# DamRsn/VocoderProject

Measured on AMD Instinct MI355X. Metric: STFT-geometry frames/sec (1024-pt frames, hop 256) through the pitch-corrector/vocoder path, higher is better.
Workload: dtype f64

## Files before the change

### include/vp_amd.h

```cpp
#ifndef VP_AMD_H
#define VP_AMD_H

#include <stddef.h>

#ifdef __cplusplus
extern "C" {
#endif

#define VP_ABI_VERSION 3

enum {
    VP_OK = 0,
    VP_ERR_INVALID_ARG = -1,
    VP_ERR_NOT_PREPARED = -2,
    VP_ERR_INVALID_OVERLAP = -3,
    VP_ERR_GEOMETRY = -4,
    VP_ERR_ORDER = -5,
    VP_ERR_NO_DEVICE = -6,
    VP_ERR_HIP = -7,
    VP_ERR_OOM = -8,
    VP_ERR_TIMEOUT = -9
};

typedef struct vp_params {
// ... 23 lines not shown

int vp_create(int device, vp_handle **out);
int vp_destroy(vp_handle *h);

int vp_set_params(vp_handle *h, const vp_params *p);
int vp_get_params(const vp_handle *h, vp_params *p);
int vp_set_stream_params(vp_handle *h, int stream, const vp_params *p);
int vp_get_stream_params(const vp_handle *h, int stream, vp_params *p);
void vp_default_params(vp_params *p);

int vp_set_pitch_shift(vp_handle *h, int stream, int on, double semitones);
int vp_get_pitch_shift(const vp_handle *h, int stream, int *on, double *semitones);

int vp_prepare_to_play(vp_handle *h, double sample_rate, int samples_per_block, int n_streams);

int vp_prepare_explicit(vp_handle *h, double sample_rate, int samples_per_block, int n_streams,
                        int frame_len_pitch, int hop_pitch, int wlen_voc, int hop_voc);

int vp_process_block(vp_handle *h, const float *in, float *out);

int vp_process_block_inplace(vp_handle *h, float *io);

int vp_process_block_device(vp_handle *h, const float *d_in, float *d_out, void *hip_stream);
int vp_process_block_mono(vp_handle *h, const float *voice, float *out);
int vp_process_block_mono_device(vp_handle *h, const float *d_voice, float *d_out, void *hip_stream);
int vp_process_blocks_mono_device(vp_handle *h, const float *d_voice, float *d_out, int n_blocks, void *hip_stream);
int vp_process_blocks_device(vp_handle *h, const float *d_in, float *d_out, int n_blocks, void *hip_stream);
int vp_process_blocks(vp_handle *h, const float *in, float *out, int n_blocks);
int vp_process_block_channels(vp_handle *h, const float *const *in, int n_in, float *const *out, int n_out);
int vp_process_block_channels_device(vp_handle *h, const float *const *d_in, int n_in, float *const *d_out, int n_out, void *hip_stream);
int vp_process_blocks_channels_device(vp_handle *h, const float *const *d_in, int n_in, float *const *d_out, int n_out, int n_blocks, void *hip_stream);
int vp_reserve_blocks(vp_handle *h, int n_blocks);
int vp_get_reserved_blocks(const vp_handle *h);
long vp_debug_alloc_count(const vp_handle *h);

#define VP_IIR_EXACT 0
#define VP_IIR_FAST 1
int vp_set_iir_mode(vp_handle *h, int mode);
int vp_get_iir_mode(const vp_handle *h);

#define VP_VOC_AUTO 0
#define VP_VOC_WORKGROUP 1
#define VP_VOC_BATCHED 2
int vp_set_vocoder_path(vp_handle *h, int path);
int vp_get_vocoder_path(const vp_handle *h);

#define VP_OVERLAP_AUTO 2
int vp_set_overlap(vp_handle *h, int on);
int vp_get_overlap(const vp_handle *h);
int vp_set_time_parallel(vp_handle *h, int on);
int vp_get_time_parallel(const vp_handle *h);
int vp_set_wave_specialised(vp_handle *h, int on);
int vp_get_wave_specialised(const vp_handle *h);

#define VP_YIN_DIRECT 0
#define VP_YIN_FFT 1
#define VP_YIN_XCORR 2
#define VP_YIN_XCORR_FORCE_FALLBACK 3
int vp_set_yin_mode(vp_handle *h, int mode);
int vp_get_yin_mode(const vp_handle *h);

int vp_get_latency(const vp_handle *h);
int vp_get_geometry(const vp_handle *h, int out[12]);
int vp_get_num_streams(const vp_handle *h);

int vp_read_pitch_state(vp_handle *h, int stream, vp_pitch_state *out);

int vp_synchronize(vp_handle *h);
int vp_debug_set_spin_limit(vp_handle *h, int polls);

#define VP_NUM_KERNEL_SLOTS 4
int vp_profile_enable(vp_handle *h, int on);
int vp_profile_read(vp_handle *h, double ms[VP_NUM_KERNEL_SLOTS], long launches[VP_NUM_KERNEL_SLOTS], int reset);
const char *vp_kernel_slot_name(int slot);
const char *vp_pitch_kernel_name(const vp_handle *h);
const char *vp_vocoder_kernel_name(const vp_handle *h);

int vp_read_ub_counters(vp_handle *h, long out[5]);

int vp_debug_read_stamps(vp_handle *h, unsigned long long out[64], int reset);
int vp_debug_read_ws_stamps(vp_handle *h, unsigned long long out[512], int reset);
int vp_debug_read_stream_ticks(vp_handle *h, unsigned long long *out, int n, int reset);

typedef struct vp_stft vp_stft;
int vp_stft_create(int device, int n_streams, int n_samples, int frame_len, int hop, vp_stft **out);
int vp_stft_destroy(vp_stft *p);
int vp_stft_num_frames(const vp_stft *p);
int vp_stft_roundtrip(vp_stft *p, const float *d_in, float *d_out, float *d_mag, void *hip_stream);
int vp_stft_pitch_shift(vp_stft *p, const float *d_in, float *d_out, double semitones, void *hip_stream);
int vp_stft_pitch_shift_curve(vp_stft *p, const float *d_in, float *d_out, const double *d_ratio, void *hip_stream);
int vp_stft_pitch_shift_locked(vp_stft *p, const float *d_in, float *d_out, const double *d_ratio, void *hip_stream);
int vp_stft_pitch_shift_locked_subbin(vp_stft *p, const float *d_in, float *d_out, const double *d_ratio, void *hip_stream);
#define VP_HARM_MAX_VOICES 4
int vp_stft_harmonize(vp_stft *p, const float *d_in, float *d_out, int n_voices, const double *d_ratio, const double *d_gain, const double *d_dry,
                      void *hip_stream);
#define VP_FORMANT_LIFTER_MIN 4
#define VP_FORMANT_LIFTER_MAX 64
int vp_stft_pitch_shift_formant(vp_stft *p, const float *d_in, float *d_out, const double *d_ratio, const double *d_formant, int lifter,
                                void *hip_stream);
int vp_stft_cross_synth(vp_stft *p, const float *d_voice, const float *d_carrier, float *d_out, const double *d_depth, int lifter, void *hip_stream);
int vp_semitones_to_ratios(const double *semitones, double *ratios, long n);
int vp_stft_time_stretch(vp_stft *p, const float *d_in, int n_in, const int *d_pos, float *d_out, double semitones, void *hip_stream);
int vp_stft_time_stretch_locked(vp_stft *p, const float *d_in, int n_in, const int *d_pos, float *d_out, const double *d_ratio, void *hip_stream);
int vp_stretch_positions(int *pos, int n_frames, int hop, double stretch, int n_in, int frame_len);
int vp_onset_num_frames(int n_in, int frame_len, int hop);
int vp_stft_onset_flux(vp_stft *p, const float *d_in, int n_in, double *d_flux, double *d_mass, void *hip_stream);
// ... 87 lines not shown
```

### vocoderproject_amd/build.py

```python
import os
import re
import shutil
import subprocess
import sys
import time

HERE = os.path.dirname(os.path.abspath(__file__))
CSRC = os.path.join(HERE, "csrc")
ROOT = os.path.dirname(HERE)
LIB = os.path.join(HERE, "libvp_amd.so")
SOURCES = ["vp_kernels.hip", "vp_voc2.hip", "vp_stft.hip", "vp_channels.hip", "vp_track.hip", "vp_capi.hip"]
ARCH = "gfx950"
NUM_TUS = 9


def deps_of(source):
    seen, todo = set(), [os.path.join(CSRC, source)]
    while todo:
        path = os.path.normpath(todo.pop())
        if path in seen:
            continue
        seen.add(path)
        with open(path, encoding="utf-8", errors="replace") as f:
            for inc in re.findall(r'^[ \t]*#[ \t]*include[ \t]*"([^"]+)"', f.read(), re.M):
                for d in (os.path.dirname(path), CSRC, os.path.join(ROOT, "include")):
                    if os.path.exists(os.path.join(d, inc)):
                        todo.append(os.path.join(d, inc))
                        break
    return sorted(seen)


DEP_PATHS = sorted({p for s in SOURCES for p in deps_of(s)})
DEPS = [os.path.basename(p) for p in DEP_PATHS]


def hipcc():
    return shutil.which("hipcc") or "/opt/rocm/bin/hipcc"


_HIPCC_VERSION = None


def hipcc_version():
    global _HIPCC_VERSION
    if _HIPCC_VERSION is None:
        try:
            _HIPCC_VERSION = subprocess.run([hipcc(), "--version"], capture_output=True, text=True, timeout=60).stdout
        except (OSError, subprocess.SubprocessError):
            _HIPCC_VERSION = "unknown"
    return _HIPCC_VERSION


def needs_build():
    if not os.path.exists(LIB):
        return True
    t = os.path.getmtime(LIB)
    return any(os.path.getmtime(p) > t for p in DEP_PATHS)


LIB_STAMPS = os.path.join(HERE, "libvp_amd_stamps.so")
LIB_POISON = os.path.join(HERE, "libvp_amd_poison.so")


CACHE_CAP_BYTES = 600 << 20


def prune_cache(cap=CACHE_CAP_BYTES):
    cache = os.path.join(HERE, ".build_cache")
    try:
        ents = []
        now = time.time()
        for f in os.listdir(cache):
            p = os.path.join(cache, f)
            try:
                if ".part" in f:
                    if now - os.path.getmtime(p) > 3600:
                        os.remove(p)
                    continue
                ents.append((os.path.getmtime(p), os.path.getsize(p), p))
            except OSError:
                pass
    except OSError:
        return
    total = sum(e[1] for e in ents)
    for _, size, path in sorted(ents):
        if total <= cap:
            break
        try:
            os.remove(path)
            total -= size
        except OSError:
            pass


def build(force=False, verbose=False, stamps=False, poison=False):
    lib = LIB_STAMPS if stamps else LIB_POISON if poison else (os.environ.get("VP_LIB_OUT") or LIB)
    if not stamps and not poison and not force and lib == LIB and not needs_build():
        return LIB
    import tempfile
    from concurrent.futures import ThreadPoolExecutor
    common = [hipcc(), "-std=c++17", "-O3", "-ffp-contract=off", "-fdenormal-fp-math=preserve-sign", "-fPIC", f"--offload-arch={ARCH}", "-Wall", "-Wno-unused-function",
              "-I", os.path.join(ROOT, "include"), "-I", CSRC]
    common += os.environ.get("VP_EXTRA_HIPCC_FLAGS", "").split()
    if stamps:
        common.append("-DVP_STAMPS")
    if poison:
        common.append("-DVP_POISON_LDS")
    groups = [0] if not (stamps or poison or os.environ.get("VP_SPLIT_BUILD") == "1") else list(range(1, NUM_TUS + 1))
    with tempfile.TemporaryDirectory(prefix="vp_build_") as tmp:
        jobs = [(os.path.join(CSRC, "vp_kernels.hip"), os.path.join(tmp, f"k{k}.o"), [f"-DVP_TU={k}"]) for k in groups]
        jobs.append((os.path.join(CSRC, "vp_voc2.hip"), os.path.join(tmp, "voc2.o"), []))
        jobs.append((os.path.join(CSRC, "vp_stft.hip"), os.path.join(tmp, "stft.o"), os.environ.get("VP_STFT_EXTRA_FLAGS", "-fno-slp-vectorize -ffp-contract=fast").split()))
        jobs.append((os.path.join(CSRC, "vp_channels.hip"), os.path.join(tmp, "channels.o"), []))
        jobs.append((os.path.join(CSRC, "vp_track.hip"), os.path.join(tmp, "track.o"), []))
        jobs.append((os.path.join(CSRC, "vp_capi.hip"), os.path.join(tmp, "capi.o"), []))

        def compile_one(job):
            import hashlib
            src, obj, extra = job
            cmd = common + extra + ["-c", src, "-o", obj]
            hsh = hashlib.sha256((hipcc_version() + " ".join(cmd[:-1]).replace(tmp, "")).encode())
            for dep in deps_of(src):
                with open(dep, "rb") as f:
                    hsh.update(f.read())
            cache = os.path.join(HERE, ".build_cache")
            os.makedirs(cache, exist_ok=True)
            cached = os.path.join(cache, os.path.basename(obj) + "." + hsh.hexdigest()[:20])
            if os.path.exists(cached) and not force and not os.environ.get("VP_NO_OBJ_CACHE"):
                try:
                    shutil.copy(cached, obj)
                    os.utime(cached)
                    return obj
                except OSError:
                    pass
            if verbose:
                print(" ".join(cmd))
            subprocess.check_call(cmd)
            part = cached + ".part%d" % os.getpid()
            shutil.copy(obj, part)
            os.replace(part, cached)
            return obj

        with ThreadPoolExecutor(len(jobs)) as ex:
            objs = list(ex.map(compile_one, jobs))
        prune_cache()
        link = [hipcc(), "-shared", "-fPIC", f"--offload-arch={ARCH}"] + objs + ["-o", lib]
        if verbose:
            print(" ".join(link))
        subprocess.check_call(link)
    return lib


if __name__ == "__main__":
    print(build(force="--force" in sys.argv, verbose=True, stamps="--stamps" in sys.argv, poison="--poison" in sys.argv))
```

### vocoderproject_amd/csrc/vp_capi.hip

```cpp
#include <hip/hip_runtime.h>

#include <algorithm>
#include <cmath>
#include <cstdint>
#include <cstdio>
#include <cstdlib>
#include <cstring>
#include <string>
#include <type_traits>
#include <vector>

#include "../../include/vp_amd.h"
#include "vp_kernels.h"
#include "vp_voc2.h"
#include "vp_stft.h"
#include "vp_channels.h"
#include "vp_track.h"

struct vp_handle {
    int device = 0;
    bool prepared = false;
    vp_params params;
    VpGeom g;
    VpDev d;
    int inCounter = 0, outCounter = 0, currCounter = 0;
    struct Cohort { int pitchOn, vocOn, vStart, pStart, nChunk, n; int *dMap; std::vector<int> ids; int ordHi = 0, oVmax = 0, oSmax = 0; };
    std::vector<Cohort> cohorts;
    bool cohortsDirty = false;
    int *dMapAll = nullptr;
    std::vector<int> mapHost;
    bool poisoned = false;
    int poisonCode = VP_ERR_HIP;
    unsigned int *faultHost = nullptr, *faultDev = nullptr;
    int spinLimit = 1 << 22;
    VpV2 v2;
    int vocPath = VP_VOC_AUTO, oVmax = 0, oSmax = 0, nWinMax = 0;
    VpV2 v2mb;
    int v2mbWin = 0;
    std::vector<void *> mbAllocs;
    float *snapV = nullptr, *snapS = nullptr; int *gateB = nullptr; double *pLin = nullptr;
    std::vector<void *> bothAllocs;
    hipStream_t auxStream = nullptr;
    hipEvent_t evFork = nullptr, evJoin = nullptr;
    double *acc2 = nullptr;
    int overlap = VP_OVERLAP_AUTO, acc2Live = 0;
    int accLive = 0;
    int waveSpec = 1;
    int timeParallel = 0;
    std::vector<void *> allocs;
    float *stageIn = nullptr, *stageOut = nullptr;
    int synthNonZero = 0;
    float *stageInB = nullptr, *stageOutB = nullptr; int stageBlocks = 0;
    int reservedBlocks = 0;
    float *chHostIn = nullptr, *chHostOut = nullptr;
    long nAllocs = 0;
    hipStream_t ownStream = nullptr;
    int vocWaves = 8;
    size_t vocLds = 0, pitchLds = 0, ldsMax = 0;
    int prof = 0;
    unsigned profTick = 0;
    bool profThis = false;
    int iirMode = 0, yinMode = 0;
    std::vector<vp_params> sparams;
    std::vector<VpStreamParams> spHost;
    std::vector<int> shiftOn;
    std::vector<double> shiftSemi, shiftBeta;
    bool perStream = false, spDirty = false;
    struct EvPair { hipEvent_t a, b; int slot; };
    std::vector<EvPair> pending;
    std::vector<hipEvent_t> evPool;
    double profMs[VP_NUM_KERNEL_SLOTS] = {0, 0, 0, 0};
    long profN[VP_NUM_KERNEL_SLOTS] = {0, 0, 0, 0};
    std::string lastError;
};

static int fail_hip(vp_handle *h, hipError_t e, const char *what)
{
    char buf[256];
    snprintf(buf, sizeof buf, "%s: %s", what, hipGetErrorString(e));
    if (h) h->lastError = buf;
    return VP_ERR_HIP;
}
#define HIPCHK(h, call) do { hipError_t _e = (call); if (_e != hipSuccess) return fail_hip((h), _e, #call); } while (0)

static int poisoned_rc(vp_handle *h)
{
    h->lastError = h->poisonCode == VP_ERR_TIMEOUT
        ? "an earlier launch timed out on an inter-wavefront wait (its output and the device state are void): prepare again"
        : "an earlier HIP failure left the handle out of step with its device state: prepare again";
    return h->poisonCode;
}
static int check_fault(vp_handle *h)
{
    if (!h->faultHost) return VP_OK;
    const unsigned f = *(volatile unsigned int *)h->faultHost;
    if (f == 0) return VP_OK;
    h->poisoned = true; h->poisonCode = VP_ERR_TIMEOUT;
    char buf[200];
    snprintf(buf, sizeof buf, "a kernel's bounded wait ran out (counter dbg[%u], see vp_debug_read_stamps): the block's output is invalid; prepare again", f & 0xff);
    h->lastError = buf;
// ... 17 lines not shown
    case VP_ERR_INVALID_OVERLAP: return "Invalid overlap";
    case VP_ERR_GEOMETRY: return "invalid frame geometry";
    case VP_ERR_ORDER: return "LPC order is larger than OrderMax";
    case VP_ERR_NO_DEVICE: return "no HIP device (this library has no CPU fallback)";
    case VP_ERR_HIP: return "HIP runtime error";
    case VP_ERR_OOM: return "out of device memory";
    case VP_ERR_TIMEOUT: return "a kernel's bounded inter-wavefront wait ran out: the output is invalid, prepare again";
    default: return "unknown error";
    }
}

extern "C" const char *vp_last_error(const vp_handle *h) { return h ? h->lastError.c_str() : ""; }

static bool pitch_lite(const vp_handle *h, bool iirFast)
{
    return h->g.S > 256 && (iirFast || h->g.orderPitch <= 16) && h->pitchLds <= 80 * 1024 && h->g.htabGlobal;
}

static bool pitch_common_geom(const vp_handle *h)
{
    return (h->g.C & 63) == 0 && h->g.orderPitch <= 15 && h->g.tauMax <= 512 && h->g.eLen >= h->g.F + 4 * h->g.tauMax + 1;
}
static bool pitch_common(const vp_handle *h)
{
    return pitch_common_geom(h) && (h->g.F == 512 || h->g.F == 1024) && h->pitchLds + 16 + vp_pitch_fft_lds_bytes(2 * (h->g.F >> 9)) <= h->ldsMax;
}

typedef void (*vp_dsp_kernel)(VpGeom, VpCall, VpDev, const float *, float *);
struct PitchPlan { vp_dsp_kernel fn; const char *name; size_t lds; };
#define VP_PLAN(K, LDS) PitchPlan{K, #K, LDS}
static PitchPlan pitch_plan(const vp_handle *h, bool fast, int nBlocks)
{
    const bool lite = pitch_lite(h, fast), com = lite ? pitch_common_geom(h) : pitch_common(h);
    const size_t lds = h->pitchLds;
    if (nBlocks > 1) {
        if (lite) return com ? VP_PLAN(vp_k_pitch_lite_fast_multi_c, lds) : VP_PLAN(vp_k_pitch_lite_fast_multi, lds);
        return fast ? (com ? VP_PLAN(vp_k_pitch_fast_multi_c, lds) : VP_PLAN(vp_k_pitch_fast_multi, lds)) : VP_PLAN(vp_k_pitch_multi, lds);
    }
    if (lite) return fast ? (com ? VP_PLAN(vp_k_pitch_lite_fast_c, lds) : VP_PLAN(vp_k_pitch_lite_fast, lds)) : VP_PLAN(vp_k_pitch_lite, lds);
    if (com) return fast ? VP_PLAN(vp_k_pitch_fast_c, lds) : VP_PLAN(vp_k_pitch_c, lds);
    return fast ? VP_PLAN(vp_k_pitch_fast, lds) : VP_PLAN(vp_k_pitch, lds);
}
static bool pitch_ws_ok(const vp_handle *h, bool fast, int nBlocks, int nSteps)
{
    static const bool off = getenv("VP_NO_WS") != nullptr;
    const VpGeom &g = h->g;
    if (off || !h->waveSpec || nBlocks != 1 || nSteps <= 0 || pitch_lite(h, fast) || g.F != 1024 || (g.C & 63) != 0 || g.C > 512 || g.cpf < 2 ||
        g.orderPitch > WS_ORDER_MAX || g.tauMax > 512) return false;
    if ((size_t)(g.toKeep + g.F + (nSteps - 1) * g.C) >= (size_t)g.inSize) return false;
    if (nSteps + (nSteps + g.cpf - 2) / (g.cpf - 1) + 1 > WS_MAXI || (nSteps + g.cpf - 2) / (g.cpf - 1) + 1 > WS_MAXS) return false;
    return vp_pitch_ws_lds_bytes(g, nSteps) + 256 <= h->ldsMax;
}

static int pitch_xfft_waves(const vp_handle *h, bool fast, int nBlocks)
{
    if (!pitch_common(h) || pitch_lite(h, fast) || (nBlocks > 1 && !fast)) return 0;
    int fw = 2 * (h->g.F >> 9);
    static const int envWaves = [] { const char *e = getenv("VP_XFFT_WAVES"); return e ? atoi(e) : 0; }();
    if (envWaves == fw / 2) fw = envWaves;
    return fw;
}
static size_t pitch_xfft_lds(const vp_handle *h) { return vp_pitch_fft_lds_bytes(2 * (h->g.F >> 9)); }
#undef VP_PLAN

extern "C" const char *vp_pitch_kernel_name(const vp_handle *h)
{
    if (!h || !h->prepared) return "";
    const bool fast = h->iirMode == VP_IIR_FAST;
    if (pitch_ws_ok(h, fast, 1, (h->g.N + h->g.C - 1) / h->g.C))
        return h->g.orderPitch > 15 ? (fast ? "vp_k_pitch_ws_o24" : "vp_k_pitch_ws_x_o24") : (fast ? "vp_k_pitch_ws" : "vp_k_pitch_ws_x");
    return pitch_plan(h, fast, 1).name;
}

static int voc_lite_slots(const vp_handle *h, bool iirFast, int nw)
{
    if (!(h->g.S > 256 && iirFast) || getenv("VP_VOC_NO_LITE")) return 0;
    int nl = std::max(1, std::min(nw, 4));
    while (nl > 1 && vp_voc_lds_bytes(h->g.W, nl) > (size_t)(80 * 1024 - 512)) nl--;
    return vp_voc_lds_bytes(h->g.W, nl) <= (size_t)(80 * 1024 - 512) ? nl : 0;
}

#define VP_V2_MIN_STREAMS 257
#define VP_V2_MIN_WINDOWS 1024
static bool voc_auto_batched(const vp_handle *h)
{
    return h->g.S >= VP_V2_MIN_STREAMS && (size_t)h->g.S * h->nWinMax >= VP_V2_MIN_WINDOWS;
}
static bool voc_pipeline_wanted(const vp_handle *h)
{
    return h->v2.xT && h->vocPath != VP_VOC_WORKGROUP && (h->vocPath == VP_VOC_BATCHED || voc_auto_batched(h));
}
static bool voc_batched_for(const vp_handle *h, int nWin, int oV, int oS)
{
    if (!voc_pipeline_wanted(h) || nWin < 1 || nWin > 64) return false;
    return oV <= V2_ORDER_MAX && oS <= VP_ORDER_MAX_SYNTH && oV >= 2 && oS >= 2;
}

static bool voc_o48(int oVmax) { return oVmax > 32 && oVmax <= 48; }

extern "C" int vp_set_vocoder_path(vp_handle *h, int path)
{
    if (!h || path < VP_VOC_AUTO || path > VP_VOC_BATCHED) return VP_ERR_INVALID_ARG;
    if (path != h->vocPath) h->cohortsDirty = true;
    h->vocPath = path;
    return VP_OK;
}
extern "C" int vp_get_vocoder_path(const vp_handle *h) { return h ? h->vocPath : VP_ERR_INVALID_ARG; }
extern "C" int vp_set_overlap(vp_handle *h, int on)
{
    if (!h || on < 0 || on > VP_OVERLAP_AUTO) return VP_ERR_INVALID_ARG;
    h->overlap = on;
    return VP_OK;
}
extern "C" int vp_get_overlap(const vp_handle *h) { return h ? h->overlap : VP_ERR_INVALID_ARG; }
extern "C" int vp_set_time_parallel(vp_handle *h, int on)
{
    if (!h) return VP_ERR_INVALID_ARG;
    h->timeParallel = on ? 1 : 0;
    return VP_OK;
}
extern "C" int vp_get_time_parallel(const vp_handle *h) { return h ? h->timeParallel : VP_ERR_INVALID_ARG; }
extern "C" int vp_set_wave_specialised(vp_handle *h, int on)
{
    if (!h) return VP_ERR_INVALID_ARG;
    h->waveSpec = on ? 1 : 0;
    return VP_OK;
}
extern "C" int vp_get_wave_specialised(const vp_handle *h) { return h ? h->waveSpec : VP_ERR_INVALID_ARG; }

extern "C" const char *vp_vocoder_kernel_name(const vp_handle *h)
{
    if (!h || !h->prepared) return "";
    {
        int oV = 0, oS = 0, nLow = 0;
        for (const auto &q : h->sparams) if (q.lpcVoice <= V2_ORDER_MAX) { oV = std::max(oV, q.lpcVoice); oS = std::max(oS, q.lpcSynth); nLow++; }
        if (nLow > 0 && voc_batched_for(h, h->nWinMax, oV, oS)) return "vp_k_v2_pipeline";
    }
    if (voc_lite_slots(h, h->iirMode == VP_IIR_FAST, h->vocWaves)) return "vp_k_vocoder_lite";
    int oV = 0;
    for (const auto &q : h->sparams) oV = std::max(oV, q.lpcVoice);
    return (oV > 32 && oV <= 48) ? "vp_k_vocoder_o48" : "vp_k_vocoder";
}

extern "C" const char *vp_kernel_slot_name(int slot)
{
    static const char *n[VP_NUM_KERNEL_SLOTS] = {"vp_k_ingest_gate", "vp_k_vocoder", "vp_k_pitch", "vp_k_emit"};
    return (slot >= 0 && slot < VP_NUM_KERNEL_SLOTS) ? n[slot] : "";
}

extern "C" void vp_default_params(vp_params *p)
{
    p->gainPitch = 0.0f; p->gainVoice = -60.0f; p->gainSynth = -60.0f; p->gainVoc = 0.0f;
    p->lpcVoice = 40; p->lpcPitch = 15; p->lpcSynth = 5; p->keyPitch = 12;
    p->pitchBool = 1; p->vocBool = 1;
}

static bool params_valid(const vp_params *p)
{
    auto gain_ok = [](float v) { return v >= -60.0f && v <= 6.0f; };
    return gain_ok(p->gainPitch) && gain_ok(p->gainVoice) && gain_ok(p->gainSynth) && gain_ok(p->gainVoc) &&
           p->lpcVoice >= 2 && p->lpcVoice <= VP_ORDER_MAX && p->lpcPitch >= 2 && p->lpcPitch <= VP_ORDER_MAX &&
           p->lpcSynth >= 2 && p->lpcSynth <= VP_ORDER_MAX_SYNTH && p->keyPitch >= 0 && p->keyPitch <= 12 &&
           (p->pitchBool == 0 || p->pitchBool == 1) && (p->vocBool == 0 || p->vocBool == 1);
}

extern "C" int vp_create(int device, vp_handle **out)
{
    if (!out) return VP_ERR_INVALID_ARG;
    *out = nullptr;
    int n = 0;
    if (hipGetDeviceCount(&n) != hipSuccess || n <= 0) return VP_ERR_NO_DEVICE;
    if (device < 0 || device >= n) return VP_ERR_INVALID_ARG;
    vp_handle *h = new vp_handle();
    h->device = device;
    vp_default_params(&h->params);
    memset(&h->g, 0, sizeof h->g);
    memset(&h->d, 0, sizeof h->d);
    if (hipSetDevice(device) != hipSuccess || hipStreamCreateWithFlags(&h->ownStream, hipStreamNonBlocking) != hipSuccess ||
        hipStreamCreateWithFlags(&h->auxStream, hipStreamNonBlocking) != hipSuccess ||
        hipEventCreateWithFlags(&h->evFork, hipEventDisableTiming) != hipSuccess ||
// ... 257 lines not shown
    int rc = fill_voc_window(vocWin, W, hop);
    if (rc) return rc;
    rc = fill_pitch_st_window(pitchSt, F, H);
    if (rc) return rc;

    std::vector<int> hannOff(g.tauMax + 1, 0);
    size_t tot = 0;
    for (int T = 1; T <= g.tauMax; T++) { hannOff[T] = (int)tot; tot += 2 * (size_t)T + 1; }
    std::vector<double> hannTab(tot);
    for (int T = 1; T <= g.tauMax; T++) fill_hann(hannTab.data() + hannOff[T], 2 * T + 1);

    std::vector<double> notes(13 * VP_NOTES_STRIDE, 0.0);
    std::vector<int> notesN(13);
    for (int k = 0; k < 13; k++) notesN[k] = build_notes(k, fMin, fMax, notes.data() + (size_t)k * VP_NOTES_STRIDE);

    hipDeviceProp_t prop;
    HIPCHK(h, hipGetDeviceProperties(&prop, h->device));
    const size_t ldsMax = std::min<size_t>((size_t)prop.maxSharedMemoryPerMultiProcessor ? prop.maxSharedMemoryPerMultiProcessor : 65536, 160 * 1024) - 256;
    g.xsSteps = 1;
    g.htabGlobal = 0;
    if (g.S > 256) {
        VpGeom t = g;
        t.xsSteps = 1;
        if (vp_pitch_lds_bytes(t) <= (size_t)80 * 1024) g.htabGlobal = 1;
    }
    {
        const int stepsMax = (N + g.C - 1) / g.C;
        size_t budget = std::min<size_t>(ldsMax, (g.S > 256 ? 80 : 112) * 1024);
        {
            VpGeom t = g;
            t.xsSteps = 1;
            if (vp_pitch_lds_bytes(t) > budget) budget = ldsMax;
        }
        for (int k = stepsMax; k >= 1; k--) {
            VpGeom t = g;
            t.xsSteps = k;
            if ((size_t)(g.toKeep + F + (k - 1) * g.C) < (size_t)g.inSize && vp_pitch_lds_bytes(t) <= budget) { g.xsSteps = k; break; }
        }
    }
    h->pitchLds = vp_pitch_lds_bytes(g);
    h->ldsMax = ldsMax;
    if (h->pitchLds > ldsMax) { h->lastError = "pitch frame does not fit LDS"; return VP_ERR_GEOMETRY; }
    int nw = 8;
    while (nw > 1 && vp_voc_lds_bytes(W, nw) > ldsMax) nw--;
    if (const char *e = getenv("VP_VOC_WAVES")) { int v = atoi(e); if (v >= 1 && v < nw) nw = v; }
    if (vp_voc_lds_bytes(W, nw) > ldsMax) { h->lastError = "vocoder window does not fit LDS"; return VP_ERR_GEOMETRY; }
    h->vocWaves = nw;
    h->vocLds = vp_voc_lds_bytes(W, nw);
    {
        const void *fns[] = {(const void *)vp_k_pitch, (const void *)vp_k_pitch_fast, (const void *)vp_k_pitch_multi,
                             (const void *)vp_k_pitch_fast_multi, (const void *)vp_k_pitch_lite, (const void *)vp_k_pitch_lite_fast,
                             (const void *)vp_k_pitch_c, (const void *)vp_k_pitch_fast_c, (const void *)vp_k_pitch_fast_multi_c,
                             (const void *)vp_k_pitch_lite_fast_c, (const void *)vp_k_pitch_lite_fast_multi, (const void *)vp_k_pitch_lite_fast_multi_c,
                             (const void *)vp_k_pitch_ws, (const void *)vp_k_pitch_ws_x, (const void *)vp_k_pitch_ws_mb, (const void *)vp_k_pitch_ws_x_mb, (const void *)vp_k_pitch_ws_mb_o24, (const void *)vp_k_pitch_ws_x_mb_o24, (const void *)vp_k_pitch_ws_o24, (const void *)vp_k_pitch_ws_x_o24,
                             (const void *)vp_k_vocoder, (const void *)vp_k_vocoder_o48, (const void *)vp_k_vocoder_lite};
        for (const void *f : fns) {
            hipFuncAttributes fa;
            HIPCHK(h, hipFuncGetAttributes(&fa, f));
            HIPCHK(h, hipFuncSetAttribute(f, hipFuncAttributeMaxDynamicSharedMemorySize, (int)(ldsMax + 256 - fa.sharedSizeBytes)));
        }
    }

    VpDev d;
    memset(&d, 0, sizeof d);
    RC(dev_alloc(h, &d.voiceRing, (size_t)S * g.inSize));
    RC(dev_alloc(h, &d.synthRing, (size_t)S * 2 * g.inSize));
    RC(dev_alloc(h, &d.outAcc, (size_t)S * g.outSize));
    RC(dev_alloc(h, &h->acc2, (size_t)S * g.outSize));
    h->acc2Live = 0; h->accLive = 0;
    RC(dev_alloc(h, &d.gate, (size_t)S * 2));
    RC(dev_alloc(h, &d.pitch, (size_t)S));
    RC(dev_alloc(h, &d.eFrame, (size_t)S * g.eLen));
    RC(dev_alloc(h, &d.outEFrame, (size_t)S * F));
    RC(dev_alloc(h, &d.yFrame, (size_t)S * F));
    RC(dev_alloc(h, &d.EeArr, (size_t)S * 20));
    RC(dev_alloc(h, &d.hImp, (size_t)S * 128));
    RC(dev_alloc(h, &d.ub, (size_t)5));
    RC(dev_alloc(h, &d.dbg, (size_t)64 + (size_t)S + 512));
    vocWin.resize((size_t)W + 16, 0.0);
    RC(dev_upload(h, &d.vocWin, vocWin));
    RC(dev_upload(h, &d.pitchStWin, pitchSt));
    RC(dev_upload(h, &d.hannTab, hannTab));
    RC(dev_upload(h, &d.hannOff, hannOff));
    RC(dev_upload(h, &d.notes, notes));
    RC(dev_upload(h, &d.notesN, notesN));
    {
        const double PI = 3.141592653589793238;
        std::vector<double> t1(64 * 8 * 2), t2(64 * 8 * 2), ts(64 * 4 * 2);
        for (int lane = 0; lane < 64; lane++) {
            for (int r = 0; r < 8; r++) {
                const double a1 = -2.0 * PI * (double)(r * (lane >> 3)) / 64.0, a2 = -2.0 * PI * (double)(r * lane) / 512.0;
                t1[(lane * 8 + r) * 2] = std::cos(a1); t1[(lane * 8 + r) * 2 + 1] = std::sin(a1);
                t2[(lane * 8 + r) * 2] = std::cos(a2); t2[(lane * 8 + r) * 2 + 1] = std::sin(a2);
            }
            for (int q = 0; q < 4; q++) {
                const double a = -2.0 * PI * (double)(64 * q + lane) / 1024.0;
                ts[(lane * 4 + q) * 2] = std::cos(a); ts[(lane * 4 + q) * 2 + 1] = std::sin(a);
            }
        }
        RC(dev_upload(h, &d.fftTw1, t1));
        RC(dev_upload(h, &d.fftTw2, t2));
        RC(dev_upload(h, &d.fftTws, ts));
    }
    RC(dev_alloc(h, &h->dMapAll, (size_t)S));
    {
        memset(&h->v2, 0, sizeof h->v2);
        h->nWinMax = (N + hop - 1) / hop;
        const size_t NW = (size_t)S * h->nWinMax;
        if (h->nWinMax <= 64 && vp_v2_init() == 0) {
            h->v2.nGroupsMax = (int)((NW + 63) / 64);
            h->v2.W4p = (W + 3) / 4 + 16;
            h->v2.W2p = (W + 1) / 2 + 2;
            RC(dev_alloc(h, &h->v2.xT, (size_t)2 * h->v2.nGroupsMax * h->v2.W4p * 256));
            RC(dev_alloc(h, &h->v2.eT, (size_t)2 * h->v2.nGroupsMax * h->v2.W2p * 128));
            RC(dev_alloc(h, &h->v2.out, NW * W));
            const size_t NWp = (size_t)h->v2.nGroupsMax * 64;
            RC(dev_alloc(h, &h->v2.rV, NWp * V2_RV_STRIDE));
            RC(dev_alloc(h, &h->v2.aV, NWp * V2_RV_STRIDE));
            RC(dev_alloc(h, &h->v2.rS, NWp * V2_RS_STRIDE));
            RC(dev_alloc(h, &h->v2.aS, NWp * V2_RS_STRIDE));
            RC(dev_alloc(h, &h->v2.meta, NWp));
            RC(dev_alloc(h, &h->v2.rank, NWp + S));
            RC(dev_alloc(h, &h->v2.liveList, NWp));
            RC(dev_alloc(h, &h->v2.EE, NW * 2));
            h->v2.nSlices = (W + V2_FIR_SLICE - 1) / V2_FIR_SLICE;
            RC(dev_alloc(h, &h->v2.EEp, NW * 2 * h->v2.nSlices));
        }
    }
    RC(dev_alloc(h, &h->stageIn, (size_t)S * 3 * N, false));
    RC(dev_alloc(h, &h->stageOut, (size_t)S * 3 * N, false));
    if (hipHostMalloc((void **)&h->chHostIn, (size_t)S * 3 * N * sizeof(float), hipHostMallocDefault) != hipSuccess ||
        hipHostMalloc((void **)&h->chHostOut, (size_t)S * 2 * N * sizeof(float), hipHostMallocDefault) != hipSuccess) {
        (void)hipGetLastError();
        free_all(h);
        h->lastError = "out of pinned host memory for the channel staging buffers";
        return VP_ERR_OOM;
    }
    {
        std::vector<VpPitchState> init(S);
        memset(init.data(), 0, init.size() * sizeof(VpPitchState));
        for (auto &p : init) p.beta = 1;
        if (hipMemcpy(d.pitch, init.data(), init.size() * sizeof(VpPitchState), hipMemcpyHostToDevice) != hipSuccess) {
            free_all(h);
            return VP_ERR_HIP;
        }
    }
    d.fault = h->faultDev; d.spinLimit = h->spinLimit;
    *(volatile unsigned int *)h->faultHost = 0;
    h->g = g;
    h->d = d;
    h->inCounter = g.toKeep + g.latency;
    h->outCounter = 0;
    h->currCounter = g.toKeep;
    h->cohorts.assign(1, vp_handle::Cohort{h->params.pitchBool, h->params.vocBool, 0, 0, 0, S, nullptr, {}});
    h->cohortsDirty = false; h->poisoned = false; h->poisonCode = VP_ERR_HIP;
    h->sparams.assign((size_t)S, h->params);
    h->spHost.assign((size_t)S, VpStreamParams{});
    h->synthNonZero = 0;
    h->shiftOn.assign((size_t)S, 0); h->shiftSemi.assign((size_t)S, 0.0); h->shiftBeta.assign((size_t)S, 1.0);
    h->perStream = false; h->spDirty = true;
    h->prepared = true;
    (void)hipDeviceSynchronize();
    return VP_OK;
}

extern "C" int vp_prepare_to_play(vp_handle *h, double sampleRate, int samplesPerBlock, int nStreams)
{
    if (!h || !(sampleRate > 0)) return VP_ERR_INVALID_ARG;
    double ratioSR = sampleRate / 44100.0;
    int hopVoc = (int)std::floor(128.0 * ratioSR);
    int wlenVoc = 4 * hopVoc;
    int corres_256 = (int)std::floor(256.0 * ratioSR);
    int hopPitch = 3 * corres_256;
    int frameLenPitch = 4 * corres_256;
    return vp_prepare_explicit(h, sampleRate, samplesPerBlock, nStreams, frameLenPitch, hopPitch, wlenVoc, hopVoc);
}

static hipEvent_t get_event(vp_handle *h)
{
    if (!h->evPool.empty()) { hipEvent_t e = h->evPool.back(); h->evPool.pop_back(); return e; }
    hipEvent_t e;
    (void)hipEventCreate(&e);
    return e;
}

struct ProfScope {
    vp_handle *h; hipStream_t st; int slot; hipEvent_t a, b; bool on;
    ProfScope(vp_handle *h_, hipStream_t st_, int slot_) : h(h_), st(st_), slot(slot_)
    {
        on = h->profThis;
        if (on) { a = get_event(h); b = get_event(h); (void)hipEventRecord(a, st); }
    }
    ~ProfScope()
    {
        if (on) { (void)hipEventRecord(b, st); h->pending.push_back({a, b, slot}); }
    }
};

static void fill_stream_params(VpStreamParams &o, const vp_params &P)
{
    o.orderVoice = P.lpcVoice; o.orderSynth = P.lpcSynth; o.key = P.keyPitch;
    o.dryOn = ((double)P.gainVoice > -59.0);
    o.synthOn = ((double)P.gainSynth > -59.0);
    o.gainPitch = (double)db_to_gain_f(P.gainPitch);
    o.gainVoc = (double)db_to_gain_f(P.gainVoc);
    o.gainVoice = (double)db_to_gain_f(P.gainVoice);
    o.gainSynth = (double)db_to_gain_f(P.gainSynth);
}
// ... 68 lines not shown
    if (rc) return rc;
    VpCall c0;
    memset(&c0, 0, sizeof c0);
    c0.inCounter = h->inCounter; c0.outCounter = h->outCounter; c0.currCounter = h->currCounter;
    c0.inplace = inplace;
    c0.iirFast = h->iirMode;
    c0.nBlocks = 1;
    if (mono) {
        c0.inMono = h->synthNonZero > 0 ? 1 : 2;
        h->synthNonZero = std::max(0, h->synthNonZero - g.N * nBlocks);
    } else {
        c0.inMono = 0;
        h->synthNonZero = g.inSize;
    }
    c0.yinCert = (h->yinMode == VP_YIN_XCORR || h->yinMode == VP_YIN_FFT) ? 1 : (h->yinMode == VP_YIN_XCORR_FORCE_FALLBACK) ? 2 : 0;

    for (auto &co : h->cohorts) {
        VpCall c = c0;
        VpDev d = h->d;
        d.streamMap = co.dMap;
        d.outAcc2 = h->acc2Live > 0 ? h->acc2 : nullptr;
        c.pitchOn = co.pitchOn; c.vocOn = co.vocOn;
        c.vStart = co.vStart;
        c.nWin = 0;
        if (c.vocOn && co.vStart < g.N) c.nWin = (g.N - co.vStart + g.h - 1) / g.h;
        c.pStart = co.pStart; c.nChunk0 = co.nChunk;
        c.nSteps = 0;
        if (c.pitchOn && co.pStart < g.N) c.nSteps = (g.N - co.pStart + g.C - 1) / g.C;

        const bool runVoc = c.nWin > 0, runPitch = c.nSteps > 0 || (nBlocks > 1 && c.pitchOn);
        bool runPitchDone = false;
        if (!runVoc && !runPitch) {
            { ProfScope ps(h, st, 0); hipLaunchKernelGGL(vp_k_ingest_gate, dim3(co.n), dim3(256), 0, st, g, c, d, d_in); }
            { ProfScope ps(h, st, 3); hipLaunchKernelGGL(vp_k_emit, dim3(co.n), dim3(256), 0, st, g, c, d, d_out); }
        } else {
            const bool batched = runVoc && voc_batched_for(h, c.nWin, co.oVmax, co.oSmax);
            if (batched && runPitch && c.iirFast && nBlocks == 1 && (h->overlap == 1 || (h->overlap == VP_OVERLAP_AUTO && !pitch_lite(h, true)))) {
                struct Fork { vp_handle *h; hipStream_t st; VpGeom g; VpCall cp; VpDev dp; const float *in; float *out; int n; hipError_t err; } fk;
                fk.h = h; fk.st = st; fk.g = g; fk.cp = c; fk.dp = d; fk.in = d_in; fk.out = d_out; fk.n = co.n; fk.err = hipSuccess;
                fk.cp.fuseIngest = 0; fk.cp.fuseEmit = 0; fk.cp.nBlocks = 1;
                fk.dp.outAcc = h->acc2; fk.dp.outAcc2 = nullptr;
                auto fork = [](void *a) {
                    Fork *f = (Fork *)a;
                    vp_handle *h = f->h;
                    if ((f->err = hipEventRecord(h->evFork, f->st)) != hipSuccess) return;
                    if ((f->err = hipStreamWaitEvent(h->auxStream, h->evFork, 0)) != hipSuccess) return;
                    ProfScope ps(h, h->auxStream, 2);
                    PitchPlan plan = pitch_plan(h, true, 1);
                    if (const int fw = f->cp.yinCert ? pitch_xfft_waves(h, true, 1) : 0) {
                        const size_t off = (plan.lds + 15) / 16 * 16;
                        f->cp.fftOff = (int)off; f->cp.fftWaves = fw; plan.lds = off + pitch_xfft_lds(h);
                    }
                    f->cp.ldsBytes = (int)plan.lds;
                    hipLaunchKernelGGL(plan.fn, dim3(f->n), dim3(512), plan.lds, h->auxStream, f->g, f->cp, f->dp, f->in, f->out);
                };
                VpCall cv = c;
                cv.fuseIngest = 1; cv.fuseEmit = 0;
                VpV2 v = h->v2;
                v.nStreams = co.n; v.oVmax = co.oVmax; v.oSmax = co.oSmax;
                { ProfScope ps(h, st, 1); vp_v2_launch(g, cv, d, v, d_in, d_out, st, fork, &fk); }
                if (fk.err != hipSuccess) return fail_hip(h, fk.err, "fork of the pitch kernel");
                HIPCHK(h, hipEventRecord(h->evJoin, h->auxStream));
                HIPCHK(h, hipStreamWaitEvent(st, h->evJoin, 0));
                VpDev de = d;
                de.outAcc2 = h->acc2;
                { ProfScope ps(h, st, 3); hipLaunchKernelGGL(vp_k_emit, dim3(co.n), dim3(256), 0, st, g, c, de, d_out); }
                h->acc2Live = (g.outSize + g.N - 1) / g.N + 1;
                runPitchDone = true;
            } else if (batched) {
                VpCall cv = c;
                cv.fuseIngest = 1; cv.fuseEmit = runPitch ? 0 : 1;
                ProfScope ps(h, st, 1);
                VpV2 v = h->v2;
                v.nStreams = co.n; v.oVmax = co.oVmax; v.oSmax = co.oSmax;
                vp_v2_launch(g, cv, d, v, d_in, d_out, st);
            } else if (runVoc) {
                VpCall cv = c;
                cv.fuseIngest = 1; cv.fuseEmit = runPitch ? 0 : 1;
                ProfScope ps(h, st, 1);
                int nw = std::min(h->vocWaves, c.nWin);
                if (nw < 4) nw = std::min(4, h->vocWaves);
                const int nl = voc_lite_slots(h, cv.iirFast != 0, nw);
                const bool lite = nl > 0;
                if (lite) nw = nl;
                cv.ldsBytes = (int)vp_voc_lds_bytes(g.W, nw);
                cv.vocWin = nw;
                const int nThreads = 64 * nw * std::max(1, 8 / nw);
                hipLaunchKernelGGL(lite ? vp_k_vocoder_lite : voc_o48(co.oVmax) ? vp_k_vocoder_o48 : vp_k_vocoder, dim3(co.n), dim3(nThreads), vp_voc_lds_bytes(g.W, nw), st,
                                   g, cv, d, d_in, d_out);
            }
            if (runPitch && !runPitchDone) {
                VpCall cp = c;
                cp.fuseIngest = runVoc ? 0 : 1; cp.fuseEmit = 1;
                cp.nBlocks = nBlocks;
                ProfScope ps(h, st, 2);
                PitchPlan plan = pitch_plan(h, cp.iirFast != 0, nBlocks);
                const int fw = cp.yinCert ? pitch_xfft_waves(h, cp.iirFast != 0, nBlocks) : 0;
                const size_t fftMin = fw ? pitch_xfft_lds(h) + 16 : 0;
                if (nBlocks == 1 && !pitch_lite(h, cp.iirFast != 0) && plan.lds + vp_pitch_acc_lds_bytes(g) + 16 + fftMin <= h->ldsMax) {
                    cp.ldsAcc = 1;
                    plan.lds = ((plan.lds + 15) / 16) * 16 + vp_pitch_acc_lds_bytes(g);
                }
                if (fw) {
                    const size_t off = (plan.lds + 15) / 16 * 16;
                    cp.fftOff = (int)off; cp.fftWaves = fw; plan.lds = off + pitch_xfft_lds(h);
                }
                cp.ldsBytes = (int)plan.lds;
                if (pitch_ws_ok(h, cp.iirFast != 0, nBlocks, cp.nSteps)) {
                    cp.ldsAcc = 1; cp.fftOff = 0; cp.fftWaves = 0;
                    cp.ldsBytes = (int)vp_pitch_ws_lds_bytes(g, cp.nSteps);
                    static const int wsWaves = [] { const char *e = getenv("VP_WS_WAVES"); const int v = e ? atoi(e) : 0; return (v >= 8 && v <= 12) ? v : 12; }();
                    VpWsSched sc;
                    memset(&sc, 0, sizeof sc);
                    if (!ws_build_sched(g, cp.nChunk0, cp.nSteps, sc)) return fail_hip(h, hipErrorInvalidValue, "pitch schedule");
                    const auto wsk = g.orderPitch > 15 ? (cp.iirFast ? vp_k_pitch_ws_o24 : vp_k_pitch_ws_x_o24) : (cp.iirFast ? vp_k_pitch_ws : vp_k_pitch_ws_x);
                    hipLaunchKernelGGL(wsk, dim3(co.n), dim3(64 * wsWaves), (size_t)cp.ldsBytes, st, g, cp, d, sc, d_in, d_out);
                } else
                hipLaunchKernelGGL(plan.fn, dim3(co.n), dim3(512), plan.lds, st, g, cp, d, d_in, d_out);
            }
        }
        hipError_t e = hipGetLastError();
        if (e != hipSuccess) return fail_hip(h, e, "kernel launch");

        for (int b = 0; b < nBlocks; b++) {
            if (co.vocOn) {
                const int nWin = (co.vStart < g.N) ? (g.N - co.vStart + g.h - 1) / g.h : 0;
                co.vStart = co.vStart + nWin * g.h - g.N;
            }
            if (co.pitchOn) {
                const int nSteps = (co.pStart < g.N) ? (g.N - co.pStart + g.C - 1) / g.C : 0;
                int nChunk = co.nChunk;
                for (int i = 0; i < nSteps; i++) {
                    if (nChunk % g.cpf == g.cpf - 1) nChunk = 1 % g.cpf;
                    else nChunk += 1;
                }
                co.nChunk = nChunk;
                co.pStart = co.pStart + nSteps * g.C - g.N;
            }
        }
    }
    for (auto &co : h->cohorts)
        if (co.vocOn) h->accLive = (g.outSize + g.N - 1) / g.N + 1;
    h->acc2Live = std::max(0, h->acc2Live - nBlocks);
    h->accLive = std::max(0, h->accLive - nBlocks);
    for (int b = 0; b < nBlocks; b++) {
        h->outCounter = (h->outCounter + g.N) % g.outSize;
        h->inCounter = (h->inCounter + g.N) % g.inSize;
        h->currCounter = (h->currCounter + g.N) % g.inSize;
    }
    guard.armed = false;
    return VP_OK;
}

extern "C" int vp_process_block_device(vp_handle *h, const float *d_in, float *d_out, void *hip_stream)
{
    if (!h || !d_in || !d_out) return VP_ERR_INVALID_ARG;
    if (!h->prepared) return VP_ERR_NOT_PREPARED;
    if (hipSetDevice(h->device) != hipSuccess) return VP_ERR_NO_DEVICE;
    return process_device(h, d_in, d_out, (hipStream_t)hip_stream, 0);
}

static int ensure_v2mb(vp_handle *h, int nWin)
{
    if (nWin <= h->v2mbWin) return VP_OK;
    for (void *p : h->mbAllocs) (void)hipFree(p);
    h->mbAllocs.clear(); h->v2mbWin = 0;
    const VpGeom &g = h->g;
    VpV2 v;
    memset(&v, 0, sizeof v);
    const size_t NW = (size_t)g.S * nWin;
    v.nGroupsMax = (int)((NW + 63) / 64);
// ... 113 lines not shown
    *done = false;
    const VpGeom &g = h->g;
    if (h->cohorts.size() != 1 || nb < 2 || nb > V2_MB_MAX || h->iirMode != VP_IIR_FAST) return VP_OK;
    { const int mn = v2_mb_min_blocks(h, h->cohorts[0], true); if (mn == 0 || nb < mn) return VP_OK; }
    auto &co = h->cohorts[0];
    if (!co.vocOn || !co.pitchOn || !voc_pipeline_wanted(h)) return VP_OK;
    if (co.oVmax > V2_ORDER_MAX || co.oSmax > VP_ORDER_MAX_SYNTH || co.oVmax < 2 || co.oSmax < 2) return VP_OK;
    if ((size_t)g.outSize * sizeof(double) > (size_t)VP_V2_MB_LDS_MAX) return VP_OK;
    VpV2MB mb;
    memset(&mb, 0, sizeof mb);
    mb.nBlocks = nb; mb.preIngested = 1;
    int vs = co.vStart, NWs = 0;
    for (int b = 0; b < nb; b++) {
        const int nWin = (vs < g.N) ? (g.N - vs + g.h - 1) / g.h : 0;
        mb.vStart[b] = vs; mb.nWin[b] = nWin; mb.first[b] = NWs;
        NWs += nWin;
        vs = vs + nWin * g.h - g.N;
    }
    if (NWs < 1 || mb.nWin[0] < 1) return VP_OK;
    for (int b = 1; b < nb; b++)
        if (mb.nWin[b] > 0 && b * g.N + mb.vStart[b] != mb.vStart[0] + mb.first[b] * g.h) return VP_OK;
    if (h->poisoned) return poisoned_rc(h);
    if (int frc = check_fault(h)) return frc;
    if (NWs > h->v2mbWin || !h->pLin) return VP_OK;
    h->profThis = h->prof > 0 && (h->profTick++ % (unsigned)h->prof) == 0;
    struct Poison { vp_handle *h; bool armed; ~Poison() { if (armed) h->poisoned = true; } } guard{h, true};
    HIPCHK(h, hipMemcpyAsync(h->snapV, h->d.voiceRing, (size_t)g.S * g.inSize * sizeof(float), hipMemcpyDeviceToDevice, st));
    HIPCHK(h, hipMemcpyAsync(h->snapS, h->d.synthRing, (size_t)g.S * 2 * g.inSize * sizeof(float), hipMemcpyDeviceToDevice, st));
    VpCall c;
    memset(&c, 0, sizeof c);
    c.inCounter = h->inCounter; c.outCounter = h->outCounter; c.currCounter = h->currCounter;
    c.iirFast = 1; c.nBlocks = nb; c.inMono = 0; c.vocOn = 1; c.pitchOn = 1;
    c.yinCert = (h->yinMode == VP_YIN_XCORR || h->yinMode == VP_YIN_FFT) ? 1 : (h->yinMode == VP_YIN_XCORR_FORCE_FALLBACK) ? 2 : 0;
    VpDev d = h->d;
    d.streamMap = co.dMap;
    d.gateB = h->gateB;
    {
        VpGeom gp = g;
        gp.outSize = V2_MB_MAX * g.N + g.outSize;
        VpCall cp = c;
        cp.outCounter = 0;
        cp.pStart = co.pStart; cp.nChunk0 = co.nChunk;
        cp.nSteps = (co.pStart < g.N) ? (g.N - co.pStart + g.C - 1) / g.C : 0;
        cp.fuseIngest = 1; cp.fuseEmit = 0; cp.pitchLin = 1;
        VpDev dp = d;
        dp.outAcc = h->pLin; dp.outAcc2 = nullptr;
        PitchPlan plan = pitch_plan(h, true, nb);
        if (const int fw = cp.yinCert ? pitch_xfft_waves(h, true, nb) : 0) {
            const size_t off = (plan.lds + 15) / 16 * 16;
            cp.fftOff = (int)off; cp.fftWaves = fw; plan.lds = off + pitch_xfft_lds(h);
        }
        cp.ldsBytes = (int)plan.lds;
        ProfScope ps(h, st, 2);
        hipLaunchKernelGGL(plan.fn, dim3(co.n), dim3(512), plan.lds, st, gp, cp, dp, d_in, d_out);
    }
    {
        VpCall cv = c;
        cv.vStart = mb.vStart[0]; cv.nWin = NWs; cv.fuseIngest = 1; cv.fuseEmit = 1;
        VpDev dv = d;
        dv.voiceRing = h->snapV; dv.synthRing = h->snapS;
        dv.pLin = h->pLin;
        dv.outAcc2 = h->acc2Live > 0 ? h->acc2 : nullptr;
        VpV2 v = h->v2mb;
        v.nStreams = co.n; v.oVmax = co.oVmax; v.oSmax = co.oSmax;
        ProfScope ps(h, st, 1);
        vp_v2_launch_blocks(g, cv, dv, v, mb, d_in, d_out, st);
    }
    hipError_t e = hipGetLastError();
    if (e != hipSuccess) return fail_hip(h, e, "kernel launch");
    co.vStart = vs;
    for (int b = 0; b < nb; b++) {
        const int nSteps = (co.pStart < g.N) ? (g.N - co.pStart + g.C - 1) / g.C : 0;
        int nChunk = co.nChunk;
        for (int i = 0; i < nSteps; i++) nChunk = (nChunk % g.cpf == g.cpf - 1) ? 1 % g.cpf : nChunk + 1;
        co.nChunk = nChunk;
        co.pStart = co.pStart + nSteps * g.C - g.N;
    }
    h->synthNonZero = g.inSize;
    h->acc2Live = std::max(0, h->acc2Live - nb);
    h->accLive = (g.outSize + g.N - 1) / g.N;
    for (int b = 0; b < nb; b++) {
        h->outCounter = (h->outCounter + g.N) % g.outSize;
        h->inCounter = (h->inCounter + g.N) % g.inSize;
        h->currCounter = (h->currCounter + g.N) % g.inSize;
    }
    guard.armed = false;
    *done = true;
    return VP_OK;
}

static int process_ws_blocks(vp_handle *h, const float *d_in, float *d_out, int nb, hipStream_t st, bool mono, bool *done)
{
    *done = false;
    static const bool off = getenv("VP_NO_WS_MB") != nullptr;
    const VpGeom &g = h->g;
    const bool fast = h->iirMode == VP_IIR_FAST;
    if (off || h->cohorts.size() != 1 || nb < 2 || nb > WS_MB_MAX) return VP_OK;
    auto &co = h->cohorts[0];
    if (!co.pitchOn || co.vocOn || co.pStart != 0 || g.N % g.C != 0 || g.N < g.C) return VP_OK;
    const int nSteps = g.N / g.C;
    if (!pitch_ws_ok(h, fast, 1, nSteps)) return VP_OK;
    {
        const int nt = 768, span = g.toKeep + g.F + (nSteps - 1) * g.C;
        if (g.N > 2 * nt || g.C > nt || span - g.N > 3 * nt || span < g.N || g.latency > g.F + (nSteps - 1) * g.C || g.latency < g.N) return VP_OK;
    }
    if (h->poisoned) return poisoned_rc(h);
    if (int frc = check_fault(h)) return frc;
    VpWsMb mb;
    memset(&mb, 0, sizeof mb);
    mb.nBlocks = nb;
    int nSched = 0, schedChunk[WS_MB_SCHEDS];
    int nChunk = co.nChunk, inC = h->inCounter, outC = h->outCounter, curC = h->currCounter;
    for (int b = 0; b < nb; b++) {
        int k = 0;
        while (k < nSched && schedChunk[k] != nChunk) k++;
        if (k == nSched) {
            if (nSched == WS_MB_SCHEDS) return VP_OK;
            if (!ws_build_sched(g, nChunk, nSteps, mb.sc[nSched])) return VP_OK;
            schedChunk[nSched++] = nChunk;
        }
        mb.schedOf[b] = k; mb.nChunk0[b] = nChunk; mb.inCtr[b] = inC; mb.outCtr[b] = outC; mb.currCtr[b] = curC;
        for (int i = 0; i < nSteps; i++) nChunk = (nChunk % g.cpf == g.cpf - 1) ? 1 % g.cpf : nChunk + 1;
        inC = (inC + g.N) % g.inSize; outC = (outC + g.N) % g.outSize; curC = (curC + g.N) % g.inSize;
    }
    h->profThis = h->prof > 0 && (h->profTick++ % (unsigned)h->prof) == 0;
    VpCall c;
    memset(&c, 0, sizeof c);
    c.inCounter = h->inCounter; c.outCounter = h->outCounter; c.currCounter = h->currCounter;
    c.iirFast = fast ? 1 : 0; c.nBlocks = 1; c.pitchOn = 1; c.vocOn = 0;
    c.pStart = 0; c.nChunk0 = co.nChunk; c.nSteps = nSteps;
    c.fuseIngest = 1; c.fuseEmit = 1; c.ldsAcc = 1;
    if (mono) {
        c.inMono = h->synthNonZero > 0 ? 1 : 2;
        h->synthNonZero = std::max(0, h->synthNonZero - g.N * nb);
    } else {
        c.inMono = 0;
        h->synthNonZero = g.inSize;
    }
    c.yinCert = (h->yinMode == VP_YIN_XCORR || h->yinMode == VP_YIN_FFT) ? 1 : (h->yinMode == VP_YIN_XCORR_FORCE_FALLBACK) ? 2 : 0;
    c.ldsBytes = (int)vp_pitch_ws_lds_bytes(g, nSteps);
    VpDev d = h->d;
    d.streamMap = co.dMap;
    d.outAcc2 = nullptr;
    {
        ProfScope ps(h, st, 2);
        const auto wsk = g.orderPitch > 15 ? (fast ? vp_k_pitch_ws_mb_o24 : vp_k_pitch_ws_x_mb_o24) : (fast ? vp_k_pitch_ws_mb : vp_k_pitch_ws_x_mb);
        hipLaunchKernelGGL(wsk, dim3(co.n), dim3(64 * 12), (size_t)c.ldsBytes, st, g, c, d, mb, d_in, d_out);
    }
    hipError_t e = hipGetLastError();
    if (e != hipSuccess) { h->poisoned = true; h->poisonCode = VP_ERR_HIP; return fail_hip(h, e, "kernel launch"); }
    co.nChunk = nChunk;
    h->inCounter = inC; h->outCounter = outC; h->currCounter = curC;
    h->acc2Live = std::max(0, h->acc2Live - nb);
    h->accLive = std::max(0, h->accLive - nb);
    *done = true;
    return VP_OK;
}

static int process_blocks_device(vp_handle *h, const float *d_in, float *d_out, int n_blocks, void *hip_stream, bool mono)
{
    if (!h || !d_in || !d_out || n_blocks < 1) return VP_ERR_INVALID_ARG;
    if (!h->prepared) return VP_ERR_NOT_PREPARED;
    if (hipSetDevice(h->device) != hipSuccess) return VP_ERR_NO_DEVICE;
    if (h->poisoned) return process_device(h, d_in, d_out, (hipStream_t)hip_stream, 0, 1, mono);
    int rc = sync_stream_state(h, (hipStream_t)hip_stream);
    if (rc) { h->poisoned = true; return rc; }
    const bool fast = h->iirMode == VP_IIR_FAST;
    const bool pitchOnly = h->cohorts.size() == 1 && h->cohorts[0].pitchOn && !h->cohorts[0].vocOn;
    const bool wsBlocks = pitchOnly && pitch_ws_ok(h, fast, 1, (h->g.N + h->g.C - 1) / h->g.C);
    if (wsBlocks && n_blocks > 1 && h->acc2Live == 0 && h->accLive == 0) {
        const size_t nIn_ = (size_t)h->g.S * (mono ? 1 : 3) * h->g.N, nOut_ = (size_t)h->g.S * 2 * h->g.N;
        while (n_blocks > 1) {
            const int nb = std::min(n_blocks, WS_MB_MAX);
            bool done = false;
            rc = process_ws_blocks(h, d_in, d_out, nb, (hipStream_t)hip_stream, mono, &done);
            if (rc) return rc;
            if (!done) break;
            d_in += nb * nIn_; d_out += nb * nOut_; n_blocks -= nb;
        }
        if (n_blocks == 0) return VP_OK;
    }
    if (pitchOnly && n_blocks > 1 && !wsBlocks && (!pitch_lite(h, fast) || fast))
        return process_device(h, d_in, d_out, (hipStream_t)hip_stream, 0, n_blocks, mono);
    const size_t nIn = (size_t)h->g.S * (mono ? 1 : 3) * h->g.N, nOut = (size_t)h->g.S * 2 * h->g.N;
    if (!mono && n_blocks > 1 && !wsBlocks) {
        int b = 0;
        while (b < n_blocks) {
            const int nb = std::min(n_blocks - b, std::min(V2_MB_MAX, std::max(h->reservedBlocks, 1)));
            bool done = false;
            rc = process_voc_blocks(h, d_in + b * nIn, d_out + b * nOut, nb, (hipStream_t)hip_stream, &done);
            if (rc) return rc;
            if (!done) rc = process_both_blocks(h, d_in + b * nIn, d_out + b * nOut, nb, (hipStream_t)hip_stream, &done);
            if (rc) return rc;
            if (!done) break;
            b += nb;
        }
        if (b == n_blocks) return VP_OK;
        d_in += b * nIn; d_out += b * nOut; n_blocks -= b;
    }
    for (int b = 0; b < n_blocks; b++) {
// ... 1324 lines not shown
```

### vocoderproject_amd/csrc/vp_common.h

```cpp
#pragma once
#include <stddef.h>

#define VP_MARKS 64
#define VP_ORDER_MAX 100
#define VP_ORDER_MAX_SYNTH 30
#define VP_NOTES_STRIDE 89

struct VpGeom {
    int S, N, F, H, C, cpf, W, h, toKeep, latency, inSize, outSize, tauMax;
    int eLen;
    int orderPitch;
    int tau0;
    int bufferIdxMax;
    int xsSteps;
    int htabGlobal;
    double fs, delta, yinTol;
    double gateThrSum;
    double levEps;
    double eeFloor;
};

struct VpCall {
    int inCounter, outCounter, currCounter;
    int vStart, nWin;
// ... 132 lines not shown
        nCh += 1;
    }
    sc.nInst = nI; sc.nStart = nS; sc.nSeg = nG;
    for (int q = 0; q <= WS_MAXS; q++) {
#ifdef WS_PARK_EVERY
        sc.segPark[q] = (q < nG) ? 1 : 0;
#else
        sc.segPark[q] = (nS > 0 && q == nG - 1) ? 1 : 0;
#endif
    }
    return nI > 0;
}

#define WS_MB_MAX 16
#define WS_MB_SCHEDS 4
struct VpWsMb {
    int nBlocks;
    int schedOf[WS_MB_MAX], nChunk0[WS_MB_MAX], inCtr[WS_MB_MAX], outCtr[WS_MB_MAX], currCtr[WS_MB_MAX];
    VpWsSched sc[WS_MB_SCHEDS];
};

struct WsCarve {
    int xs, eF, fr, qtab, htab, P, dY, gtab, r, aPrev, hp, aF, xp, hist, tw, oA, st, ctl, end;
};
VP_HD static inline int ws_even(int v) { return (v + 1) & ~1; }
VP_HD static inline WsCarve ws_carve(const VpGeom &g, int nSteps)
{
    WsCarve c;
    int o = 0;
    c.xs = o;    o += ws_even(g.toKeep + g.F + (nSteps - 1) * g.C + 4);
    c.eF = o;    o += ws_even(g.eLen);
    c.fr = o;    o += 4 * g.F + 2048;
    c.qtab = o;  o += ws_even(2 * g.tauMax + 4);
    c.htab = o;  o += ws_even(2 * g.tauMax + 2);
    c.P = o;     o += ws_even(g.F + g.tauMax + 2 > 450 ? g.F + g.tauMax + 2 : 450);
    c.dY = o;    o += ws_even(vp_dy_len(g.tauMax) + 1);
    c.gtab = o;  o += 2 * VP_MARKS + (6 * VP_MARKS + 1) / 2 + 1;
    o = ws_even(o);
    c.r = o;     o += 2 * 64;
    c.aPrev = o; o += 2 * (VP_ORDER_MAX + 1 + 1);
    c.hp = o;    o += 2 * WS_HP(g);
    c.aF = o;    o += 2 * WS_AF(g);
    c.xp = o;    o += (g.orderPitch > 15 ? 128 : 64);
    c.hist = o;  o += 2 * WS_HIST(g);
    c.tw = o;    o += 2 * VP_FFT_TW_D2;
    c.oA = o;    o += ws_even(g.N + g.C + 1);
    c.st = o;    o += 2 * ((int)(sizeof(VpPitchState) + 15) / 16 * 2);
    c.ctl = o;   o += ((int)sizeof(WsCtl) + 7) / 8;
    c.end = ws_even(o);
    return c;
}
VP_HD static inline size_t vp_pitch_ws_lds_bytes(const VpGeom &g, int nSteps) { return (size_t)ws_carve(g, nSteps).end * sizeof(double); }

VP_HD static inline size_t voc_wave_doubles(int W)
{
    return (size_t)4 * W + 2 * (VP_ORDER_MAX + 1) + 2 * (VP_ORDER_MAX_SYNTH + 1) + 2;
}
#define VP_VOC_SHARED_DOUBLES(W) ((size_t)(W) + 20 + 16 + 8)
```

### vocoderproject_amd/csrc/vp_kernels.h

```cpp
#pragma once
#include <hip/hip_runtime.h>

#include "vp_common.h"

__global__ void vp_k_ingest_gate(VpGeom g, VpCall c, VpDev d, const float *__restrict__ in);
__global__ void vp_k_vocoder(VpGeom g, VpCall c, VpDev d, const float *__restrict__ in, float *__restrict__ out);
__global__ void vp_k_vocoder_o48(VpGeom g, VpCall c, VpDev d, const float *__restrict__ in, float *__restrict__ out);
__global__ void vp_k_vocoder_lite(VpGeom g, VpCall c, VpDev d, const float *__restrict__ in, float *__restrict__ out);
__global__ void vp_k_pitch(VpGeom g, VpCall c, VpDev d, const float *__restrict__ in, float *__restrict__ out);
__global__ void vp_k_pitch_lite(VpGeom g, VpCall c, VpDev d, const float *__restrict__ in, float *__restrict__ out);
__global__ void vp_k_pitch_fast(VpGeom g, VpCall c, VpDev d, const float *__restrict__ in, float *__restrict__ out);
__global__ void vp_k_pitch_lite_fast(VpGeom g, VpCall c, VpDev d, const float *__restrict__ in, float *__restrict__ out);
__global__ void vp_k_pitch_multi(VpGeom g, VpCall c, VpDev d, const float *__restrict__ in, float *__restrict__ out);
__global__ void vp_k_pitch_fast_multi(VpGeom g, VpCall c, VpDev d, const float *__restrict__ in, float *__restrict__ out);
__global__ void vp_k_pitch_c(VpGeom g, VpCall c, VpDev d, const float *__restrict__ in, float *__restrict__ out);
__global__ void vp_k_pitch_fast_c(VpGeom g, VpCall c, VpDev d, const float *__restrict__ in, float *__restrict__ out);
__global__ void vp_k_pitch_fast_multi_c(VpGeom g, VpCall c, VpDev d, const float *__restrict__ in, float *__restrict__ out);
__global__ void vp_k_pitch_lite_fast_c(VpGeom g, VpCall c, VpDev d, const float *__restrict__ in, float *__restrict__ out);
__global__ void vp_k_pitch_lite_fast_multi(VpGeom g, VpCall c, VpDev d, const float *__restrict__ in, float *__restrict__ out);
__global__ void vp_k_pitch_lite_fast_multi_c(VpGeom g, VpCall c, VpDev d, const float *__restrict__ in, float *__restrict__ out);
__global__ void vp_k_pitch_ws(VpGeom g, VpCall c, VpDev d, VpWsSched sc, const float *__restrict__ in, float *__restrict__ out);
__global__ void vp_k_pitch_ws_x(VpGeom g, VpCall c, VpDev d, VpWsSched sc, const float *__restrict__ in, float *__restrict__ out);
__global__ void vp_k_pitch_ws_mb(VpGeom g, VpCall c, VpDev d, VpWsMb mb, const float *__restrict__ in, float *__restrict__ out);
__global__ void vp_k_pitch_ws_x_mb(VpGeom g, VpCall c, VpDev d, VpWsMb mb, const float *__restrict__ in, float *__restrict__ out);
__global__ void vp_k_pitch_ws_mb_o24(VpGeom g, VpCall c, VpDev d, VpWsMb mb, const float *__restrict__ in, float *__restrict__ out);
__global__ void vp_k_pitch_ws_x_mb_o24(VpGeom g, VpCall c, VpDev d, VpWsMb mb, const float *__restrict__ in, float *__restrict__ out);
__global__ void vp_k_pitch_ws_o24(VpGeom g, VpCall c, VpDev d, VpWsSched sc, const float *__restrict__ in, float *__restrict__ out);
__global__ void vp_k_pitch_ws_x_o24(VpGeom g, VpCall c, VpDev d, VpWsSched sc, const float *__restrict__ in, float *__restrict__ out);
__global__ void vp_k_emit(VpGeom g, VpCall c, VpDev d, float *__restrict__ out);


static inline size_t vp_pitch_fft_lds_bytes(int waves) { return 64 + (size_t)VP_FFT_TW_D2 * 16 + (size_t)waves * 8192; }
static inline size_t vp_voc_lds_bytes(int W, int nWaves)
{
    return (VP_VOC_SHARED_DOUBLES(W) + (size_t)nWaves * voc_wave_doubles(W)) * sizeof(double);
}
```

### vocoderproject_amd/csrc/vp_kernels.hip

```cpp
#include <hip/hip_runtime.h>
#include <utility>
#include <limits.h>

#include "vp_common.h"

#ifndef VP_TU
#define VP_TU 0
#endif
#define VP_TU_HAS(K) (VP_TU == 0 || VP_TU == (K))
#define VP_NUM_TUS 6

#define WAVE 64

#ifndef VP_LEV_SCALAR_MIN
#define VP_LEV_SCALAR_MIN 41
#endif

typedef __attribute__((address_space(3))) double lds_f64;
typedef __attribute__((address_space(3))) float lds_f32;
typedef __attribute__((address_space(3))) int lds_i32;

struct VpTmo { unsigned long long *ctr; unsigned int *fault; int limit; };
__device__ __forceinline__ VpTmo vp_tmo(const VpDev &d, int slot) { VpTmo t; t.ctr = &d.dbg[slot]; t.fault = d.fault; t.limit = d.spinLimit; return t; }
__device__ __forceinline__ void vp_timeout(const VpTmo &t, int slot = 61)
{
    atomicAdd(t.ctr, 1ULL);
    if (t.fault) __hip_atomic_store(t.fault, (unsigned)(0x100 | slot), __ATOMIC_RELAXED, __HIP_MEMORY_SCOPE_SYSTEM);
}

#ifdef VP_STAMPS
__device__ unsigned long long vp_last_stamp;
#define STAMP(D, ID) do { if (blockIdx.x == 0 && threadIdx.x == 0) { unsigned long long _t = wall_clock64(); \
        (D).dbg[ID] += _t - vp_last_stamp; vp_last_stamp = _t; } } while (0)
#define STAMP0(D) do { if (blockIdx.x == 0 && threadIdx.x == 0) { vp_last_stamp = wall_clock64(); vp_dbg_g = (D).dbg; } } while (0)
__device__ unsigned long long *vp_dbg_g;
__device__ unsigned long long vp_last_g;
#define STAMPG_BEGIN() do { if (blockIdx.x == 0 && threadIdx.x == 0) vp_last_g = wall_clock64(); } while (0)
#define STAMPG(ID) do { if (blockIdx.x == 0 && threadIdx.x == 0) { unsigned long long _t = wall_clock64(); \
        vp_dbg_g[ID] += _t - vp_last_g; vp_last_g = _t; } } while (0)
__device__ unsigned long long vp_last_l;
#define STAMPL_BEGIN() do { if (blockIdx.x == 0 && threadIdx.x == blockDim.x - 1) vp_last_l = wall_clock64(); } while (0)
#define STAMPL(ID) do { if (blockIdx.x == 0 && threadIdx.x == blockDim.x - 1) { unsigned long long _t = wall_clock64(); \
        vp_dbg_g[ID] += _t - vp_last_l; vp_last_l = _t; } } while (0)
__device__ unsigned long long vp_last_w[16];
#define STAMPW_BEGIN() do { if (blockIdx.x == 0 && (threadIdx.x & 63) == 0) vp_last_w[threadIdx.x >> 6] = wall_clock64(); } while (0)
#define STAMPW(ID) do { if (blockIdx.x == 0 && (threadIdx.x & 63) == 0) { unsigned long long _t = wall_clock64(); \
        vp_dbg_g[(ID) + (threadIdx.x >> 6)] += _t - vp_last_w[threadIdx.x >> 6]; vp_last_w[threadIdx.x >> 6] = _t; } } while (0)
#else
#define STAMPW_BEGIN() do { } while (0)
#define STAMPW(ID) do { } while (0)
#define STAMPL_BEGIN() do { } while (0)
#define STAMPL(ID) do { } while (0)
#define STAMPG_BEGIN() do { } while (0)
#define STAMPG(ID) do { } while (0)
#define STAMP(D, ID) do { } while (0)
#define STAMP0(D) do { } while (0)
#endif

#ifndef VP_LPC_FAST
#define VP_LPC_FAST 1
#endif
#ifndef VP_ACR_AHEAD
#define VP_ACR_AHEAD 1
// ... 240 lines not shown
```

### vocoderproject_amd/csrc/vp_pitch_ws.inc

```

#ifdef VP_STAMPS
#define WS_SLOT(D, W, E) (D).dbg[64 + g.S + (c.nChunk0 & 3) * 128 + (W) * 8 + (E)]
#define WS_EV(D, W, E) do { if (blockIdx.x == 0 && (threadIdx.x & 63) == 0) atomicAdd(&WS_SLOT(D, W, E), (unsigned long long)wall_clock64()); } while (0)
#define WS_EV0(D, W, E) do { if (blockIdx.x == 0 && threadIdx.x == 0) atomicAdd(&WS_SLOT(D, W, E), (unsigned long long)wall_clock64()); } while (0)
#define WS_TB() unsigned long long ws_tb_ = wall_clock64()
#define WS_TA(D, W, E) do { if (blockIdx.x == 0 && (threadIdx.x & 63) == 0) { const unsigned long long t_ = wall_clock64(); atomicAdd(&WS_SLOT(D, W, E), t_ - ws_tb_); ws_tb_ = t_; } } while (0)
#define WS_TR() do { ws_tb_ = wall_clock64(); } while (0)
#define WS_FINE(D, K) do { if (i == 0) WS_EV(D, 12 + (K) / 8, (K) % 8); } while (0)
#define WS_FINEP(D, K) do { if (si == 0 && rank < 2) WS_EV(D, 13 + rank, K); } while (0)
#define WS_FINER(D, J) do { if ((J) < 7) WS_EV(D, 15, J); } while (0)
#define WS_STAT(D, K, V) do { if (blockIdx.x == 0 && (threadIdx.x & 63) == 0) atomicAdd(&(D).dbg[64 + g.S + (K)], (unsigned long long)(V)); } while (0)
#define WS_CLK() wall_clock64()
#else
#define WS_EV(D, W, E) do { } while (0)
#define WS_EV0(D, W, E) do { } while (0)
#define WS_TB() do { } while (0)
#define WS_TA(D, W, E) do { } while (0)
#define WS_TR() do { } while (0)
#define WS_FINE(D, K) do { } while (0)
#define WS_FINEP(D, K) do { } while (0)
#define WS_FINER(D, J) do { } while (0)
#define WS_STAT(D, K, V) do { } while (0)
#define WS_CLK() 0ULL
#endif

typedef __attribute__((address_space(3))) WsCtl lds_ctl;
__device__ __forceinline__ void ws_wait_ge(lds_i32 *flag, int target, const VpDev &d)
{
    int spin = 0;
    while (__hip_atomic_load(flag, __ATOMIC_ACQUIRE, __HIP_MEMORY_SCOPE_WORKGROUP) < target) {
        if (++spin >= d.spinLimit) { if ((vp_tid() & 63) == 0) vp_timeout(vp_tmo(d, 61)); break; }
        __builtin_amdgcn_s_sleep(1);
    }
}
__device__ __forceinline__ void ws_signal(lds_i32 *flag, int value)
{
    __threadfence_block();
    if ((vp_tid() & 63) == 0) __hip_atomic_store(flag, value, __ATOMIC_RELEASE, __HIP_MEMORY_SCOPE_WORKGROUP);
}
__device__ __forceinline__ void ws_group_barrier(lds_i32 *ctr, int n, int &gen, const VpDev &d)
{
    gen += 1;
    __threadfence_block();
    if ((vp_tid() & 63) == 0) __hip_atomic_fetch_add(ctr, 1, __ATOMIC_RELEASE, __HIP_MEMORY_SCOPE_WORKGROUP);
    ws_wait_ge(ctr, n * gen, d);
}

__device__ __forceinline__ void ws_prefix_sums(const lds_f64 *w, lds_f64 *P, int nb)
{
    asm volatile("" : "+s"(nb));
    const int lane = vp_tid() & 63, per = (nb + WAVE - 1) / WAVE, j0 = lane * per;
    double v[24];
#pragma unroll
    for (int u = 0; u < 24; u++) { const int j = j0 + u; v[u] = (u < per && j < nb) ? w[min(j, nb - 1)] : 0.0; }
    double loc = 0.0;
#pragma unroll
    for (int u = 0; u < 24; u++) { const int j = j0 + u; if (u < per && j < nb) loc += v[u] * v[u]; }
    double inc = loc;
    for (int off = 1; off < WAVE; off <<= 1) { const double o = __shfl_up(inc, off, WAVE); if (lane >= off) inc += o; }
    double run = inc - loc;
#pragma unroll
    for (int u = 0; u < 24; u++) { const int j = j0 + u; if (u < per && j <= nb) { P[j] = run; if (j < nb) run += v[u] * v[u]; } }
}

__device__ __forceinline__ void ws_yin_pick_wave(const VpGeom &g, const VpDev &d, const PitchLds &L, lds_state *st)
{
    const int lane = vp_tid() & 63;
    for (int k = 1 + lane; k < g.tauMax; k += WAVE) {
        const double cm = L.cum[k], q = (double)k / cm;
        L.dY[k] = L.dY[k] * q;
    }
    wave_sync();
    int tau = INT_MAX;
    for (int k0 = g.tau0; k0 < g.tauMax; k0 += WAVE) {
        const int k = k0 + lane;
        const unsigned long long m = __ballot(k < g.tauMax && L.dY[min(k, g.tauMax - 1)] < g.yinTol);
        if (m) { tau = k0 + (int)__builtin_ctzll(m); break; }
    }
    if (tau < g.tauMax) {
        while (true) {
            const double a = L.dY[tau + 1], b = L.dY[tau];
            if (!(a < b)) break;
            tau += 1;
            if (tau + 1 >= g.tauMax) break;
        }
        if (lane == 0) {
            if (tau >= g.tauMax) atomicAdd(&d.ub[3], 1ULL);
            st->pitch = g.fs / tau;
            st->period = tau;
        }
    }
}


struct SegTab {
    lds_f64 *x0, *xN;
    lds_i32 *stMark, *srcBase, *flags, *startIdx, *stopIdx, *eLim;
};
// ... 8 lines not shown
__device__ __forceinline__ void ws_psola_table_seg(const VpGeom &g, const VpDev &d, const lds_state *st, lds_state *stIdx, const SegTab &G, int kFirst, int kLast,
                                                   int pSFirst, lds_ctl *ctl, int sg, bool park)
{
    const int lane = vp_tid() & 63;
    const int T = (st->pitch > 1) ? st->period : st->prevVoicedPeriod;
    const int nG = 2 * T + 1;
    const int nSt = st->nSt;
    const int smi0 = stIdx->stMarkIdx;
    const int smi = smi0 + lane;
    const bool have = smi < nSt;
    const int stMark = have ? st->stMarks[smi] : 0;
    const int v = stMark - T;
    const int kd = max(kFirst, v >= 0 ? v / g.C : 0);
    const bool due = have && kd <= kLast;
    const unsigned long long notDue = ~__ballot(due);
    const int ng = notDue ? (int)__builtin_ctzll(notDue) : 64;
    if (lane < ng) {
        const int pS = pSFirst + (kd - kFirst) * g.C;
        bool q2 = false;
        int clIdx = closest_an_mark_idx(g, st, stMark, T, kd, pS, q2);
        if (q2) atomicAdd(&d.ub[0], 1ULL);
        int clAnMark;
        if (clIdx >= 0)
            clAnMark = st->anMarks[clIdx];
        else {
            int j = st->nPrevAn - clIdx;
            atomicAdd(&d.ub[1], 1ULL);
            clAnMark = (j >= 0 && j < VP_MARKS) ? st->prevAnMarks[j] : 0;
        }
        const double dSt = (double)stMark;
        const double beta = st->beta;
        const double x0 = dSt + (double)(0 - T) / beta;
        const double xN = dSt + (double)(nG - 1 - T) / beta;
        G.x0[lane] = x0; G.xN[lane] = xN;
        G.stMark[lane] = stMark;
        G.srcBase[lane] = g.toKeep + clAnMark - T;
        G.flags[lane] = (smi == 0 ? 1 : 0) | (smi == nSt - 1 ? 2 : 0);
        G.startIdx[lane] = max(max((int)floor(x0), 0), kd * g.C);
        G.stopIdx[lane] = min((int)ceil(xN), g.F);
        G.eLim[lane] = min(g.eLen, g.toKeep + g.F + kd * g.C);
    }
    int lo = 0, hi = 0;
    if (lane < ng) { lo = G.startIdx[lane]; hi = G.stopIdx[lane]; }
    lo = __builtin_amdgcn_readfirstlane(lo);
#pragma unroll
    for (int off = 32; off > 0; off >>= 1) hi = max(hi, __shfl_xor(hi, off, WAVE));
    if (park) { lo = kFirst * g.C; hi = max(hi, (kLast + 1) * g.C); }
    if (lane == 0) {
        stIdx->stMarkIdx = smi0 + ng;
        ctl->gNg[sg] = ng; ctl->gLo[sg] = lo; ctl->gHi[sg] = hi;
        ctl->gNT[sg] = ((ng > 0 || park) && hi > lo) ? (hi - lo + WAVE - 1) / WAVE : 0;
    }
}
__device__ __forceinline__ void ws_psola_gather_seg(const VpGeom &g, const VpDev &d, const PitchLds &L, const SegTab &G, lds_ctl *ctl, int sg, int jA, int jB,
                                                    int kFirst, bool first, const lds_f64 *hpPark = nullptr, int nChunk0 = 0)
{
    const lds_state *st = L.st;
    const int lane = vp_tid() & 63;
    const int nT = ctl->gNT[sg], lo = ctl->gLo[sg], hi = ctl->gHi[sg], ng = ctl->gNg[sg];
    const lds_f64 *hw = L.htab;
    bool have = false;
    int T = 0, nG = 1;
    double beta = 1.0, mx0 = 0.0, mxN = 0.0;
    int mst = 0, msrc = 0, mfl = 0, ma = 0, mb = 0, mlim = 0;
    auto below = [&](int x) -> int { return (x <= lo) ? 0 : min((x - lo + WAVE - 1) / WAVE, nT); };
    auto count = [&](int r) -> int {
        const int a = (r == 0) ? 0 : below((kFirst + r) * g.C), b = (r == jB - jA) ? nT : below((kFirst + r + 1) * g.C);
        return b - a;
    };
    auto release = [&](int j) {
        ws_wait_ge(&ctl->psDone, j, d);
        for (;;) {
            if (lane == 0) ctl->instMode[j] = hpPark ? 3 : 2;
            ws_signal(&ctl->psDone, j + 1);
            j++;
            if (j > jB || count(j - jA) != 0) break;
        }
    };
    if (first) {
        if (count(0) == 0) release(jA);
    }
    for (;;) {
        int m = 0;
        if (lane == 0) m = __hip_atomic_fetch_add((lds_i32 *)&ctl->gNext[sg], 1, __ATOMIC_RELAXED, __HIP_MEMORY_SCOPE_WORKGROUP);
        m = __builtin_amdgcn_readfirstlane(m);
        if (m >= nT) break;
        const unsigned long long tTrip0 = WS_CLK();
        (void)tTrip0;
        if (!have) {
            have = true;
            T = (st->pitch > 1) ? st->period : st->prevVoicedPeriod;
            nG = 2 * T + 1;
            beta = st->beta;
            const int ql = max(min(lane, ng - 1), 0);
            mx0 = G.x0[ql]; mxN = G.xN[ql];
            mst = G.stMark[ql]; msrc = G.srcBase[ql]; mfl = G.flags[ql]; ma = G.startIdx[ql]; mb = G.stopIdx[ql]; mlim = G.eLim[ql];
        }
        const int b = lo + WAVE * m;
        const int i = b + lane;
        const bool in = i < hi;
        const double di = (double)i;
        double accv = in ? L.oE[i] : 0.0;
        unsigned long long mask = __ballot(lane < ng && ma < b + WAVE && mb > b);
        struct Entry { int sa, sb, stM, srcBase, fl, eLim; double x0, xN; };
        auto entry = [&](int q) -> Entry {
            Entry e;
            e.sa = __builtin_amdgcn_readlane(ma, q); e.sb = __builtin_amdgcn_readlane(mb, q);
            e.x0 = __hiloint2double(__builtin_amdgcn_readlane(__double2hiint(mx0), q), __builtin_amdgcn_readlane(__double2loint(mx0), q));
            e.xN = __hiloint2double(__builtin_amdgcn_readlane(__double2hiint(mxN), q), __builtin_amdgcn_readlane(__double2loint(mxN), q));
            e.stM = __builtin_amdgcn_readlane(mst, q); e.srcBase = __builtin_amdgcn_readlane(msrc, q); e.fl = __builtin_amdgcn_readlane(mfl, q);
            e.eLim = __builtin_amdgcn_readlane(mlim, q);
            return e;
        };
        auto slow = [&](const Entry &e, bool &act) -> double {
            act = in && i >= e.sa && i < e.sb && di >= e.x0 && di <= e.xN;
            if (!act) return 0.0;
            const double dSt = (double)e.stM;
            int j = (int)ceil((di - dSt) * beta) + T;
            j = max(0, min(j, nG - 1));
            const double q0 = L.qtab[j], qm = L.qtab[max(j - 1, 0)], qp = L.qtab[min(j + 1, nG - 1)];
            double xj = dSt + q0, xjm = 0.0;
            if (j < nG - 1 && xj < di) {
                xjm = xj; j++; xj = dSt + qp;
                while (j < nG - 1 && xj < di) { xjm = xj; j++; xj = dSt + L.qtab[j]; }
// ... 28 lines not shown
            const double xj0 = dSt + q0, xm0 = dSt + qm, xp0 = dSt + qp;
            const bool up = j0 < nG - 1 && xj0 < di;
            const bool upMore = up && (j0 + 1 < nG - 1) && xp0 < di;
            const bool down = !up && j0 > 0 && xm0 >= di;
            ok = !act || !(upMore || down);
            const int j = up ? j0 + 1 : j0;
            const double xj = up ? xp0 : xj0, xjm = up ? xj0 : xm0;
            const int ja = max(j - 1, 0);
            const int srcA = e.srcBase + ja, srcB = e.srcBase + j;
            const double ea = L.eF[max(0, min(srcA, e.eLim - 1))], eb = L.eF[max(0, min(srcB, e.eLim - 1))];
            const double ha = hw[ja], hb = hw[j];
            const double eva = (srcA >= 0 && srcA < e.eLim) ? ea : 0.0, evb = (srcB >= 0 && srcB < e.eLim) ? eb : 0.0;
            const bool wa = (e.fl & 1) ? (ja >= T) : ((e.fl & 2) ? (ja < T) : true), wb = (e.fl & 1) ? (j >= T) : ((e.fl & 2) ? (j < T) : true);
            const double ya = wa ? eva * ha : eva, yb = wb ? evb * hb : evb;
            const double itp = ya + (yb - ya) / (xj - xjm) * (di - xjm);
            return (j > 0) ? itp : yb;
        };
        while (mask) {
            const int q1 = (int)__builtin_ctzll(mask);
            mask &= mask - 1;
            const bool two = mask != 0;
            const int q2 = two ? (int)__builtin_ctzll(mask) : q1;
            mask &= mask - 1;
            const Entry e1 = entry(q1), e2 = entry(q2);
            bool a1, a2, ok1, ok2;
            double v1 = fast(e1, a1, ok1), v2 = fast(e2, a2, ok2);
            WS_STAT(d, 2, 1);
#ifdef WS_GATHER_TEST
            if (WS_GATHER_TEST == 1) ok1 = false;
            if (WS_GATHER_TEST == 2 && ((b >> 6) & 1) && lane == 5) ok2 = false;
#endif
            if (__ballot(!(ok1 && ok2))) { v1 = slow(e1, a1); v2 = slow(e2, a2); WS_STAT(d, 3, 1); }
            if (a1) accv += v1;
            if (two && a2) accv += v2;
        }
        if (in) L.oE[i] = accv;
        if (hpPark && b < (kFirst + jB - jA + 1) * g.C) {
            iir_block_park((const lds_f64 *)L.oE, L.yF, b, hpPark);
#ifdef VP_STAMPS
            { const struct { int nChunk0; } c = {nChunk0}; if (m == 0) WS_EV(d, 13, 7); }
#endif
        }
        WS_STAT(d, 0, 1); WS_STAT(d, 1, WS_CLK() - tTrip0);
        int r = 0;
        for (int q = 1; q <= jB - jA; q++) r += (b >= (kFirst + q) * g.C) ? 1 : 0;
        __threadfence_block();
        int was = 0;
        if (lane == 0) was = __hip_atomic_fetch_add((lds_i32 *)&ctl->gDone[jA + r], 1, __ATOMIC_ACQ_REL, __HIP_MEMORY_SCOPE_WORKGROUP);
        was = __builtin_amdgcn_readfirstlane(was);
        if (was + 1 == count(r)) release(jA + r);
    }
}

template <bool FAST, bool BIG>
__device__ __forceinline__ void ws_background(const VpGeom &g0, const VpCall &c, const VpDev &d, const VpWsSched &sc, lds_f64 *sm, const WsCarve &cv0,
                                              lds_ctl *ctl, int bw, int gateOpen)
{
    lds_state *stBG = (lds_state *)(sm + cv0.st) + 1;
    const bool lead = bw == WS_NBG - 1;
    int bgBarGen = 0;
    PitchLds L;
    L.qtab = nullptr; L.htab = nullptr;
    L.st = stBG;
    L.ishare = (int *)ctl->ishareBG;
    L.fftFlag = (int *)ctl->fftFlag;
    L.xcA = nullptr;
    L.oA = nullptr; L.pend = nullptr;
    L.gateOpen = gateOpen;
    const int wq = (int)(blockDim.x / WAVE) - WS_NBG + bw;
    (void)wq;
    const int nStart = sc.nStart;
    for (int i = 0; i < nStart; i++) {
        const int gen = i + 1;
        VpGeom g = g0;
        WsCarve cv = cv0;
        asm volatile("" : "+s"(g.tauMax), "+s"(g.F), "+s"(g.C), "+s"(g.toKeep), "+s"(g.orderPitch), "+s"(g.tau0));
        asm volatile("" : "+s"(cv.xs), "+s"(cv.fr), "+s"(cv.P), "+s"(cv.dY), "+s"(cv.r), "+s"(cv.aPrev), "+s"(cv.hp), "+s"(cv.xp), "+s"(cv.aF), "+s"(cv.tw));
        L.eF = sm + cv.P;
        L.cum = sm + cv.P;
        L.dY = sm + cv.dY;
        L.fftTw = (lds_d2 *)(sm + cv.tw);
        if (lead) WS_FINE(d, 0);
        const int lane = vp_tid() & 63;
        if (!gateOpen) {
            if (lead) {
                ws_wait_ge(&ctl->bgAdopt, i, d);
                if (lane == 0) { stBG->nAn = 0; stBG->prevPitch = 0; stBG->gateOpen = 0; ctl->pubMode = 0; }
                ws_signal(&ctl->bgPub, gen);
            }
            continue;
        }
        const int pn = sc.startPar[i], tS = sc.startStep[i];
        ws_wait_ge(&ctl->fillTurn, sc.startNeed[i], d);
        if (i == 0) WS_EV(d, wq, 0);
        L.xs = sm + cv.xs + ((g.toKeep - g.tauMax) & 1) + tS * g.C;
        L.r = sm + cv.r + pn * 64;
        L.aPrev = sm + cv.aPrev + pn * (VP_ORDER_MAX + 2);
        lds_f64 *frBase = sm + cv.fr;
        lds_f64 *oEn = pn ? frBase + 3 * g.F + 2048 : frBase, *yFn = pn ? frBase + 2 * g.F + 2048 : frBase + g.F;
        L.oE = oEn; L.yF = yFn;
        L.fftBuf = (lds_d2 *)(pn ? frBase + 2 * g.F : frBase);
        const int base = g.toKeep - g.tauMax;
        const lds_f64 *xw = L.xs + base, *xf = L.xs + g.toKeep;
        const int xcCert = c.yinCert;
        VP_PRIO_UP();
        if (xcCert) xcorr_fft_wave(g, d, L, xw, lead ? 0 : bw + 1, WS_NBG, gen);
        VP_PRIO_DOWN();
        if (i == 0) WS_EV(d, wq, 1);
        if (bw == 0) {
            if (xcCert) { ws_prefix_sums(xw, L.eF, g.F + g.tauMax); ws_signal(&ctl->pDone, gen); }
            if (i == 0) WS_EV(d, wq, 2);
        } else if (bw == 1) {
            if (BIG) {
                if (FAST) autocorr_rows_fast<true, false>(xf, g.F, g.orderPitch, L.r, 1, 2);
                else for (int lag0 = 8; lag0 <= g.orderPitch; lag0 += 16) autocorr_rows_exact8(xf, g.F, g.orderPitch, lag0, L.r);
            } else
            if (FAST) {
                const double t1 = autocorr_rows_fast_half<true>(xf, g.F, 1);
                if (lane < 16) L.r[32 + lane] = t1;
            } else
                autocorr_rows_exact8(xf, g.F, g.orderPitch, 0, L.r);
            ws_signal(&ctl->acDone, gen);
            if (i == 0) WS_EV(d, wq, 2);
        } else if (bw == 2) {
            VP_PRIO_UP();
            const int order = g.orderPitch;
            if (BIG) {
                if (FAST) autocorr_rows_fast<true, false>(xf, g.F, order, L.r, 0, 2);
                else for (int lag0 = 0; lag0 <= order; lag0 += 16) autocorr_rows_exact8(xf, g.F, order, lag0, L.r);
                ws_wait_ge(&ctl->acDone, gen, d);
            } else
            if (FAST) {
                const double t0 = autocorr_rows_fast_half<true>(xf, g.F, 0);
                ws_wait_ge(&ctl->acDone, gen, d);
                const double t1 = L.r[32 + (lane & 15)];
                if (lane < 16 && lane <= order) L.r[lane] = (t0 + t1) / vp_f64_here(g.F);
            } else {
                if (order >= 8) autocorr_rows_exact8(xf, g.F, order, 8, L.r);
                ws_wait_ge(&ctl->acDone, gen, d);
            }
            if (i == 0) WS_EV(d, wq, 2);
            const bool z = !BIG ? levinson_row16(L.r, L.aPrev, order, VP_ORDER_MAX + 1, g.levEps)
                           : FAST ? levinson_fast64(L.r, L.aPrev, order, VP_ORDER_MAX + 1, g.levEps)
                                  : levinson_row48(L.r, L.aPrev, order, VP_ORDER_MAX + 1, g.levEps);
            if (i == 0) WS_EV(d, wq, 3);
            lds_f64 *hpad = sm + cv.hp + pn * WS_HP(g), *xp = sm + cv.xp, *aFn = sm + cv.aF + pn * WS_AF(g);
            hpad[lane] = 0.0;
            xp[lane] = (lane == 0) ? 1.0 : 0.0;
            const int nh = (BIG && order > 16) ? 2 * WAVE : WAVE;
            if (BIG) xp[WAVE + lane] = 0.0;
            iir_fast_wave(xp, hpad + WAVE, nh, (const lds_f64 *)L.aPrev, order, (const lds_f64 *)nullptr, 1.0);
            if (lane < WS_AF(g)) aFn[lane] = (lane <= order) ? L.aPrev[lane] : 0.0;
            if (lane == 0) ctl->lpcZ[pn] = z ? 1 : 0;
            ws_signal(&ctl->lpcDone, gen);
            if (i == 0) WS_EV(d, wq, 4);
            VP_PRIO_DOWN();
        }
        if (lead) {
            VP_PRIO_UP();
            int fallback = 1;
            ws_wait_ge(&ctl->bgAdopt, i, d);
            if (lane == 0) {
                stBG->gateOpen = 1;
                stBG->prevPeriod = stBG->period;
                stBG->prevPitch = stBG->pitch;
                if (stBG->pitch > 1) { stBG->prevVoicedPeriod = stBG->period; stBG->prevVoicedPitch = stBG->pitch; }
                stBG->pitch = 0; stBG->period = 0;
                ctl->ishareBG[0] = INT_MAX;
                ctl->ishareBG[1] = 0;
            }
            wave_sync();
            WS_FINE(d, 1);
            if (xcCert) {
                ws_wait_ge(&ctl->pDone, gen, d);
                if (i == 0) WS_EV(d, wq, 2);
                xc_scan_pick(g, L, stBG, xcCert, true);
                wave_sync();
                fallback = ctl->ishareBG[1] != 0;
                if (lane == 0) atomicAdd(&d.dbg[fallback ? 63 : 62], 1ULL);
                ws_signal(&ctl->xcDone, gen);
                if (!fallback) {
                    if (lane == 0) ctl->pickT[pn] = (stBG->pitch > 1) ? stBG->period : stBG->prevVoicedPeriod;
                    ws_signal(&ctl->tDone, gen);
                }
            }
            if (lane == 0) ctl->pickState = fallback;
            ws_signal(&ctl->pickDone, gen);
            if (i == 0) WS_EV(d, wq, 3);
            VP_PRIO_DOWN();
        }
        ws_wait_ge(&ctl->pickDone, gen, d);
        if (ctl->pickState) {
            if (lead && lane == 0) { ctl->ishareBG[0] = INT_MAX; ctl->ishareBG[1] = 0; }
            yin2_exact_waves(g, L, base, bw * WAVE + (vp_tid() & 63), 0, WS_NBG, (g.tauMax + 1) >> 1);
            ws_group_barrier(&ctl->bgBar, WS_NBG, bgBarGen, d);
            if (lead) {
                yin_cumsum_wave(g, L, vp_tid() & 63);
                wave_sync();
                ws_yin_pick_wave(g, d, L, stBG);
                wave_sync();
                if ((vp_tid() & 63) == 0) ctl->pickT[pn] = (stBG->pitch > 1) ? stBG->period : stBG->prevVoicedPeriod;
                ws_signal(&ctl->tDone, gen);
            }
            ws_group_barrier(&ctl->bgBar, WS_NBG, bgBarGen, d);
        }
        if (!lead) {
            if (xcCert) ws_wait_ge(&ctl->xcDone, gen, d);
            for (int q = bw * WAVE + lane; q < g.F; q += (WS_NBG - 1) * WAVE) { oEn[q] = 0.0; yFn[q] = 0.0; }
            __threadfence_block();
            if (lane == 0) __hip_atomic_fetch_add((lds_i32 *)&ctl->zeroDone, 1, __ATOMIC_RELEASE, __HIP_MEMORY_SCOPE_WORKGROUP);
            continue;
        }
        VP_PRIO_UP();
        {
            const int key = stBG->sp.key;
            const NoteRegs nr = notes_request(d.notes + (size_t)key * VP_NOTES_STRIDE);
            const int notesN = d.notesN[key];
            WS_FINE(d, 2);
            pitch_marks(g, L, d.ub);
            WS_FINE(d, 3);
            place_st_marks(g, c, d, stBG, nr, notesN);
        }
        wave_sync();
        if (i == 0) WS_EV(d, wq, 4);
        ws_wait_ge(&ctl->lpcDone, gen, d);
        if (stBG->nAn != 0) {
            const int ncopy = ctl->lpcZ[pn] ? VP_ORDER_MAX + 1 : g.orderPitch + 1;
            for (int q = lane; q < ncopy; q += WAVE) stBG->a[q] = L.aPrev[q];
        }
        WS_FINE(d, 4);
        ws_wait_ge(&ctl->zeroDone, (WS_NBG - 1) * gen, d);
        WS_FINE(d, 5);
        if (lane == 0) ctl->pubMode = stBG->nAn != 0 ? 2 : 1;
        ws_signal(&ctl->bgPub, gen);
        WS_EV(d, wq, i == 0 ? 5 : 6);
        VP_PRIO_DOWN();
    }
}

template <bool FAST>
__device__ __forceinline__ void ws_producer(const VpGeom &g, const VpCall &c, const VpDev &d, const VpWsSched &sc, lds_f64 *sm, const WsCarve &cv,
                                            lds_ctl *ctl, int rank, int nP, int gateOpen, bool firstBlock = true, bool lastBlock = true)
{
    const int lane = vp_tid() & 63, tp = rank * WAVE + lane, ntp = nP * WAVE;
    lds_state *st = (lds_state *)(sm + cv.st), *stPub = st + 1;
    lds_f64 *xsAll = sm + cv.xs + ((g.toKeep - g.tauMax) & 1);
    lds_f64 *frBase = sm + cv.fr;
    int barGen = 0;
    bool qValid = false;
    PitchLds L;
    L.st = st;
    L.eF = sm + cv.eF;
    L.qtab = sm + cv.qtab;
    L.htab = sm + cv.htab;
    const SegTab G = ws_seg_tab(sm + cv.gtab);
    const int order = g.orderPitch;
    const int wq = rank + 2;
    (void)wq;
    WS_EV(d, wq, 0);
    WS_TB();
    const int s_ = vp_stream(d);
    if (firstBlock && c.nChunk0 != 0 && st->nAn != 0) {
        const double *ge = d.eFrame + (size_t)s_ * g.eLen;
        const int lim = min(g.eLen, g.toKeep + g.F + (c.nChunk0 - 1) * g.C);
        for (int q = tp; q < lim; q += ntp) L.eF[q] = ge[q];
    }
    for (int sg = 0; sg < sc.nSeg; sg++) {
        const int jA = sc.segA[sg], jB = sc.segB[sg];
        const int t = sc.instStep[jA], kFirst = sc.instK[jA], kLast = sc.instK[jB], p = sc.instPar[jA], si = sc.instStart[jA];
        const int pS = c.pStart + t * g.C;
        const bool park = FAST && order <= 16 && sc.segPark[sg] != 0;
        const lds_f64 *hpPark = park ? (const lds_f64 *)(sm + cv.hp + p * WS_HP(g)) : (const lds_f64 *)nullptr;
        WS_TR();
        L.xs = xsAll + t * g.C;
        L.oE = p ? frBase + 3 * g.F + 2048 : frBase;
        L.yF = p ? frBase + 2 * g.F + 2048 : frBase + g.F;
        int mode;
        if (si >= 0) {
            const int jEnd = g.toKeep + g.F + (jB - jA) * g.C;
            if (gateOpen && rank != 0) {
                ws_wait_ge(&ctl->lpcDone, si + 1, d);
                WS_TA(d, wq, 1);
                const lds_f64 *aN = sm + cv.aF + p * WS_AF(g);
                for (int q = 4 * (tp - WAVE); q < jEnd; q += 4 * (ntp - WAVE)) fir4((const lds_f64 *)L.xs, aN, order, q, jEnd, L.eF);
                for (int q = jEnd + tp - WAVE; q < g.eLen; q += ntp - WAVE) L.eF[q] = 0.0;
                WS_TA(d, wq, 2);
                ws_wait_ge(&ctl->tDone, si + 1, d);
                WS_TA(d, wq, 1);
                const int T = ctl->pickT[p];
                const double *hg = d.hannTab + d.hannOff[T];
                for (int q = tp - WAVE; q < 2 * T + 1; q += ntp - WAVE) L.htab[q] = hg[q];
                WS_TA(d, wq, 2);
            }
            ws_wait_ge(&ctl->bgPub, si + 1, d);
            WS_TA(d, wq, 1);
            WS_FINEP(d, 0);
            mode = ctl->pubMode;
            if (rank == 0) {
                if (mode == 2) {
                    if (lane == 0) st->stMarkIdx = 0;
                    wave_sync();
                    ws_psola_table_seg(g, d, stPub, st, G, kFirst, kLast, pS, ctl, sg, park);
                }
                WS_TA(d, wq, 4);
                WS_FINEP(d, 2);
            } else {
                if (rank == 1) {
                    const int keep = (int)(offsetof(VpPitchState, stMarkIdx) / sizeof(int));
                    const lds_i32 *src = (const lds_i32 *)stPub;
                    lds_i32 *dst = (lds_i32 *)st;
                    for (int q = lane; q < (int)(sizeof(VpPitchState) / sizeof(int)); q += WAVE) if (q != keep) dst[q] = src[q];
                    WS_FINEP(d, 1);
                }
                if (mode == 2) {
                    const int T = (stPub->pitch > 1) ? stPub->period : stPub->prevVoicedPeriod;
                    const double beta = stPub->beta;
                    for (int q = tp - WAVE; q < 2 * T + 1; q += ntp - WAVE) L.qtab[q] = (double)(q - T) / beta;
                }
                WS_TA(d, wq, 2);
                WS_FINEP(d, 2);
            }
            if (mode == 1) for (int q = tp; q < jEnd; q += ntp) L.eF[q] = 0.0;
            qValid = mode == 2;
            ws_group_barrier(&ctl->prodBar, nP, barGen, d);
            WS_TA(d, wq, 3);
            WS_FINEP(d, 3);
            if (rank == 0) ws_signal(&ctl->bgAdopt, si + 1);
        } else {
            mode = (st->nAn != 0) ? 2 : 0;
            if (mode == 2) {
                if (rank == 0) {
                    ws_psola_table_seg(g, d, st, st, G, kFirst, kLast, pS, ctl, sg, park);
                    WS_TA(d, wq, 4);
                } else {
                    const int j0 = g.toKeep + g.F - g.C, jEnd = j0 + (jB - jA + 1) * g.C;
                    for (int q = j0 + 4 * (tp - WAVE); q < jEnd; q += 4 * (ntp - WAVE)) fir4((const lds_f64 *)L.xs, (const lds_f64 *)st->a, order, q, jEnd, L.eF + kFirst * g.C);
                    for (int q = kFirst * g.C + jEnd + tp - WAVE; q < g.eLen; q += ntp - WAVE) L.eF[q] = 0.0;
                    if (!qValid) {
                        const int T = (st->pitch > 1) ? st->period : st->prevVoicedPeriod;
                        const double beta = st->beta;
                        const double *hg = d.hannTab + d.hannOff[T];
                        for (int q = tp - WAVE; q < 2 * T + 1; q += ntp - WAVE) { L.qtab[q] = (double)(q - T) / beta; L.htab[q] = hg[q]; }
                    }
                    WS_TA(d, wq, 2);
                }
                qValid = true;
                ws_group_barrier(&ctl->prodBar, nP, barGen, d);
                WS_TA(d, wq, 3);
            }
        }
        if (mode == 2) {
            ws_psola_gather_seg(g, d, L, G, ctl, sg, jA, jB, kFirst, rank == 0, hpPark, c.nChunk0);
            WS_FINEP(d, 4);
            WS_TA(d, wq, 5);
            ws_wait_ge(&ctl->psDone, jB + 1, d);
            WS_FINEP(d, 6);
            WS_TA(d, wq, 3);
        } else {
            ws_group_barrier(&ctl->prodBar, nP, barGen, d);
            WS_TA(d, wq, 3);
            if (rank == 0) {
                if (lane <= jB - jA) ctl->instMode[jA + lane] = (lane == 0) ? mode : 0;
                ws_signal(&ctl->psDone, jB + 1);
            }
        }
    }
    {
        int nChunkEnd = c.nChunk0;
        for (int t = 0; t < c.nSteps; t++) { if (nChunkEnd == g.cpf - 1) nChunkEnd = 0; nChunkEnd += 1; }
        if (lastBlock && nChunkEnd != 0 && st->nAn != 0) {
            double *ge = d.eFrame + (size_t)s_ * g.eLen;
            for (int q = tp; q < g.eLen; q += ntp) ge[q] = L.eF[q];
        }
    }
    WS_EV(d, wq, 7);
}

template <bool FAST, bool BIG>
__device__ __forceinline__ void ws_recursion(const VpGeom &g, const VpCall &c, const VpDev &d, const VpWsSched &sc, lds_f64 *sm, const WsCarve &cv,
                                             lds_ctl *ctl, int me, int nIir, double gainPitch)
{
    const int nInst = sc.nInst;
    const int lane = vp_tid() & 63;
    lds_f64 *frBase = sm + cv.fr, *oA = sm + cv.oA;
    const int order = g.orderPitch;
    const int nW = g.C / WAVE;
    VP_PRIO_UP();
    WS_EV(d, me, 0);
    WS_TB();
    auto fill = [&](int j, const double (&win)[8]) {
        const int p = sc.instPar[j], pS = c.pStart + sc.instStep[j] * g.C, shift = sc.instK[j] * g.C;
        const lds_f64 *yF = p ? frBase + 2 * g.F + 2048 : frBase + g.F;
        if (ctl->instMode[j] >= 1) {
#pragma unroll
            for (int u = 0; u < 8; u++) if (u < nW) {
                const int i = lane + WAVE * u;
                oA[pS + i] += yF[shift + i] * win[u] * gainPitch;
            }
        }
        ws_signal(&ctl->fillTurn, j + 1);
    };
    auto window = [&](int j, double (&win)[8]) {
        const int shift = sc.instK[j] * g.C;
#pragma unroll
        for (int u = 0; u < 8; u++) win[u] = (u < nW) ? d.pitchStWin[shift + lane + WAVE * u] : 0.0;
    };
    int fj = 0;
    auto flush = [&](int upto, bool block) {
        for (; fj < upto; fj++) {
            if (sc.instPar[fj] != me) continue;
            if (!block && __hip_atomic_load(&ctl->fillTurn, __ATOMIC_ACQUIRE, __HIP_MEMORY_SCOPE_WORKGROUP) < fj) break;
            ws_wait_ge(&ctl->fillTurn, fj, d);
            double win[8];
            window(fj, win);
            fill(fj, win);
        }
    };
    int jPark = nInst;
    if (FAST && order <= 16) for (int sg = sc.nSeg - 1; sg >= 0 && sc.segPark[sg] != 0; sg--) jPark = sc.segA[sg];
    for (int j = 0; j < jPark; j++) {
        const int p = sc.instPar[j];
        if (nIir > 1 && p != me) continue;
        WS_TR();
        const int k = sc.instK[j], shift = k * g.C;
        lds_f64 *oE = p ? frBase + 3 * g.F + 2048 : frBase, *yF = p ? frBase + 2 * g.F + 2048 : frBase + g.F;
        const lds_f64 *aF = sm + cv.aF + p * WS_AF(g), *hpad = sm + cv.hp + p * WS_HP(g);
        if (!FAST && nIir > 1) {
            int spin = 0;
            while (__hip_atomic_load(&ctl->psDone, __ATOMIC_ACQUIRE, __HIP_MEMORY_SCOPE_WORKGROUP) < j + 1) {
                flush(j, false);
                if (++spin >= d.spinLimit) { if (lane == 0) vp_timeout(vp_tmo(d, 61)); break; }
                __builtin_amdgcn_s_sleep(1);
            }
        } else
        ws_wait_ge(&ctl->psDone, j + 1, d);
        WS_TA(d, me, 1);
        if (me == 0) WS_FINER(d, j);
        const int mode = ctl->instMode[j];
        if (mode == 2) {
            if (FAST)
            {
                if (BIG && order > 16) iir_block_wave_hc<32>((const lds_f64 *)(oE + shift), yF + shift, g.C, aF, order, min(order, shift), hpad, 1.0);
                else iir_block_wave_regs((const lds_f64 *)(oE + shift), yF + shift, g.C, aF, order, shift > 0, hpad);
            } else {
                lds_f64 *hist = sm + cv.hist + me * WS_HIST(g);
                const int nh = min(order, shift);
                for (int q = 0; q < order; q++) hist[q] = (q < nh) ? yF[shift - 1 - q] : 0.0;
                if (BIG && order > 16) iir_exact_lane<24>((const lds_f64 *)(oE + shift), yF + shift, g.C, aF, order, (const lds_f64 *)hist, 1.0);
                else iir_exact_row16((const lds_f64 *)(oE + shift), yF + shift, g.C, aF, order, (const lds_f64 *)hist, 1.0);
            }
        }
        WS_TA(d, me, 2);
        if (FAST)
            ws_signal(&ctl->iirDone, j + 1);
        else
            flush(j + 1, false);
        WS_TA(d, me, 4);
    }
    if constexpr (FAST) {
        IirWalkRegs R;
        bool haveR = false;
        for (int j = jPark; j < nInst; j++) {
            const int p = sc.instPar[j];
            WS_TR();
            const int k = sc.instK[j], shift = k * g.C;
            lds_f64 *oE = p ? frBase + 3 * g.F + 2048 : frBase, *yF = p ? frBase + 2 * g.F + 2048 : frBase + g.F;
            const lds_f64 *aF = sm + cv.aF + p * WS_AF(g), *hpad = sm + cv.hp + p * WS_HP(g);
            if (sc.instStart[j] >= 0) haveR = false;
            else if (!haveR) { iir_block_walk_load(R, aF, order, hpad); haveR = true; }
            ws_wait_ge(&ctl->psDone, j + 1, d);
            WS_TA(d, me, 1);
            WS_FINER(d, j);
            if (ctl->instMode[j] == 3) {
                if (!haveR) { iir_block_walk_load(R, aF, order, hpad); haveR = true; }
                if (j == jPark) WS_EV(d, 14, 7);
                iir_block_walk(R, (const lds_f64 *)(oE + shift), yF + shift, g.C, order, shift > 0);
            }
            WS_TA(d, me, 2);
            ws_signal(&ctl->iirDone, j + 1);
            WS_TA(d, me, 4);
        }
    }
    if (!FAST) { WS_TR(); flush(nInst, true); WS_TA(d, me, 3); }
    WS_EV(d, me, me == 0 ? 6 : 7);
    VP_PRIO_DOWN();
}

__device__ __forceinline__ void ws_filler(const VpGeom &g, const VpCall &c, const VpDev &d, const VpWsSched &sc, lds_f64 *sm, const WsCarve &cv,
                                          lds_ctl *ctl, double gainPitch)
{
    const int lane = vp_tid() & 63;
    lds_f64 *frBase = sm + cv.fr, *oA = sm + cv.oA;
    const int nW = g.C / WAVE;
    VP_PRIO_UP();
    for (int j = 0; j < sc.nInst; j++) {
        const int p = sc.instPar[j], pS = c.pStart + sc.instStep[j] * g.C, shift = sc.instK[j] * g.C;
        const lds_f64 *yF = p ? frBase + 2 * g.F + 2048 : frBase + g.F;
        double win[8];
#pragma unroll
        for (int u = 0; u < 8; u++) win[u] = (u < nW) ? d.pitchStWin[shift + lane + WAVE * u] : 0.0;
        ws_wait_ge(&ctl->iirDone, j + 1, d);
        if (ctl->instMode[j] >= 1) {
#pragma unroll
            for (int u = 0; u < 8; u++) if (u < nW) {
                const int i = lane + WAVE * u;
                oA[pS + i] += yF[shift + i] * win[u] * gainPitch;
            }
        }
        ws_signal(&ctl->fillTurn, j + 1);
    }
    VP_PRIO_DOWN();
}

__device__ __forceinline__ void ws_emit_block(const VpGeom &g, const VpCall &c, const VpDev &d, float *__restrict__ out, const lds_state *stl,
                                              const lds_f64 *oA)
{
    const int s = vp_stream(d);
    const float *vr = d.voiceRing + (size_t)s * g.inSize;
    const float *sr0 = d.synthRing + (size_t)s * 2 * g.inSize;
    const float *sr1 = sr0 + g.inSize;
    double *acc = d.outAcc + (size_t)s * g.outSize;
    double *acc2 = d.outAcc2 ? d.outAcc2 + (size_t)s * g.outSize : nullptr;
    float *o = out + (size_t)s * (c.inplace ? 3 : 2) * g.N;
    const int dryOn = stl->sp.dryOn, synthOn = stl->sp.synthOn;
    const double gainVoice = stl->sp.gainVoice, gainSynth = stl->sp.gainSynth;
    for (int i = vp_tid(); i < g.N; i += blockDim.x) {
        int pos = c.outCounter + i, pin = c.currCounter + i;
        pos -= (pos >= g.outSize) ? g.outSize : 0;
        pin -= (pin >= g.inSize) ? g.inSize : 0;
        double v = oA[i];
        if (acc2) { v += acc2[pos]; acc2[pos] = 0.0; }
        if (dryOn) v += (double)vr[pin] * gainVoice;
        double l = v, r = v;
        if (synthOn) { l += (double)sr0[pin] * gainSynth; r += (double)sr1[pin] * gainSynth; }
        o[i] = (float)l;
        o[g.N + i] = (float)r;
        if (c.inplace) o[2 * g.N + i] = 0.0f;
        acc[pos] = 0.0;
    }
}

__device__ __forceinline__ void ws_mb_launder(VpGeom &g, VpCall &c, VpDev &d)
{
    asm volatile("" : "+s"(g.S), "+s"(g.N), "+s"(g.F), "+s"(g.H), "+s"(g.C), "+s"(g.cpf), "+s"(g.toKeep), "+s"(g.latency), "+s"(g.inSize), "+s"(g.outSize), "+s"(g.tauMax), "+s"(g.eLen), "+s"(g.orderPitch), "+s"(g.tau0));
    asm volatile("" : "+s"(c.inCounter), "+s"(c.outCounter), "+s"(c.currCounter), "+s"(c.pStart), "+s"(c.nChunk0), "+s"(c.nSteps), "+s"(c.inMono), "+s"(c.yinCert));
    asm volatile("" : "+s"(d.voiceRing), "+s"(d.synthRing), "+s"(d.outAcc), "+s"(d.pitch), "+s"(d.eFrame), "+s"(d.outEFrame), "+s"(d.yFrame), "+s"(d.hImp));
    asm volatile("" : "+s"(d.pitchStWin), "+s"(d.hannTab), "+s"(d.hannOff), "+s"(d.notes), "+s"(d.notesN), "+s"(d.fftTw1), "+s"(d.fftTw2), "+s"(d.fftTws), "+s"(d.dbg), "+s"(d.ub), "+s"(d.gate));
}
__device__ __forceinline__ void ws_lds_barrier() { asm volatile("s_waitcnt lgkmcnt(0)\n\ts_barrier" ::: "memory"); }
__device__ __forceinline__ void ws_mb_launder_carve(WsCarve &cv)
{
    asm volatile("" : "+s"(cv.xs), "+s"(cv.eF), "+s"(cv.fr), "+s"(cv.qtab), "+s"(cv.htab), "+s"(cv.P), "+s"(cv.dY), "+s"(cv.gtab), "+s"(cv.r), "+s"(cv.aPrev));
    asm volatile("" : "+s"(cv.hp), "+s"(cv.aF), "+s"(cv.xp), "+s"(cv.hist), "+s"(cv.tw), "+s"(cv.oA), "+s"(cv.st), "+s"(cv.ctl));
}
// ... 79 lines not shown
        const lds_i32 *src = (const lds_i32 *)st;
        lds_i32 *dst = (lds_i32 *)stBG;
        for (int i = tid; i < (int)(sizeof(VpPitchState) / sizeof(int)); i += nt) dst[i] = src[i];
    }
    if (pl == 1 && nChunkEnd != 0 && st->nAn != 0) {
        const lds_f64 *oE1 = oE0 + 3 * g.F + 2048, *yF1 = oE0 + 2 * g.F + 2048;
        for (int i = done + tid; i < g.F; i += nt) oE0[i] = oE1[i];
        for (int i = max(0, done - g.orderPitch) + tid; i < done; i += nt) yF0[i] = yF1[i];
        if (tid < WS_HP(g)) (sm + cv.hp)[tid] = (sm + cv.hp + WS_HP(g))[tid];
        if (tid < WS_AF(g)) (sm + cv.aF)[tid] = (sm + cv.aF + WS_AF(g))[tid];
    }
    {
        const double part = wave_sum(sn - so);
        if ((tid & 63) == 0) gateRed[tid >> 6] = part;
    }
    ws_lds_barrier();
    {
        double T = gateT;
#pragma unroll
        for (int w = 0; w < 16; w++) T += gateRed[w];
        const double Tm = fmax(gateRed[16], T);
        const double band = Tm * vp_f64_here(2 * g.inSize + 64 + 2 * (blk + 1) * (2 * N + 64)) * 1.1102230246251565e-16 * 1.5;
        gateT = T;
        if (tid == 0) gateRed[16] = Tm;
        if (T - g.gateThrSum > band) gateOpen = 1;
        else if (g.gateThrSum - T > band) gateOpen = 0;
        else {
            __threadfence_block();
            __syncthreads();
            if (tid == 0) {
                const float *vr = d.voiceRing + (size_t)s * g.inSize;
                double seq = 0.0;
                for (int i = 0; i < g.inSize; i++) { double a = (double)vr[i]; seq += a * a; }
                ctl->ishareP[0] = !(seq < g.gateThrSum);
                gateRed[15] = seq;
            }
            __syncthreads();
            gateOpen = ctl->ishareP[0];
            gateT = gateRed[15];
            __syncthreads();
            if (tid == 0) { ctl->ishareP[0] = 0; gateRed[15] = 0.0; gateRed[16] = gateT; }
        }
        if (tid == 0) d.gate[s * 2 + 0] = gateOpen;
    }
    asm volatile("" :: "v"(touch));
    c.inCounter = inCn; c.outCounter = outCn; c.currCounter = curCn; c.nChunk0 = mbp->nChunk0[blk + 1];
    scp = &mbp->sc[mbp->schedOf[blk + 1]];
    inb = inn;
    outb += (size_t)g.S * 2 * N;
    ws_mb_launder(g, c, d);
    ws_mb_launder_carve(cv);
}

#include "vp_pitch_ws_body.inc"
#define WS_MB 1
#include "vp_pitch_ws_body.inc"
#undef WS_MB

#if VP_TU_HAS(6)
__global__ __launch_bounds__(768) void vp_k_pitch_ws(VpGeom g, VpCall c, VpDev d, VpWsSched sc, const float *__restrict__ in, float *__restrict__ out)
{
    extern __shared__ double smem[];
    pitch_ws_body<true, false>(g, c, d, sc, in, out, smem);
}
__global__ __launch_bounds__(768) void vp_k_pitch_ws_x(VpGeom g, VpCall c, VpDev d, VpWsSched sc, const float *__restrict__ in, float *__restrict__ out)
{
    extern __shared__ double smem[];
    pitch_ws_body<false, false>(g, c, d, sc, in, out, smem);
}
#endif
#if VP_TU_HAS(6)
__global__ __launch_bounds__(768) void vp_k_pitch_ws_mb(VpGeom g, VpCall c, VpDev d, VpWsMb mb, const float *__restrict__ in, float *__restrict__ out)
{
    extern __shared__ double smem[];
    pitch_ws_body_mb<true, false>(g, c, d, &mb, in, out, smem);
}
#endif
#if VP_TU_HAS(7)
__global__ __launch_bounds__(768) void vp_k_pitch_ws_o24(VpGeom g, VpCall c, VpDev d, VpWsSched sc, const float *__restrict__ in, float *__restrict__ out)
{
    extern __shared__ double smem[];
    pitch_ws_body<true, true>(g, c, d, sc, in, out, smem);
}
__global__ __launch_bounds__(768) void vp_k_pitch_ws_x_o24(VpGeom g, VpCall c, VpDev d, VpWsSched sc, const float *__restrict__ in, float *__restrict__ out)
{
    extern __shared__ double smem[];
    pitch_ws_body<false, true>(g, c, d, sc, in, out, smem);
}
#endif
#if VP_TU_HAS(8)
__global__ __launch_bounds__(768) void vp_k_pitch_ws_x_mb(VpGeom g, VpCall c, VpDev d, VpWsMb mb, const float *__restrict__ in, float *__restrict__ out)
{
    extern __shared__ double smem[];
    pitch_ws_body_mb<false, false>(g, c, d, &mb, in, out, smem);
}
#endif
#if VP_TU_HAS(9)
__global__ __launch_bounds__(768) void vp_k_pitch_ws_mb_o24(VpGeom g, VpCall c, VpDev d, VpWsMb mb, const float *__restrict__ in, float *__restrict__ out)
{
    extern __shared__ double smem[];
    pitch_ws_body_mb<true, true>(g, c, d, &mb, in, out, smem);
}
__global__ __launch_bounds__(768) void vp_k_pitch_ws_x_mb_o24(VpGeom g, VpCall c, VpDev d, VpWsMb mb, const float *__restrict__ in, float *__restrict__ out)
{
    extern __shared__ double smem[];
    pitch_ws_body_mb<false, true>(g, c, d, &mb, in, out, smem);
}
#endif
```

### vocoderproject_amd/csrc/vp_pitch_ws_body.inc

```
#ifdef WS_MB
template <bool FAST, bool BIG>
__device__ __forceinline__ void pitch_ws_body_mb(const VpGeom &g_, const VpCall &c_, const VpDev &d_, const VpWsMb *mbp, const float *__restrict__ in,
                                                 float *__restrict__ out, double *smem)
{
    VpGeom g = g_;
    VpCall c = c_;
    VpDev d = d_;
    const VpWsSched *scp = &mbp->sc[mbp->schedOf[0]];
    c.inCounter = mbp->inCtr[0]; c.outCounter = mbp->outCtr[0]; c.currCounter = mbp->currCtr[0]; c.nChunk0 = mbp->nChunk0[0];
    ws_mb_launder(g, c, d);
#define sc (*scp)
#else
template <bool FAST, bool BIG>
__device__ __forceinline__ void pitch_ws_body(const VpGeom &g, const VpCall &c, const VpDev &d, const VpWsSched &sc, const float *__restrict__ in,
                                              float *__restrict__ out, double *smem)
{
#endif
    const int s = vp_stream(d), nt = blockDim.x, tid = vp_tid();
    const int nSteps = c.nSteps;
    VP_POISON(smem, c.ldsBytes);
    STAMP0(d);
#ifdef VP_STAMPS
    if (blockIdx.x == 0 && threadIdx.x == 0) atomicAdd(&WS_SLOT(d, 15, 7), (unsigned long long)wall_clock64());
#endif
    {
        const int *ws_ = (const int *)&sc;
        int acc_ = 0;
#pragma unroll
        for (int q = 0; q < (int)(sizeof(VpWsSched) / sizeof(int)); q += 16) acc_ += ws_[q];
        asm volatile("" :: "s"(acc_));
    }
    const bool fusedPro = c.fuseIngest && !c.vocOn;
    if (c.fuseIngest && !fusedPro) ingest_gate_block(g, c, d, in);
    lds_f64 *sm = (lds_f64 *)smem;
#ifdef WS_MB
    WsCarve cv = ws_carve(g, nSteps);
#else
    const WsCarve cv = ws_carve(g, nSteps);
#endif
    lds_ctl *ctl = (lds_ctl *)(sm + cv.ctl);
    lds_state *st = (lds_state *)(sm + cv.st), *stBG = st + 1;
    lds_f64 *xsAll = sm + cv.xs + ((g.toKeep - g.tauMax) & 1);
    lds_f64 *oE0 = sm + cv.fr, *yF0 = oE0 + g.F, *oA = sm + cv.oA;
    const float *vr = d.voiceRing + (size_t)s * g.inSize;
    const int pS0 = c.pStart;
    const int span = g.toKeep + g.F + (nSteps - 1) * g.C;

#ifdef WS_MB
    __shared__ double gateRed[17];
#else
    __shared__ double gateRed[16];
#endif
    constexpr int TR = 8;
    const int mono = c.inMono;
    const float *xin = in + (size_t)s * (mono ? 1 : 3) * g.N;
    float gv[TR], xv[TR], wv0[4], wv1[4], wv2[4];
    double av[4], ov[2], yv = 0.0, hv = 0.0, a0v = 0.0;
    int sv_[2];
    d2 tv[2];
    const int idx0 = pS0 - g.toKeep;
    const int p0 = ring_pos(c.currCounter, idx0, g.inSize);
    const int done0 = c.nChunk0 * g.C;
    typedef float f4v __attribute__((ext_vector_type(4)));
    typedef double d2v __attribute__((ext_vector_type(2)));
    const bool vec = ((g.N | g.inSize | c.inCounter | p0 | (idx0 - g.latency) | span) & 3) == 0 && ((c.outCounter | g.outSize | (g.N + g.C)) & 1) == 0 &&
                     g.inSize <= 4 * nt && span <= 4 * nt && g.N + g.C <= 2 * nt && (((size_t)xin | (size_t)vr) & 15) == 0;
    f4v gq = {0.f, 0.f, 0.f, 0.f}, xq = {0.f, 0.f, 0.f, 0.f}, w0q = {0.f, 0.f, 0.f, 0.f}, w1q = {0.f, 0.f, 0.f, 0.f}, w2q = {0.f, 0.f, 0.f, 0.f};
    d2v aq = {0.0, 0.0};
    if (vec) {
        if (fusedPro) {
            const int p = 4 * tid;
            if (p < g.inSize) {
                int k = p - c.inCounter;
                k += (k < 0) ? g.inSize : 0;
                gq = (k < g.N) ? *(const f4v *)(xin + k) : *(const f4v *)(vr + p);
            }
            if (p < g.N) {
                w0q = *(const f4v *)(xin + p);
                if (mono == 0) { w1q = *(const f4v *)(xin + g.N + p); w2q = *(const f4v *)(xin + 2 * g.N + p); }
            }
        }
        const int j = 4 * tid;
        if (j < span) {
            int pp = p0 + j;
            pp -= (pp >= g.inSize) ? g.inSize : 0;
            const int k = idx0 + j - g.latency;
            xq = (fusedPro && k >= 0 && k < g.N) ? *(const f4v *)(xin + k) : *(const f4v *)(vr + pp);
        }
        const int q = 2 * tid;
        if (q < g.N + g.C) {
            int pos = c.outCounter + q;
            pos -= (pos >= g.outSize) ? g.outSize : 0;
            aq = *(const d2v *)(d.outAcc + (size_t)s * g.outSize + pos);
        }
    } else {
    if (fusedPro) {
#pragma unroll
        for (int u = 0; u < TR; u++) {
            const int p = tid + u * nt;
            int k = p - c.inCounter;
            k += (k < 0) ? g.inSize : 0;
            gv[u] = (p < g.inSize) ? ((k < g.N) ? xin[k] : vr[p]) : 0.0f;
        }
#pragma unroll
        for (int u = 0; u < 4; u++) {
            const int i = tid + u * nt;
            wv0[u] = (i < g.N) ? xin[i] : 0.0f;
            wv1[u] = (i < g.N && mono == 0) ? xin[g.N + i] : 0.0f;
            wv2[u] = (i < g.N && mono == 0) ? xin[2 * g.N + i] : 0.0f;
        }
    }
#pragma unroll
    for (int u = 0; u < TR; u++) {
        const int j = tid + u * nt;
        int pp = p0 + j;
        pp -= (pp >= g.inSize) ? g.inSize : 0;
        const int k = idx0 + j - g.latency;
        xv[u] = (j < span) ? ((fusedPro && k >= 0 && k < g.N) ? xin[k] : vr[pp]) : 0.0f;
    }
// ... 78 lines not shown
                    float *sr0 = d.synthRing + (size_t)s * 2 * g.inSize;
                    sr0[p] = wv1[u];
                    sr0[g.inSize + p] = wv2[u];
                }
            }
        }
        for (int i = tid + 4 * nt; i < g.N; i += nt) {
            const int p = (c.inCounter + i) % g.inSize;
            vrw[p] = xin[i];
            if (mono != 2) {
                float *sr0 = d.synthRing + (size_t)s * 2 * g.inSize;
                sr0[p] = mono ? 0.0f : xin[g.N + i];
                sr0[g.inSize + p] = mono ? 0.0f : xin[2 * g.N + i];
            }
        }
    }
#pragma unroll
    for (int u = 0; u < TR; u++) { const int j = tid + u * nt; if (j < span) xsAll[j] = (double)xv[u]; }
    for (int j = tid + TR * nt; j < span; j += nt) {
        int pp = p0 + j;
        pp -= (pp >= g.inSize) ? g.inSize : 0;
        const int k = idx0 + j - g.latency;
        xsAll[j] = (double)((fusedPro && k >= 0 && k < g.N) ? xin[k] : vr[pp]);
    }
    {
        const double *acc = d.outAcc + (size_t)s * g.outSize;
#pragma unroll
        for (int u = 0; u < 4; u++) { const int q = tid + u * nt; if (q < g.N + g.C) oA[q] = av[u]; }
        for (int q = tid + 4 * nt; q < g.N + g.C; q += nt) oA[q] = acc[(c.outCounter + q) % g.outSize];
    }
    }
    {
        lds_i32 *dst = (lds_i32 *)st, *dst2 = (lds_i32 *)stBG;
#pragma unroll
        for (int u = 0; u < 2; u++) { const int i = tid + u * nt; if (i < (int)(sizeof(VpPitchState) / sizeof(int))) { dst[i] = sv_[u]; dst2[i] = sv_[u]; } }
    }
    if (c.nChunk0 != 0) {
        const double *go = d.outEFrame + (size_t)s * g.F;
#pragma unroll
        for (int u = 0; u < 2; u++) { const int i = done0 + tid + u * nt; if (i < g.F) oE0[i] = ov[u]; }
        for (int i = done0 + tid + 2 * nt; i < g.F; i += nt) oE0[i] = go[i];
        { const int i = max(0, done0 - g.orderPitch) + tid; if (i < done0) yF0[i] = yv; }
        lds_f64 *hp0 = sm + cv.hp;
        if (tid < WAVE) hp0[tid] = 0.0;
        if (tid < (BIG ? 2 * WAVE : WAVE)) hp0[WAVE + tid] = hv;
        if (tid < WS_AF(g)) (sm + cv.aF)[tid] = a0v;
    }
    {
        lds_d2 *tw = (lds_d2 *)(sm + cv.tw);
#pragma unroll
        for (int u = 0; u < 2; u++) { const int i = tid + u * nt; if (i < VP_FFT_TW_D2) tw[i] = tv[u]; }
    }
    for (int i = tid; i < (int)(sizeof(WsCtl) / sizeof(int)); i += nt) ((lds_i32 *)ctl)[i] = 0;
    if (tid >= nt / WAVE && tid < 16) gateRed[tid] = 0.0;
    WS_EV0(d, 1, 1);
    __syncthreads();
    WS_EV0(d, 1, 2);
    int gateOpen;
#ifdef WS_MB
    double gateT = 0.0;
#endif
    if (fusedPro) {
        double T = 0.0;
#pragma unroll
        for (int w = 0; w < 16; w++) T += gateRed[w];
#ifdef WS_MB
        gateT = T;
        if (tid == 0) gateRed[16] = T;
#endif
        const double band = T * vp_f64_here(2 * g.inSize + 64) * 1.1102230246251565e-16 * 1.5;
        if (T - g.gateThrSum > band) gateOpen = 1;
        else if (g.gateThrSum - T > band) gateOpen = 0;
        else {
            if (tid == 0) {
                double seq = 0.0;
                for (int i = 0; i < g.inSize; i++) { double a = (double)vr[i]; seq += a * a; }
                ctl->ishareP[0] = !(seq < g.gateThrSum);
            }
            __syncthreads();
            gateOpen = ctl->ishareP[0];
            __syncthreads();
        }
        if (tid == 0) d.gate[s * 2 + 0] = gateOpen;
    } else
        gateOpen = d.gate[s * 2 + 0];
    STAMP(d, 15);
    const double gainPitch = st->sp.gainPitch;
#ifndef WS_MB
    const int nInst = sc.nInst;
#endif
    const int wv = tid >> 6;
#ifdef WS_MB
    {
        double *acc = d.outAcc + (size_t)s * g.outSize;
        for (int q = tid; q < g.N + g.C; q += nt) {
            int pos = c.outCounter + q;
            pos -= (pos >= g.outSize) ? g.outSize : 0;
            acc[pos] = 0.0;
        }
    }
    const float *inb = in;
    float *outb = out;
    const int nB = mbp->nBlocks;
    for (int blk = 0; ; blk++) {
#endif

    const int NW = nt / WAVE, nRec = FAST ? 1 : 2, nFG = FAST ? 2 : 2, nP = NW - WS_NBG - nFG;
    if (wv >= NW - WS_NBG)
    {
        const int x = wv - (NW - WS_NBG);
        ws_background<FAST, BIG>(g, c, d, sc, sm, cv, ctl, FAST ? (0x1230 >> (4 * x)) & 15 : x, gateOpen);
    }
    else if (wv < nRec)
        ws_recursion<FAST, BIG>(g, c, d, sc, sm, cv, ctl, wv, nRec, gainPitch);
    else if (FAST && wv == 1)
        ws_filler(g, c, d, sc, sm, cv, ctl, gainPitch);
    else
#ifdef WS_MB
        ws_producer<FAST>(g, c, d, sc, sm, cv, ctl, wv - nFG, nP, gateOpen, blk == 0, blk == nB - 1);
    if (blk != nB - 1) ws_lds_barrier(); else
    __syncthreads();
    if (blk == nB - 1) break;
    ws_mb_boundary(g, c, d, mbp, blk, scp, sm, cv, ctl, st, stBG, xsAll, oE0, yF0, oA, gateRed, inb, outb, span, gateT, gateOpen);
    }
#define out outb
#else
        ws_producer<FAST>(g, c, d, sc, sm, cv, ctl, wv - nFG, nP, gateOpen);
    __syncthreads();
#endif
    STAMP(d, 8);

#ifdef WS_MB
    const int nInst = sc.nInst;
#endif
    {
        const int tid = vp_tid();
        {
            int *dst = (int *)(d.pitch + s);
            const lds_i32 *src = (const lds_i32 *)st;
            for (int i = tid; i < (int)(sizeof(VpPitchState) / sizeof(int)); i += nt) dst[i] = src[i];
        }
        const int pl = sc.instPar[nInst - 1];
        int nChunkEnd = c.nChunk0;
        for (int t = 0; t < nSteps; t++) { if (nChunkEnd == g.cpf - 1) nChunkEnd = 0; nChunkEnd += 1; }
        if (nChunkEnd != 0 && st->nAn != 0) {
            double *go = d.outEFrame + (size_t)s * g.F, *gy = d.yFrame + (size_t)s * g.F;
            const lds_f64 *oEl = pl ? oE0 + 3 * g.F + 2048 : oE0, *yFl = pl ? oE0 + 2 * g.F + 2048 : yF0;
            const int done = nChunkEnd * g.C;
            for (int i = done + tid; i < g.F; i += nt) go[i] = oEl[i];
            for (int i = max(0, done - g.orderPitch) + tid; i < done; i += nt) gy[i] = yFl[i];
            if (tid < (BIG ? 2 * WAVE : WAVE)) d.hImp[(size_t)s * 2 * WAVE + tid] = (sm + cv.hp + pl * WS_HP(g))[WAVE + tid];
        }
        STAMP(d, 11);
        double *acc = d.outAcc + (size_t)s * g.outSize;
        for (int q = (c.fuseEmit ? g.N : 0) + tid; q < g.N + g.C; q += nt) {
            int pos = c.outCounter + q;
            pos -= (pos >= g.outSize) ? g.outSize : 0;
            acc[pos] = oA[q];
        }
        if (c.fuseEmit) ws_emit_block(g, c, d, out, st, (const lds_f64 *)oA);
    }
#ifdef VP_STAMPS
    if (blockIdx.x == 0 && threadIdx.x == 0) { atomicAdd(&WS_SLOT(d, 0, 7), 1ULL); atomicAdd(&WS_SLOT(d, 0, 5), (unsigned long long)wall_clock64()); }
#endif
#ifdef WS_MB
#undef out
#undef sc
#endif
}
```

### vocoderproject_amd/processor.py

```python
import ctypes as C
import os

import numpy as np

_HERE = os.path.dirname(os.path.abspath(__file__))
LIB_PATH = os.environ.get("VP_AMD_LIB") or os.path.join(_HERE, "libvp_amd.so")

PARAM_IDS = ("gainPitch", "gainVoice", "gainSynth", "gainVoc", "lpcVoice", "lpcPitch",
             "lpcSynth", "keyPitch", "pitchBool", "vocBool")
KEYS = ("A", "A#", "B", "C", "C#", "D", "D#", "E", "F", "F#", "G", "G#", "Chrom")
GEOM_KEYS = ("N", "F", "H", "C", "W", "h", "toKeep", "latency", "inSize", "outSize", "tauMax", "chunksPerFrame")
KERNEL_SLOTS = 4
MARK_CAP = 64


class VpParams(C.Structure):
    _fields_ = [("gainPitch", C.c_float), ("gainVoice", C.c_float), ("gainSynth", C.c_float), ("gainVoc", C.c_float),
                ("lpcVoice", C.c_int), ("lpcPitch", C.c_int), ("lpcSynth", C.c_int), ("keyPitch", C.c_int),
                ("pitchBool", C.c_int), ("vocBool", C.c_int)]


class VpPitchState(C.Structure):
    _fields_ = [("period", C.c_int), ("prevPeriod", C.c_int), ("prevVoicedPeriod", C.c_int), ("periodNew", C.c_int),
                ("nAn", C.c_int), ("nSt", C.c_int), ("stMarkIdx", C.c_int), ("gateOpen", C.c_int),
# ... 31 lines not shown
    L.vp_prepare_explicit.argtypes = [vp, C.c_double, C.c_int, C.c_int, C.c_int, C.c_int, C.c_int, C.c_int]
    L.vp_process_block.argtypes = [vp, fp, fp]
    L.vp_process_block_inplace.argtypes = [vp, fp]
    L.vp_process_block_device.argtypes = [vp, fp, fp, C.c_void_p]
    L.vp_get_latency.argtypes = [vp]
    L.vp_get_geometry.argtypes = [vp, C.POINTER(C.c_int)]
    L.vp_get_num_streams.argtypes = [vp]
    L.vp_read_pitch_state.argtypes = [vp, C.c_int, C.POINTER(VpPitchState)]
    L.vp_synchronize.argtypes = [vp]
    L.vp_profile_enable.argtypes = [vp, C.c_int]
    L.vp_profile_read.argtypes = [vp, C.POINTER(C.c_double), C.POINTER(C.c_long), C.c_int]
    L.vp_kernel_slot_name.argtypes = [C.c_int]
    L.vp_kernel_slot_name.restype = C.c_char_p
    if hasattr(L, "vp_process_blocks_device"):
        L.vp_process_blocks_device.argtypes = [C.c_void_p, C.c_void_p, C.c_void_p, C.c_int, C.c_void_p]
    if hasattr(L, "vp_set_stream_params"):
        L.vp_set_stream_params.argtypes = [C.c_void_p, C.c_int, C.c_void_p]
        L.vp_get_stream_params.argtypes = [C.c_void_p, C.c_int, C.c_void_p]
    if hasattr(L, "vp_process_block_mono"):
        L.vp_process_block_mono.argtypes = [C.c_void_p, C.c_void_p, C.c_void_p]
        L.vp_process_block_mono_device.argtypes = [C.c_void_p, C.c_void_p, C.c_void_p, C.c_void_p]
        L.vp_process_blocks_mono_device.argtypes = [C.c_void_p, C.c_void_p, C.c_void_p, C.c_int, C.c_void_p]
    if hasattr(L, "vp_process_block_channels"):
        L.vp_process_block_channels.argtypes = [C.c_void_p, C.c_void_p, C.c_int, C.c_void_p, C.c_int]
        L.vp_process_block_channels_device.argtypes = [C.c_void_p, C.c_void_p, C.c_int, C.c_void_p, C.c_int, C.c_void_p]
        L.vp_process_blocks_channels_device.argtypes = [C.c_void_p, C.c_void_p, C.c_int, C.c_void_p, C.c_int, C.c_int, C.c_void_p]
    if hasattr(L, "vp_process_blocks"):
        L.vp_process_blocks.argtypes = [C.c_void_p, C.c_void_p, C.c_void_p, C.c_int]
    if hasattr(L, "vp_set_pitch_shift"):
        L.vp_set_pitch_shift.argtypes = [C.c_void_p, C.c_int, C.c_int, C.c_double]
        L.vp_get_pitch_shift.argtypes = [C.c_void_p, C.c_int, C.POINTER(C.c_int), C.POINTER(C.c_double)]
    L.vp_pitch_kernel_name.argtypes = [C.c_void_p]
    L.vp_pitch_kernel_name.restype = C.c_char_p
    if hasattr(L, "vp_vocoder_kernel_name"):
        L.vp_vocoder_kernel_name.argtypes = [C.c_void_p]
        L.vp_vocoder_kernel_name.restype = C.c_char_p
    if hasattr(L, "vp_set_vocoder_path"):
        L.vp_set_vocoder_path.argtypes = [C.c_void_p, C.c_int]
        L.vp_get_vocoder_path.argtypes = [C.c_void_p]
    if hasattr(L, "vp_set_overlap"):
        L.vp_set_overlap.argtypes = [C.c_void_p, C.c_int]
        L.vp_get_overlap.argtypes = [C.c_void_p]
    if hasattr(L, "vp_reserve_blocks"):
        L.vp_reserve_blocks.argtypes = [C.c_void_p, C.c_int]
        L.vp_get_reserved_blocks.argtypes = [C.c_void_p]
        L.vp_debug_alloc_count.argtypes = [C.c_void_p]
        L.vp_debug_alloc_count.restype = C.c_long
    if hasattr(L, "vp_set_time_parallel"):
        L.vp_set_time_parallel.argtypes = [C.c_void_p, C.c_int]
        L.vp_get_time_parallel.argtypes = [C.c_void_p]
    if hasattr(L, "vp_set_wave_specialised"):
        L.vp_set_wave_specialised.argtypes = [C.c_void_p, C.c_int]
        L.vp_get_wave_specialised.argtypes = [C.c_void_p]
    if hasattr(L, "vp_debug_set_spin_limit"):
        L.vp_debug_set_spin_limit.argtypes = [C.c_void_p, C.c_int]
    L.vp_read_ub_counters.argtypes = [vp, C.POINTER(C.c_long)]
    L.vp_debug_read_stamps.argtypes = [vp, C.POINTER(C.c_ulonglong), C.c_int]
    L.vp_set_yin_mode.argtypes = [vp, C.c_int]
    L.vp_get_yin_mode.argtypes = [vp]
    L.vp_set_iir_mode.argtypes = [vp, C.c_int]
    L.vp_get_iir_mode.argtypes = [vp]
    L.vp_stft_create.argtypes = [C.c_int, C.c_int, C.c_int, C.c_int, C.c_int, C.POINTER(vp)]
    L.vp_stft_destroy.argtypes = [vp]
    L.vp_stft_num_frames.argtypes = [vp]
    L.vp_stft_roundtrip.argtypes = [vp, fp, fp, fp, C.c_void_p]
    L.vp_stft_pitch_shift.argtypes = [vp, fp, fp, C.c_double, C.c_void_p]
    L.vp_stft_is_fused.argtypes = [vp]
    if hasattr(L, "vp_stft_pitch_shift_curve"):
        L.vp_stft_pitch_shift_curve.argtypes = [vp, fp, fp, C.c_void_p, C.c_void_p]
        L.vp_semitones_to_ratios.argtypes = [C.c_void_p, C.c_void_p, C.c_long]
        L.vp_pv_process_blocks_curve_device.argtypes = [vp, fp, fp, C.c_void_p, C.c_int, C.c_void_p]
    if hasattr(L, "vp_stft_pitch_shift_locked"):
        L.vp_stft_pitch_shift_locked.argtypes = [vp, fp, fp, C.c_void_p, C.c_void_p]
        L.vp_pv_process_blocks_locked_device.argtypes = [vp, fp, fp, C.c_void_p, C.c_int, C.c_void_p]
    if hasattr(L, "vp_stft_pitch_shift_locked_subbin"):
        L.vp_stft_pitch_shift_locked_subbin.argtypes = [vp, fp, fp, C.c_void_p, C.c_void_p]
        L.vp_pv_process_blocks_locked_subbin_device.argtypes = [vp, fp, fp, C.c_void_p, C.c_int, C.c_void_p]
    if hasattr(L, "vp_stft_time_stretch"):
        L.vp_stft_time_stretch.argtypes = [vp, fp, C.c_int, C.c_void_p, fp, C.c_double, C.c_void_p]
        L.vp_stretch_positions.argtypes = [C.c_void_p, C.c_int, C.c_int, C.c_double, C.c_int, C.c_int]
    if hasattr(L, "vp_stft_time_stretch_locked"):
        L.vp_stft_time_stretch_locked.argtypes = [vp, fp, C.c_int, C.c_void_p, fp, C.c_void_p, C.c_void_p]
    if hasattr(L, "vp_stft_onset_flux"):
        L.vp_onset_num_frames.argtypes = [C.c_int, C.c_int, C.c_int]
        L.vp_stft_onset_flux.argtypes = [vp, fp, C.c_int, C.c_void_p, C.c_void_p, C.c_void_p]
        L.vp_onset_pick.argtypes = [C.c_void_p, C.c_void_p, C.c_int, C.c_double, C.c_void_p]
        L.vp_stretch_positions_transient.argtypes = [C.c_void_p, C.c_void_p, C.c_int, C.c_int, C.c_double, C.c_int, C.c_int, C.c_void_p, C.c_int]
        L.vp_stft_time_stretch_locked_reset.argtypes = [vp, fp, C.c_int, C.c_void_p, fp, C.c_void_p, C.c_void_p, C.c_void_p]
    if hasattr(L, "vp_stft_track_pitch"):
        L.vp_track_tau_max.argtypes = [C.c_double]
        L.vp_stft_track_pitch.argtypes = [vp, fp, C.c_double, C.c_void_p, C.c_void_p, C.c_void_p, C.c_void_p]
        L.vp_stft_autotune.argtypes = [vp, fp, fp, C.c_double, C.c_void_p, C.c_void_p, C.c_void_p, C.c_void_p]
        L.vp_stft_last_error.argtypes = [vp]
        L.vp_stft_last_error.restype = C.c_char_p
    L.vp_stft_set_runs.argtypes = [vp, C.c_int]
    L.vp_stft_set_precision.argtypes = [vp, C.c_int]
    L.vp_stft_get_precision.argtypes = [vp]
    if hasattr(L, "vp_pv_create"):
        L.vp_pv_create.argtypes = [C.c_int, C.c_int, C.c_int, C.c_int, C.c_int, C.POINTER(vp)]
        L.vp_pv_destroy.argtypes = [vp]
        L.vp_pv_get_latency.argtypes = [vp]
        L.vp_pv_set_semitones.argtypes = [vp, C.c_int, C.c_double]
        L.vp_pv_get_semitones.argtypes = [vp, C.c_int, C.POINTER(C.c_double)]
        L.vp_pv_reset.argtypes = [vp, C.c_int]
        L.vp_pv_process_block.argtypes = [vp, fp, fp]
        L.vp_pv_process_blocks_device.argtypes = [vp, fp, fp, C.c_int, C.c_void_p]
# ... 74 lines not shown
            pass

    def _chk(self, rc):
        if rc:
            raise VpError(rc, f"{self.L.vp_error_string(rc).decode()} ({self.L.vp_last_error(self.h).decode()})")

    def setParameter(self, pid, value):
        if pid not in PARAM_IDS:
            raise KeyError(pid)
        old = getattr(self._p, pid)
        setattr(self._p, pid, type(old)(value))
        rc = self.L.vp_set_params(self.h, C.byref(self._p))
        if rc:
            setattr(self._p, pid, old)
            self._chk(rc)

    def getParameter(self, pid):
        return getattr(self._p, pid)

    def setStreamParameter(self, stream, pid, value):
        if pid not in PARAM_IDS:
            raise KeyError(pid)
        q = VpParams()
        self._chk(self.L.vp_get_stream_params(self.h, int(stream), C.byref(q)))
        setattr(q, pid, type(getattr(q, pid))(value))
        self._chk(self.L.vp_set_stream_params(self.h, int(stream), C.byref(q)))

    def setPitchShift(self, semitones, on=True, stream=-1):
        self._chk(self.L.vp_set_pitch_shift(self.h, int(stream), int(bool(on)), float(semitones)))

    def getPitchShift(self, stream):
        on, semi = C.c_int(), C.c_double()
        self._chk(self.L.vp_get_pitch_shift(self.h, int(stream), C.byref(on), C.byref(semi)))
        return bool(on.value), semi.value

    def getStreamParameter(self, stream, pid):
        q = VpParams()
        self._chk(self.L.vp_get_stream_params(self.h, int(stream), C.byref(q)))
        return getattr(q, pid)

    def set_iir_mode(self, mode):
        self._chk(self.L.vp_set_iir_mode(self.h, {"exact": 0, "fast": 1}[mode] if isinstance(mode, str) else int(mode)))

    def set_vocoder_path(self, path):
        self._chk(self.L.vp_set_vocoder_path(self.h, {"auto": 0, "workgroup": 1, "batched": 2}[path] if isinstance(path, str) else int(path)))

    def set_overlap(self, on):
        self._chk(self.L.vp_set_overlap(self.h, 2 if on == "auto" else int(bool(on))))

    def set_time_parallel(self, on):
        self._chk(self.L.vp_set_time_parallel(self.h, int(bool(on))))

    def set_wave_specialised(self, on):
        self._chk(self.L.vp_set_wave_specialised(self.h, int(bool(on))))

    def set_yin_mode(self, mode):
        self._chk(self.L.vp_set_yin_mode(self.h, {"direct": 0, "fft": 1, "xcorr": 2, "xcorr_force_fallback": 3}[mode] if isinstance(mode, str) else int(mode)))

    def get_yin_mode(self):
        return {0: "direct", 1: "fft", 2: "xcorr", 3: "xcorr_force_fallback"}[self.L.vp_get_yin_mode(self.h)]

    def get_iir_mode(self):
        return "fast" if self.L.vp_get_iir_mode(self.h) == 1 else "exact"

    def prepareToPlay(self, sampleRate, samplesPerBlock, nStreams=1):
        self._chk(self.L.vp_prepare_to_play(self.h, float(sampleRate), int(samplesPerBlock), int(nStreams)))
        self.n_streams, self.N = int(nStreams), int(samplesPerBlock)

    def prepareExplicit(self, sampleRate, samplesPerBlock, nStreams, frameLenPitch, hopPitch, wlenVoc, hopVoc):
        self._chk(self.L.vp_prepare_explicit(self.h, float(sampleRate), int(samplesPerBlock), int(nStreams),
                                             int(frameLenPitch), int(hopPitch), int(wlenVoc), int(hopVoc)))
        self.n_streams, self.N = int(nStreams), int(samplesPerBlock)

    def getLatencySamples(self):
        rc = self.L.vp_get_latency(self.h)
        if rc < 0:
            self._chk(rc)
        return rc

    @property
    def latency(self):
        return self.getLatencySamples()

    def geometry(self):
        g = (C.c_int * 12)()
        self._chk(self.L.vp_get_geometry(self.h, g))
        return dict(zip(GEOM_KEYS, list(g)))

    def processBlock(self, buffer):
        assert isinstance(buffer, np.ndarray) and buffer.dtype == np.float32 and buffer.flags.c_contiguous
        assert buffer.shape == (self.n_streams, 3, self.N), buffer.shape
        self._chk(self.L.vp_process_block_inplace(self.h, buffer.ctypes.data))

    def process(self, x):
        assert x.dtype == np.float32 and x.flags.c_contiguous and x.shape == (self.n_streams, 3, self.N)
        out = np.empty((self.n_streams, 2, self.N), np.float32)
        self._chk(self.L.vp_process_block(self.h, x.ctypes.data, out.ctypes.data))
        return out

    def process_mono(self, voice):
        assert voice.dtype == np.float32 and voice.flags.c_contiguous and voice.shape == (self.n_streams, self.N)
        out = np.empty((self.n_streams, 2, self.N), np.float32)
        self._chk(self.L.vp_process_block_mono(self.h, voice.ctypes.data, out.ctypes.data))
        return out

    def process_mono_device(self, d_voice, d_out, stream=None):
        assert d_voice.is_cuda and d_out.is_cuda and d_voice.is_contiguous() and d_out.is_contiguous()
# ... 85 lines not shown
        else:
            self._chk(self.L.vp_process_blocks_channels_device(self.h, in_table.data_ptr(), int(n_in), out_table.data_ptr(), int(n_out), int(n_blocks),
                                                               C.c_void_p(stream)))

    def run(self, x):
        S, _, T = x.shape
        assert S == self.n_streams and T % self.N == 0
        out = np.empty((S, 2, T), np.float32)
        for b in range(T // self.N):
            blk = np.ascontiguousarray(x[:, :, b * self.N:(b + 1) * self.N])
            out[:, :, b * self.N:(b + 1) * self.N] = self.process(blk)
        return out

    def synchronize(self):
        self._chk(self.L.vp_synchronize(self.h))

    def pitch_state(self, stream):
        st = VpPitchState()
        self._chk(self.L.vp_read_pitch_state(self.h, int(stream), C.byref(st)))
        return dict(period=st.period, prevPeriod=st.prevPeriod, prevVoicedPeriod=st.prevVoicedPeriod,
                    periodNew=st.periodNew, pitch=st.pitch, prevPitch=st.prevPitch, beta=st.beta,
                    closestFreq=st.closestFreq, gateOpen=st.gateOpen, stMarkIdx=st.stMarkIdx,
                    anMarks=list(st.anMarks[:st.nAn]), stMarks=list(st.stMarks[:st.nSt]), a=np.array(st.a[:]))

    def ub_counters(self):
        c = (C.c_long * 5)()
        self._chk(self.L.vp_read_ub_counters(self.h, c))
        return list(c)

    def debug_stamps(self, reset=True):
        v = (C.c_ulonglong * 64)()
        self._chk(self.L.vp_debug_read_stamps(self.h, v, int(bool(reset))))
        return [t / 100.0 for t in v]

    def yin_certified_counts(self, reset=True):
        v = (C.c_ulonglong * 64)()
        self._chk(self.L.vp_debug_read_stamps(self.h, v, int(bool(reset))))
        assert int(v[61]) == 0, "the prefix-sum flag of VP_YIN_XCORR timed out (kernel bug)"
        return int(v[62]), int(v[63])

    def profile_enable(self, on=True):
        self._chk(self.L.vp_profile_enable(self.h, int(on)))

    def profile_read(self, reset=True):
        ms = (C.c_double * KERNEL_SLOTS)()
        n = (C.c_long * KERNEL_SLOTS)()
        self._chk(self.L.vp_profile_read(self.h, ms, n, int(bool(reset))))
        names = [self.L.vp_kernel_slot_name(i).decode() for i in range(KERNEL_SLOTS)]
        names[2] = self.pitch_kernel_name() or names[2]
        return {names[i]: (ms[i], n[i]) for i in range(KERNEL_SLOTS)}

    def pitch_kernel_name(self):
        return self.L.vp_pitch_kernel_name(self.h).decode()

    def debug_set_spin_limit(self, polls):
        self._chk(self.L.vp_debug_set_spin_limit(self.h, int(polls)))

    def vocoder_kernel_name(self):
        return self.L.vp_vocoder_kernel_name(self.h).decode()


def semitones_to_ratios(semitones):
    L = load_library()
    st = np.ascontiguousarray(semitones, dtype=np.float64)
    r = np.empty_like(st)
    rc = L.vp_semitones_to_ratios(st.ctypes.data, r.ctypes.data, st.size)
    if rc:
        raise VpError(rc, L.vp_error_string(rc).decode())
    return r


def stretch_positions(n_frames, hop, stretch, n_in, frame_len=1024):
    L = load_library()
    pos = np.empty(int(n_frames), dtype=np.int32)
    rc = L.vp_stretch_positions(pos.ctypes.data, int(n_frames), int(hop), float(stretch), int(n_in), int(frame_len))
    if rc:
        raise VpError(rc, L.vp_error_string(rc).decode())
    return pos


ONSET_THRESHOLD = 0.2
ONSET_SPAN_MIN, ONSET_SPAN_MAX = 1, 8


def default_onset_span(frame_len, hop):
    return max(int(frame_len) // (2 * int(hop)), 1)


def pick_onsets(flux, mass, thr=ONSET_THRESHOLD):
    L = load_library()
    fl, ms = np.ascontiguousarray(flux, dtype=np.float64), np.ascontiguousarray(mass, dtype=np.float64)
    if fl.ndim != 1 or fl.shape != ms.shape:
        raise ValueError(f"pick_onsets: flux and mass are one row each of one length, got {fl.shape} and {ms.shape}")
    on = np.zeros(fl.shape, dtype=np.uint8)
    rc = L.vp_onset_pick(fl.ctypes.data, ms.ctypes.data, fl.size, float(thr), on.ctypes.data)
    if rc:
        raise VpError(rc, L.vp_error_string(rc).decode())
    return on


def stretch_positions_transient(onsets, n_frames, hop, stretch, n_in, frame_len=1024, span=None):
    L = load_library()
    K = default_onset_span(frame_len, hop) if span is None else int(span)
    on = np.ascontiguousarray(onsets, dtype=np.uint8)
    nG = L.vp_onset_num_frames(int(n_in), int(frame_len), int(hop))
    if nG < 0:
# ... 794 lines not shown
```

Measured before the change: 25.37 million.

## Add geometry-specialised lean wave-specialised pitch kernel with constant geometry and deferred timeouts

Adds a new pitch kernel variant that hard-codes the common geometry (1024-pt frame, hop 256, order 15, tauMax 441) and call flags as compile-time constants, forces the vectorised ingest path, and defers spin-timeout reporting to a single LDS flag checked at kernel end. It is selected automatically when wave-specialised mode, fast IIR, and the exact geometry and alignment conditions hold. The aim is to cut scalar register pressure and branch overhead in the inner wave-specialised loops. It also adds a debug hook that reports the launched pitch kernel symbol, at the cost of another kernel instantiation and a narrower selection condition.

```diff
diff --git a/include/vp_amd.h b/include/vp_amd.h
--- a/include/vp_amd.h
+++ b/include/vp_amd.h
@@ -99,6 +99,7 @@
 int vp_get_time_parallel(const vp_handle *h);
 int vp_set_wave_specialised(vp_handle *h, int on);
 int vp_get_wave_specialised(const vp_handle *h);
+const char *vp_debug_pitch_symbol(const vp_handle *h);
 
 #define VP_YIN_DIRECT 0
 #define VP_YIN_FFT 1
diff --git a/vocoderproject_amd/build.py b/vocoderproject_amd/build.py
--- a/vocoderproject_amd/build.py
+++ b/vocoderproject_amd/build.py
@@ -11,7 +11,7 @@
 LIB = os.path.join(HERE, "libvp_amd.so")
 SOURCES = ["vp_kernels.hip", "vp_voc2.hip", "vp_stft.hip", "vp_channels.hip", "vp_track.hip", "vp_capi.hip"]
 ARCH = "gfx950"
-NUM_TUS = 9
+NUM_TUS = 10
 
 
 def deps_of(source):
@@ -93,14 +93,18 @@
             pass
 
 
+def compile_command():
+    return [hipcc(), "-std=c++17", "-O3", "-ffp-contract=off", "-fdenormal-fp-math=preserve-sign", "-fPIC", f"--offload-arch={ARCH}", "-Wall", "-Wno-unused-function",
+            "-I", os.path.join(ROOT, "include"), "-I", CSRC]
+
+
 def build(force=False, verbose=False, stamps=False, poison=False):
     lib = LIB_STAMPS if stamps else LIB_POISON if poison else (os.environ.get("VP_LIB_OUT") or LIB)
     if not stamps and not poison and not force and lib == LIB and not needs_build():
         return LIB
     import tempfile
     from concurrent.futures import ThreadPoolExecutor
-    common = [hipcc(), "-std=c++17", "-O3", "-ffp-contract=off", "-fdenormal-fp-math=preserve-sign", "-fPIC", f"--offload-arch={ARCH}", "-Wall", "-Wno-unused-function",
-              "-I", os.path.join(ROOT, "include"), "-I", CSRC]
+    common = compile_command()
     common += os.environ.get("VP_EXTRA_HIPCC_FLAGS", "").split()
     if stamps:
         common.append("-DVP_STAMPS")
diff --git a/vocoderproject_amd/csrc/vp_capi.hip b/vocoderproject_amd/csrc/vp_capi.hip
--- a/vocoderproject_amd/csrc/vp_capi.hip
+++ b/vocoderproject_amd/csrc/vp_capi.hip
@@ -46,6 +46,7 @@
     int overlap = VP_OVERLAP_AUTO, acc2Live = 0;
     int accLive = 0;
     int waveSpec = 1;
+    const char *pitchSymbol = "";
     int timeParallel = 0;
     std::vector<void *> allocs;
     float *stageIn = nullptr, *stageOut = nullptr;
@@ -169,6 +170,19 @@
     return vp_pitch_ws_lds_bytes(g, nSteps) + 256 <= h->ldsMax;
 }
 
+struct WsPlan { void (*fn)(VpGeom, VpCall, VpDev, VpWsSched, const float *, float *); const char *name; };
+struct WsMbPlan { void (*fn)(VpGeom, VpCall, VpDev, VpWsMb, const float *, float *); const char *name; };
+#define VP_WS_PLAN(K) WsPlan{K, #K}
+#define VP_WS_MB_PLAN(K) WsMbPlan{K, #K}
+static bool pitch_ws_lean_ok(const vp_handle *h, const VpCall &cp, const VpDev &d, int wsWaves, const float *d_in)
+{
+    const VpGeom &g = h->g;
+    if (h->waveSpec != 1 || !cp.iirFast || !pitch_common(h) || !vp_ws_lean_geom(g) || wsWaves != WS_LEAN_WAVES) return false;
+    if (!cp.fuseIngest || !cp.fuseEmit || cp.vocOn || !cp.pitchOn || cp.yinCert != 1 || d.outAcc2 || cp.nBlocks != 1) return false;
+    if (cp.pStart != 0 || g.N % g.C != 0 || cp.nSteps != g.N / g.C || cp.nSteps < 1 || cp.nSteps > 4) return false;
+    return vp_ws_vec_ok(g, cp, 64 * wsWaves, vp_ws_p0(g, cp), (size_t)d_in, (size_t)d.voiceRing);
+}
+
 static int pitch_xfft_waves(const vp_handle *h, bool fast, int nBlocks)
 {
     if (!pitch_common(h) || pitch_lite(h, fast) || (nBlocks > 1 && !fast)) return 0;
@@ -240,9 +254,10 @@
 extern "C" int vp_set_wave_specialised(vp_handle *h, int on)
 {
     if (!h) return VP_ERR_INVALID_ARG;
-    h->waveSpec = on ? 1 : 0;
-    return VP_OK;
-}
+    h->waveSpec = on == 2 ? 2 : on ? 1 : 0;
+    return VP_OK;
+}
+extern "C" const char *vp_debug_pitch_symbol(const vp_handle *h) { return h ? h->pitchSymbol : ""; }
 extern "C" int vp_get_wave_specialised(const vp_handle *h) { return h ? h->waveSpec : VP_ERR_INVALID_ARG; }
 
 extern "C" const char *vp_vocoder_kernel_name(const vp_handle *h)
@@ -606,7 +621,7 @@
                              (const void *)vp_k_pitch_fast_multi, (const void *)vp_k_pitch_lite, (const void *)vp_k_pitch_lite_fast,
                              (const void *)vp_k_pitch_c, (const void *)vp_k_pitch_fast_c, (const void *)vp_k_pitch_fast_multi_c,
                              (const void *)vp_k_pitch_lite_fast_c, (const void *)vp_k_pitch_lite_fast_multi, (const void *)vp_k_pitch_lite_fast_multi_c,
-                             (const void *)vp_k_pitch_ws, (const void *)vp_k_pitch_ws_x, (const void *)vp_k_pitch_ws_mb, (const void *)vp_k_pitch_ws_x_mb, (const void *)vp_k_pitch_ws_mb_o24, (const void *)vp_k_pitch_ws_x_mb_o24, (const void *)vp_k_pitch_ws_o24, (const void *)vp_k_pitch_ws_x_o24,
+                             (const void *)vp_k_pitch_ws, (const void *)vp_k_pitch_ws_x, (const void *)vp_k_pitch_ws_mb, (const void *)vp_k_pitch_ws_x_mb, (const void *)vp_k_pitch_ws_mb_o24, (const void *)vp_k_pitch_ws_x_mb_o24, (const void *)vp_k_pitch_ws_o24, (const void *)vp_k_pitch_ws_x_o24, (const void *)vp_k_pitch_ws_l,
                              (const void *)vp_k_vocoder, (const void *)vp_k_vocoder_o48, (const void *)vp_k_vocoder_lite};
         for (const void *f : fns) {
             hipFuncAttributes fa;
@@ -708,6 +723,7 @@
     h->currCounter = g.toKeep;
     h->cohorts.assign(1, vp_handle::Cohort{h->params.pitchBool, h->params.vocBool, 0, 0, 0, S, nullptr, {}});
     h->cohortsDirty = false; h->poisoned = false; h->poisonCode = VP_ERR_HIP;
+    h->pitchSymbol = "";
     h->sparams.assign((size_t)S, h->params);
     h->spHost.assign((size_t)S, VpStreamParams{});
     h->synthNonZero = 0;
@@ -882,6 +898,7 @@
                         f->cp.fftOff = (int)off; f->cp.fftWaves = fw; plan.lds = off + pitch_xfft_lds(h);
                     }
                     f->cp.ldsBytes = (int)plan.lds;
+                    h->pitchSymbol = plan.name;
                     hipLaunchKernelGGL(plan.fn, dim3(f->n), dim3(512), plan.lds, h->auxStream, f->g, f->cp, f->dp, f->in, f->out);
                 };
                 VpCall cv = c;
@@ -943,10 +960,16 @@
                     VpWsSched sc;
                     memset(&sc, 0, sizeof sc);
                     if (!ws_build_sched(g, cp.nChunk0, cp.nSteps, sc)) return fail_hip(h, hipErrorInvalidValue, "pitch schedule");
-                    const auto wsk = g.orderPitch > 15 ? (cp.iirFast ? vp_k_pitch_ws_o24 : vp_k_pitch_ws_x_o24) : (cp.iirFast ? vp_k_pitch_ws : vp_k_pitch_ws_x);
-                    hipLaunchKernelGGL(wsk, dim3(co.n), dim3(64 * wsWaves), (size_t)cp.ldsBytes, st, g, cp, d, sc, d_in, d_out);
-                } else
-                hipLaunchKernelGGL(plan.fn, dim3(co.n), dim3(512), plan.lds, st, g, cp, d, d_in, d_out);
+                    const bool lean = pitch_ws_lean_ok(h, cp, d, wsWaves, d_in);
+                    const WsPlan wsk = lean ? VP_WS_PLAN(vp_k_pitch_ws_l)
+                                            : g.orderPitch > 15 ? (cp.iirFast ? VP_WS_PLAN(vp_k_pitch_ws_o24) : VP_WS_PLAN(vp_k_pitch_ws_x_o24))
+                                                                : (cp.iirFast ? VP_WS_PLAN(vp_k_pitch_ws) : VP_WS_PLAN(vp_k_pitch_ws_x));
+                    h->pitchSymbol = wsk.name;
+                    hipLaunchKernelGGL(wsk.fn, dim3(co.n), dim3(64 * wsWaves), (size_t)cp.ldsBytes, st, g, cp, d, sc, d_in, d_out);
+                } else {
+                    h->pitchSymbol = plan.name;
+                    hipLaunchKernelGGL(plan.fn, dim3(co.n), dim3(512), plan.lds, st, g, cp, d, d_in, d_out);
+                }
             }
         }
         hipError_t e = hipGetLastError();
@@ -1166,6 +1189,7 @@
         }
         cp.ldsBytes = (int)plan.lds;
         ProfScope ps(h, st, 2);
+        h->pitchSymbol = plan.name;
         hipLaunchKernelGGL(plan.fn, dim3(co.n), dim3(512), plan.lds, st, gp, cp, dp, d_in, d_out);
     }
     {
@@ -1258,8 +1282,10 @@
     d.outAcc2 = nullptr;
     {
         ProfScope ps(h, st, 2);
-        const auto wsk = g.orderPitch > 15 ? (fast ? vp_k_pitch_ws_mb_o24 : vp_k_pitch_ws_x_mb_o24) : (fast ? vp_k_pitch_ws_mb : vp_k_pitch_ws_x_mb);
-        hipLaunchKernelGGL(wsk, dim3(co.n), dim3(64 * 12), (size_t)c.ldsBytes, st, g, c, d, mb, d_in, d_out);
+        const WsMbPlan wsk = g.orderPitch > 15 ? (fast ? VP_WS_MB_PLAN(vp_k_pitch_ws_mb_o24) : VP_WS_MB_PLAN(vp_k_pitch_ws_x_mb_o24))
+                                               : (fast ? VP_WS_MB_PLAN(vp_k_pitch_ws_mb) : VP_WS_MB_PLAN(vp_k_pitch_ws_x_mb));
+        h->pitchSymbol = wsk.name;
+        hipLaunchKernelGGL(wsk.fn, dim3(co.n), dim3(64 * 12), (size_t)c.ldsBytes, st, g, c, d, mb, d_in, d_out);
     }
     hipError_t e = hipGetLastError();
     if (e != hipSuccess) { h->poisoned = true; h->poisonCode = VP_ERR_HIP; return fail_hip(h, e, "kernel launch"); }
diff --git a/vocoderproject_amd/csrc/vp_common.h b/vocoderproject_amd/csrc/vp_common.h
--- a/vocoderproject_amd/csrc/vp_common.h
+++ b/vocoderproject_amd/csrc/vp_common.h
@@ -208,6 +208,25 @@
 }
 VP_HD static inline size_t vp_pitch_ws_lds_bytes(const VpGeom &g, int nSteps) { return (size_t)ws_carve(g, nSteps).end * sizeof(double); }
 
+VP_HD static inline int vp_ws_p0(const VpGeom &g, const VpCall &c) { return (c.currCounter + c.pStart - g.toKeep + g.inSize) % g.inSize; }
+VP_HD static inline bool vp_ws_vec_ok(const VpGeom &g, const VpCall &c, int nt, int p0, size_t xinAddr, size_t vrAddr)
+{
+    const int idx0 = c.pStart - g.toKeep, span = g.toKeep + g.F + (c.nSteps - 1) * g.C;
+    return ((g.N | g.inSize | c.inCounter | p0 | (idx0 - g.latency) | span) & 3) == 0 && ((c.outCounter | g.outSize | (g.N + g.C)) & 1) == 0 &&
+           g.inSize <= 4 * nt && span <= 4 * nt && g.N + g.C <= 2 * nt && ((xinAddr | vrAddr) & 15) == 0;
+}
+
+#define WS_LEAN_F 1024
+#define WS_LEAN_C 256
+#define WS_LEAN_ORDER 15
+#define WS_LEAN_TAUMAX 441
+#define WS_LEAN_WAVES 12
+VP_HD static inline bool vp_ws_lean_geom(const VpGeom &g)
+{
+    return g.F == WS_LEAN_F && g.C == WS_LEAN_C && g.cpf == 4 && g.H == WS_LEAN_F - WS_LEAN_C && g.toKeep == WS_LEAN_F && g.eLen == 2 * WS_LEAN_F + 3 * WS_LEAN_C &&
+           g.orderPitch == WS_LEAN_ORDER && g.tauMax == WS_LEAN_TAUMAX;
+}
+
 VP_HD static inline size_t voc_wave_doubles(int W)
 {
     return (size_t)4 * W + 2 * (VP_ORDER_MAX + 1) + 2 * (VP_ORDER_MAX_SYNTH + 1) + 2;
diff --git a/vocoderproject_amd/csrc/vp_kernels.h b/vocoderproject_amd/csrc/vp_kernels.h
--- a/vocoderproject_amd/csrc/vp_kernels.h
+++ b/vocoderproject_amd/csrc/vp_kernels.h
@@ -21,6 +21,7 @@
 __global__ void vp_k_pitch_lite_fast_multi_c(VpGeom g, VpCall c, VpDev d, const float *__restrict__ in, float *__restrict__ out);
 __global__ void vp_k_pitch_ws(VpGeom g, VpCall c, VpDev d, VpWsSched sc, const float *__restrict__ in, float *__restrict__ out);
 __global__ void vp_k_pitch_ws_x(VpGeom g, VpCall c, VpDev d, VpWsSched sc, const float *__restrict__ in, float *__restrict__ out);
+__global__ void vp_k_pitch_ws_l(VpGeom g, VpCall c, VpDev d, VpWsSched sc, const float *__restrict__ in, float *__restrict__ out);
 __global__ void vp_k_pitch_ws_mb(VpGeom g, VpCall c, VpDev d, VpWsMb mb, const float *__restrict__ in, float *__restrict__ out);
 __global__ void vp_k_pitch_ws_x_mb(VpGeom g, VpCall c, VpDev d, VpWsMb mb, const float *__restrict__ in, float *__restrict__ out);
 __global__ void vp_k_pitch_ws_mb_o24(VpGeom g, VpCall c, VpDev d, VpWsMb mb, const float *__restrict__ in, float *__restrict__ out);
diff --git a/vocoderproject_amd/csrc/vp_kernels.hip b/vocoderproject_amd/csrc/vp_kernels.hip
--- a/vocoderproject_amd/csrc/vp_kernels.hip
+++ b/vocoderproject_amd/csrc/vp_kernels.hip
@@ -8,7 +8,6 @@
 #define VP_TU 0
 #endif
 #define VP_TU_HAS(K) (VP_TU == 0 || VP_TU == (K))
-#define VP_NUM_TUS 6
 
 #define WAVE 64
 
diff --git a/vocoderproject_amd/csrc/vp_pitch_ws.inc b/vocoderproject_amd/csrc/vp_pitch_ws.inc
--- a/vocoderproject_amd/csrc/vp_pitch_ws.inc
+++ b/vocoderproject_amd/csrc/vp_pitch_ws.inc
@@ -25,11 +25,17 @@
 #endif
 
 typedef __attribute__((address_space(3))) WsCtl lds_ctl;
+__shared__ __attribute__((aligned(16))) int ws_lean_tmo[4];
+template <bool LEAN = false>
 __device__ __forceinline__ void ws_wait_ge(lds_i32 *flag, int target, const VpDev &d)
 {
     int spin = 0;
     while (__hip_atomic_load(flag, __ATOMIC_ACQUIRE, __HIP_MEMORY_SCOPE_WORKGROUP) < target) {
-        if (++spin >= d.spinLimit) { if ((vp_tid() & 63) == 0) vp_timeout(vp_tmo(d, 61)); break; }
+        if (++spin >= d.spinLimit) {
+            if constexpr (LEAN) ws_lean_tmo[0] = 1;
+            else if ((vp_tid() & 63) == 0) vp_timeout(vp_tmo(d, 61));
+            break;
+        }
         __builtin_amdgcn_s_sleep(1);
     }
 }
@@ -38,12 +44,13 @@
     __threadfence_block();
     if ((vp_tid() & 63) == 0) __hip_atomic_store(flag, value, __ATOMIC_RELEASE, __HIP_MEMORY_SCOPE_WORKGROUP);
 }
+template <bool LEAN = false>
 __device__ __forceinline__ void ws_group_barrier(lds_i32 *ctr, int n, int &gen, const VpDev &d)
 {
     gen += 1;
     __threadfence_block();
     if ((vp_tid() & 63) == 0) __hip_atomic_fetch_add(ctr, 1, __ATOMIC_RELEASE, __HIP_MEMORY_SCOPE_WORKGROUP);
-    ws_wait_ge(ctr, n * gen, d);
+    ws_wait_ge<LEAN>(ctr, n * gen, d);
 }
 
 __device__ __forceinline__ void ws_prefix_sums(const lds_f64 *w, lds_f64 *P, int nb)
@@ -158,6 +165,7 @@
         ctl->gNT[sg] = ((ng > 0 || park) && hi > lo) ? (hi - lo + WAVE - 1) / WAVE : 0;
     }
 }
+template <bool LEAN = false>
 __device__ __forceinline__ void ws_psola_gather_seg(const VpGeom &g, const VpDev &d, const PitchLds &L, const SegTab &G, lds_ctl *ctl, int sg, int jA, int jB,
                                                     int kFirst, bool first, const lds_f64 *hpPark = nullptr, int nChunk0 = 0)
 {
@@ -175,7 +183,7 @@
         return b - a;
     };
     auto release = [&](int j) {
-        ws_wait_ge(&ctl->psDone, j, d);
+        ws_wait_ge<LEAN>(&ctl->psDone, j, d);
         for (;;) {
             if (lane == 0) ctl->instMode[j] = hpPark ? 3 : 2;
             ws_signal(&ctl->psDone, j + 1);
@@ -310,7 +318,7 @@
     }
 }
 
-template <bool FAST, bool BIG>
+template <bool FAST, bool BIG, bool LEAN = false>
 __device__ __forceinline__ void ws_background(const VpGeom &g0, const VpCall &c, const VpDev &d, const VpWsSched &sc, lds_f64 *sm, const WsCarve &cv0,
                                               lds_ctl *ctl, int bw, int gateOpen)
 {
@@ -332,6 +340,8 @@
         const int gen = i + 1;
         VpGeom g = g0;
         WsCarve cv = cv0;
+        if constexpr (LEAN) asm volatile("" : "+s"(g.tau0));
+        else
         asm volatile("" : "+s"(g.tauMax), "+s"(g.F), "+s"(g.C), "+s"(g.toKeep), "+s"(g.orderPitch), "+s"(g.tau0));
         asm volatile("" : "+s"(cv.xs), "+s"(cv.fr), "+s"(cv.P), "+s"(cv.dY), "+s"(cv.r), "+s"(cv.aPrev), "+s"(cv.hp), "+s"(cv.xp), "+s"(cv.aF), "+s"(cv.tw));
         L.eF = sm + cv.P;
@@ -342,14 +352,14 @@
         const int lane = vp_tid() & 63;
         if (!gateOpen) {
             if (lead) {
-                ws_wait_ge(&ctl->bgAdopt, i, d);
+                ws_wait_ge<LEAN>(&ctl->bgAdopt, i, d);
                 if (lane == 0) { stBG->nAn = 0; stBG->prevPitch = 0; stBG->gateOpen = 0; ctl->pubMode = 0; }
                 ws_signal(&ctl->bgPub, gen);
             }
             continue;
         }
         const int pn = sc.startPar[i], tS = sc.startStep[i];
-        ws_wait_ge(&ctl->fillTurn, sc.startNeed[i], d);
+        ws_wait_ge<LEAN>(&ctl->fillTurn, sc.startNeed[i], d);
         if (i == 0) WS_EV(d, wq, 0);
         L.xs = sm + cv.xs + ((g.toKeep - g.tauMax) & 1) + tS * g.C;
         L.r = sm + cv.r + pn * 64;
@@ -386,16 +396,16 @@
             if (BIG) {
                 if (FAST) autocorr_rows_fast<true, false>(xf, g.F, order, L.r, 0, 2);
                 else for (int lag0 = 0; lag0 <= order; lag0 += 16) autocorr_rows_exact8(xf, g.F, order, lag0, L.r);
-                ws_wait_ge(&ctl->acDone, gen, d);
+                ws_wait_ge<LEAN>(&ctl->acDone, gen, d);
             } else
             if (FAST) {
                 const double t0 = autocorr_rows_fast_half<true>(xf, g.F, 0);
-                ws_wait_ge(&ctl->acDone, gen, d);
+                ws_wait_ge<LEAN>(&ctl->acDone, gen, d);
                 const double t1 = L.r[32 + (lane & 15)];
                 if (lane < 16 && lane <= order) L.r[lane] = (t0 + t1) / vp_f64_here(g.F);
             } else {
                 if (order >= 8) autocorr_rows_exact8(xf, g.F, order, 8, L.r);
-                ws_wait_ge(&ctl->acDone, gen, d);
+                ws_wait_ge<LEAN>(&ctl->acDone, gen, d);
             }
             if (i == 0) WS_EV(d, wq, 2);
             const bool z = !BIG ? levinson_row16(L.r, L.aPrev, order, VP_ORDER_MAX + 1, g.levEps)
@@ -417,7 +427,7 @@
         if (lead) {
             VP_PRIO_UP();
             int fallback = 1;
-            ws_wait_ge(&ctl->bgAdopt, i, d);
+            ws_wait_ge<LEAN>(&ctl->bgAdopt, i, d);
             if (lane == 0) {
                 stBG->gateOpen = 1;
                 stBG->prevPeriod = stBG->period;
@@ -430,7 +440,7 @@
             wave_sync();
             WS_FINE(d, 1);
             if (xcCert) {
-                ws_wait_ge(&ctl->pDone, gen, d);
+                ws_wait_ge<LEAN>(&ctl->pDone, gen, d);
                 if (i == 0) WS_EV(d, wq, 2);
                 xc_scan_pick(g, L, stBG, xcCert, true);
                 wave_sync();
@@ -447,11 +457,11 @@
             if (i == 0) WS_EV(d, wq, 3);
             VP_PRIO_DOWN();
         }
-        ws_wait_ge(&ctl->pickDone, gen, d);
+        ws_wait_ge<LEAN>(&ctl->pickDone, gen, d);
         if (ctl->pickState) {
             if (lead && lane == 0) { ctl->ishareBG[0] = INT_MAX; ctl->ishareBG[1] = 0; }
             yin2_exact_waves(g, L, base, bw * WAVE + (vp_tid() & 63), 0, WS_NBG, (g.tauMax + 1) >> 1);
-            ws_group_barrier(&ctl->bgBar, WS_NBG, bgBarGen, d);
+            ws_group_barrier<LEAN>(&ctl->bgBar, WS_NBG, bgBarGen, d);
             if (lead) {
                 yin_cumsum_wave(g, L, vp_tid() & 63);
                 wave_sync();
@@ -460,10 +470,10 @@
                 if ((vp_tid() & 63) == 0) ctl->pickT[pn] = (stBG->pitch > 1) ? stBG->period : stBG->prevVoicedPeriod;
                 ws_signal(&ctl->tDone, gen);
             }
-            ws_group_barrier(&ctl->bgBar, WS_NBG, bgBarGen, d);
+            ws_group_barrier<LEAN>(&ctl->bgBar, WS_NBG, bgBarGen, d);
         }
         if (!lead) {
-            if (xcCert) ws_wait_ge(&ctl->xcDone, gen, d);
+            if (xcCert) ws_wait_ge<LEAN>(&ctl->xcDone, gen, d);
             for (int q = bw * WAVE + lane; q < g.F; q += (WS_NBG - 1) * WAVE) { oEn[q] = 0.0; yFn[q] = 0.0; }
             __threadfence_block();
             if (lane == 0) __hip_atomic_fetch_add((lds_i32 *)&ctl->zeroDone, 1, __ATOMIC_RELEASE, __HIP_MEMORY_SCOPE_WORKGROUP);
@@ -481,13 +491,13 @@
         }
         wave_sync();
         if (i == 0) WS_EV(d, wq, 4);
-        ws_wait_ge(&ctl->lpcDone, gen, d);
+        ws_wait_ge<LEAN>(&ctl->lpcDone, gen, d);
         if (stBG->nAn != 0) {
             const int ncopy = ctl->lpcZ[pn] ? VP_ORDER_MAX + 1 : g.orderPitch + 1;
             for (int q = lane; q < ncopy; q += WAVE) stBG->a[q] = L.aPrev[q];
         }
         WS_FINE(d, 4);
-        ws_wait_ge(&ctl->zeroDone, (WS_NBG - 1) * gen, d);
+        ws_wait_ge<LEAN>(&ctl->zeroDone, (WS_NBG - 1) * gen, d);
         WS_FINE(d, 5);
         if (lane == 0) ctl->pubMode = stBG->nAn != 0 ? 2 : 1;
         ws_signal(&ctl->bgPub, gen);
@@ -496,7 +506,7 @@
     }
 }
 
-template <bool FAST>
+template <bool FAST, bool LEAN = false>
 __device__ __forceinline__ void ws_producer(const VpGeom &g, const VpCall &c, const VpDev &d, const VpWsSched &sc, lds_f64 *sm, const WsCarve &cv,
                                             lds_ctl *ctl, int rank, int nP, int gateOpen, bool firstBlock = true, bool lastBlock = true)
 {
@@ -537,20 +547,20 @@
         if (si >= 0) {
             const int jEnd = g.toKeep + g.F + (jB - jA) * g.C;
             if (gateOpen && rank != 0) {
-                ws_wait_ge(&ctl->lpcDone, si + 1, d);
+                ws_wait_ge<LEAN>(&ctl->lpcDone, si + 1, d);
                 WS_TA(d, wq, 1);
                 const lds_f64 *aN = sm + cv.aF + p * WS_AF(g);
                 for (int q = 4 * (tp - WAVE); q < jEnd; q += 4 * (ntp - WAVE)) fir4((const lds_f64 *)L.xs, aN, order, q, jEnd, L.eF);
                 for (int q = jEnd + tp - WAVE; q < g.eLen; q += ntp - WAVE) L.eF[q] = 0.0;
                 WS_TA(d, wq, 2);
-                ws_wait_ge(&ctl->tDone, si + 1, d);
+                ws_wait_ge<LEAN>(&ctl->tDone, si + 1, d);
                 WS_TA(d, wq, 1);
                 const int T = ctl->pickT[p];
                 const double *hg = d.hannTab + d.hannOff[T];
                 for (int q = tp - WAVE; q < 2 * T + 1; q += ntp - WAVE) L.htab[q] = hg[q];
                 WS_TA(d, wq, 2);
             }
-            ws_wait_ge(&ctl->bgPub, si + 1, d);
+            ws_wait_ge<LEAN>(&ctl->bgPub, si + 1, d);
             WS_TA(d, wq, 1);
             WS_FINEP(d, 0);
             mode = ctl->pubMode;
@@ -580,7 +590,7 @@
             }
             if (mode == 1) for (int q = tp; q < jEnd; q += ntp) L.eF[q] = 0.0;
             qValid = mode == 2;
-            ws_group_barrier(&ctl->prodBar, nP, barGen, d);
+            ws_group_barrier<LEAN>(&ctl->prodBar, nP, barGen, d);
             WS_TA(d, wq, 3);
             WS_FINEP(d, 3);
             if (rank == 0) ws_signal(&ctl->bgAdopt, si + 1);
@@ -603,19 +613,19 @@
                     WS_TA(d, wq, 2);
                 }
                 qValid = true;
-                ws_group_barrier(&ctl->prodBar, nP, barGen, d);
+                ws_group_barrier<LEAN>(&ctl->prodBar, nP, barGen, d);
                 WS_TA(d, wq, 3);
             }
         }
         if (mode == 2) {
-            ws_psola_gather_seg(g, d, L, G, ctl, sg, jA, jB, kFirst, rank == 0, hpPark, c.nChunk0);
+            ws_psola_gather_seg<LEAN>(g, d, L, G, ctl, sg, jA, jB, kFirst, rank == 0, hpPark, c.nChunk0);
             WS_FINEP(d, 4);
             WS_TA(d, wq, 5);
-            ws_wait_ge(&ctl->psDone, jB + 1, d);
+            ws_wait_ge<LEAN>(&ctl->psDone, jB + 1, d);
             WS_FINEP(d, 6);
             WS_TA(d, wq, 3);
         } else {
-            ws_group_barrier(&ctl->prodBar, nP, barGen, d);
+            ws_group_barrier<LEAN>(&ctl->prodBar, nP, barGen, d);
             WS_TA(d, wq, 3);
             if (rank == 0) {
                 if (lane <= jB - jA) ctl->instMode[jA + lane] = (lane == 0) ? mode : 0;
@@ -634,7 +644,7 @@
     WS_EV(d, wq, 7);
 }
 
-template <bool FAST, bool BIG>
+template <bool FAST, bool BIG, bool LEAN = false>
 __device__ __forceinline__ void ws_recursion(const VpGeom &g, const VpCall &c, const VpDev &d, const VpWsSched &sc, lds_f64 *sm, const WsCarve &cv,
                                              lds_ctl *ctl, int me, int nIir, double gainPitch)
 {
@@ -668,7 +678,7 @@
         for (; fj < upto; fj++) {
             if (sc.instPar[fj] != me) continue;
             if (!block && __hip_atomic_load(&ctl->fillTurn, __ATOMIC_ACQUIRE, __HIP_MEMORY_SCOPE_WORKGROUP) < fj) break;
-            ws_wait_ge(&ctl->fillTurn, fj, d);
+            ws_wait_ge<LEAN>(&ctl->fillTurn, fj, d);
             double win[8];
             window(fj, win);
             fill(fj, win);
@@ -687,11 +697,15 @@
             int spin = 0;
             while (__hip_atomic_load(&ctl->psDone, __ATOMIC_ACQUIRE, __HIP_MEMORY_SCOPE_WORKGROUP) < j + 1) {
                 flush(j, false);
-                if (++spin >= d.spinLimit) { if (lane == 0) vp_timeout(vp_tmo(d, 61)); break; }
+                if (++spin >= d.spinLimit) {
+                    if constexpr (LEAN) ws_lean_tmo[0] = 1;
+                    else if (lane == 0) vp_timeout(vp_tmo(d, 61));
+                    break;
+                }
                 __builtin_amdgcn_s_sleep(1);
             }
         } else
-        ws_wait_ge(&ctl->psDone, j + 1, d);
+        ws_wait_ge<LEAN>(&ctl->psDone, j + 1, d);
         WS_TA(d, me, 1);
         if (me == 0) WS_FINER(d, j);
         const int mode = ctl->instMode[j];
@@ -726,7 +740,7 @@
             const lds_f64 *aF = sm + cv.aF + p * WS_AF(g), *hpad = sm + cv.hp + p * WS_HP(g);
             if (sc.instStart[j] >= 0) haveR = false;
             else if (!haveR) { iir_block_walk_load(R, aF, order, hpad); haveR = true; }
-            ws_wait_ge(&ctl->psDone, j + 1, d);
+            ws_wait_ge<LEAN>(&ctl->psDone, j + 1, d);
             WS_TA(d, me, 1);
             WS_FINER(d, j);
             if (ctl->instMode[j] == 3) {
@@ -744,6 +758,7 @@
     VP_PRIO_DOWN();
 }
 
+template <bool LEAN = false>
 __device__ __forceinline__ void ws_filler(const VpGeom &g, const VpCall &c, const VpDev &d, const VpWsSched &sc, lds_f64 *sm, const WsCarve &cv,
                                           lds_ctl *ctl, double gainPitch)
 {
@@ -757,7 +772,7 @@
         double win[8];
 #pragma unroll
         for (int u = 0; u < 8; u++) win[u] = (u < nW) ? d.pitchStWin[shift + lane + WAVE * u] : 0.0;
-        ws_wait_ge(&ctl->iirDone, j + 1, d);
+        ws_wait_ge<LEAN>(&ctl->iirDone, j + 1, d);
         if (ctl->instMode[j] >= 1) {
 #pragma unroll
             for (int u = 0; u < 8; u++) if (u < nW) {
@@ -943,11 +958,12 @@
     ws_mb_launder_carve(cv);
 }
 
+#define WS_IS_LEAN false
 #include "vp_pitch_ws_body.inc"
 #define WS_MB 1
 #include "vp_pitch_ws_body.inc"
 #undef WS_MB
-
+#undef WS_IS_LEAN
 #if VP_TU_HAS(6)
 __global__ __launch_bounds__(768) void vp_k_pitch_ws(VpGeom g, VpCall c, VpDev d, VpWsSched sc, const float *__restrict__ in, float *__restrict__ out)
 {
@@ -998,3 +1014,15 @@
     pitch_ws_body_mb<false, true>(g, c, d, &mb, in, out, smem);
 }
 #endif
+#if VP_TU_HAS(10)
+#define WS_IS_LEAN true
+#define WS_LEAN 1
+#include "vp_pitch_ws_body.inc"
+#undef WS_LEAN
+#undef WS_IS_LEAN
+__global__ __launch_bounds__(768) void vp_k_pitch_ws_l(VpGeom g, VpCall c, VpDev d, VpWsSched sc, const float *__restrict__ in, float *__restrict__ out)
+{
+    extern __shared__ double smem[];
+    pitch_ws_body_l(g, c, d, sc, in, out, smem);
+}
+#endif
diff --git a/vocoderproject_amd/csrc/vp_pitch_ws_body.inc b/vocoderproject_amd/csrc/vp_pitch_ws_body.inc
--- a/vocoderproject_amd/csrc/vp_pitch_ws_body.inc
+++ b/vocoderproject_amd/csrc/vp_pitch_ws_body.inc
@@ -10,6 +10,18 @@
     c.inCounter = mbp->inCtr[0]; c.outCounter = mbp->outCtr[0]; c.currCounter = mbp->currCtr[0]; c.nChunk0 = mbp->nChunk0[0];
     ws_mb_launder(g, c, d);
 #define sc (*scp)
+#elif defined(WS_LEAN)
+__device__ __forceinline__ void pitch_ws_body_l(const VpGeom &g_, const VpCall &c_, const VpDev &d_, const VpWsSched &sc, const float *__restrict__ in,
+                                                float *__restrict__ out, double *smem)
+{
+    constexpr bool FAST = true, BIG = false;
+    VpGeom g = g_;
+    g.F = WS_LEAN_F; g.C = WS_LEAN_C; g.H = WS_LEAN_F - WS_LEAN_C; g.cpf = 4; g.toKeep = WS_LEAN_F; g.eLen = 2 * WS_LEAN_F + 3 * WS_LEAN_C;
+    g.orderPitch = WS_LEAN_ORDER; g.tauMax = WS_LEAN_TAUMAX;
+    VpCall c = c_;
+    c.fuseIngest = 1; c.fuseEmit = 1; c.vocOn = 0; c.pitchOn = 1; c.yinCert = 1; c.iirFast = 1; c.pStart = 0;
+    VpDev d = d_;
+    d.outAcc2 = nullptr;
 #else
 template <bool FAST, bool BIG>
 __device__ __forceinline__ void pitch_ws_body(const VpGeom &g, const VpCall &c, const VpDev &d, const VpWsSched &sc, const float *__restrict__ in,
@@ -63,8 +75,12 @@
     const int done0 = c.nChunk0 * g.C;
     typedef float f4v __attribute__((ext_vector_type(4)));
     typedef double d2v __attribute__((ext_vector_type(2)));
+#ifdef WS_LEAN
+    constexpr bool vec = true;
+#else
     const bool vec = ((g.N | g.inSize | c.inCounter | p0 | (idx0 - g.latency) | span) & 3) == 0 && ((c.outCounter | g.outSize | (g.N + g.C)) & 1) == 0 &&
                      g.inSize <= 4 * nt && span <= 4 * nt && g.N + g.C <= 2 * nt && (((size_t)xin | (size_t)vr) & 15) == 0;
+#endif
     f4v gq = {0.f, 0.f, 0.f, 0.f}, xq = {0.f, 0.f, 0.f, 0.f}, w0q = {0.f, 0.f, 0.f, 0.f}, w1q = {0.f, 0.f, 0.f, 0.f}, w2q = {0.f, 0.f, 0.f, 0.f};
     d2v aq = {0.0, 0.0};
     if (vec) {
@@ -249,6 +265,9 @@
         for (int u = 0; u < 2; u++) { const int i = tid + u * nt; if (i < VP_FFT_TW_D2) tw[i] = tv[u]; }
     }
     for (int i = tid; i < (int)(sizeof(WsCtl) / sizeof(int)); i += nt) ((lds_i32 *)ctl)[i] = 0;
+#ifdef WS_LEAN
+    if (tid == 0) ws_lean_tmo[0] = 0;
+#endif
     if (tid >= nt / WAVE && tid < 16) gateRed[tid] = 0.0;
     WS_EV0(d, 1, 1);
     __syncthreads();
@@ -306,15 +325,15 @@
     if (wv >= NW - WS_NBG)
     {
         const int x = wv - (NW - WS_NBG);
-        ws_background<FAST, BIG>(g, c, d, sc, sm, cv, ctl, FAST ? (0x1230 >> (4 * x)) & 15 : x, gateOpen);
+        ws_background<FAST, BIG, WS_IS_LEAN>(g, c, d, sc, sm, cv, ctl, FAST ? (0x1230 >> (4 * x)) & 15 : x, gateOpen);
     }
     else if (wv < nRec)
-        ws_recursion<FAST, BIG>(g, c, d, sc, sm, cv, ctl, wv, nRec, gainPitch);
+        ws_recursion<FAST, BIG, WS_IS_LEAN>(g, c, d, sc, sm, cv, ctl, wv, nRec, gainPitch);
     else if (FAST && wv == 1)
-        ws_filler(g, c, d, sc, sm, cv, ctl, gainPitch);
+        ws_filler<WS_IS_LEAN>(g, c, d, sc, sm, cv, ctl, gainPitch);
     else
 #ifdef WS_MB
-        ws_producer<FAST>(g, c, d, sc, sm, cv, ctl, wv - nFG, nP, gateOpen, blk == 0, blk == nB - 1);
+        ws_producer<FAST, WS_IS_LEAN>(g, c, d, sc, sm, cv, ctl, wv - nFG, nP, gateOpen, blk == 0, blk == nB - 1);
     if (blk != nB - 1) ws_lds_barrier(); else
     __syncthreads();
     if (blk == nB - 1) break;
@@ -322,7 +341,7 @@
     }
 #define out outb
 #else
-        ws_producer<FAST>(g, c, d, sc, sm, cv, ctl, wv - nFG, nP, gateOpen);
+        ws_producer<FAST, WS_IS_LEAN>(g, c, d, sc, sm, cv, ctl, wv - nFG, nP, gateOpen);
     __syncthreads();
 #endif
     STAMP(d, 8);
@@ -357,6 +376,9 @@
         }
         if (c.fuseEmit) ws_emit_block(g, c, d, out, st, (const lds_f64 *)oA);
     }
+#ifdef WS_LEAN
+    if (tid == 0 && ws_lean_tmo[0] != 0) vp_timeout(vp_tmo(d, 61));
+#endif
 #ifdef VP_STAMPS
     if (blockIdx.x == 0 && threadIdx.x == 0) { atomicAdd(&WS_SLOT(d, 0, 7), 1ULL); atomicAdd(&WS_SLOT(d, 0, 5), (unsigned long long)wall_clock64()); }
 #endif
diff --git a/vocoderproject_amd/processor.py b/vocoderproject_amd/processor.py
--- a/vocoderproject_amd/processor.py
+++ b/vocoderproject_amd/processor.py
@@ -107,6 +107,9 @@
     if hasattr(L, "vp_set_wave_specialised"):
         L.vp_set_wave_specialised.argtypes = [C.c_void_p, C.c_int]
         L.vp_get_wave_specialised.argtypes = [C.c_void_p]
+    if hasattr(L, "vp_debug_pitch_symbol"):
+        L.vp_debug_pitch_symbol.argtypes = [C.c_void_p]
+        L.vp_debug_pitch_symbol.restype = C.c_char_p
     if hasattr(L, "vp_debug_set_spin_limit"):
         L.vp_debug_set_spin_limit.argtypes = [C.c_void_p, C.c_int]
     L.vp_read_ub_counters.argtypes = [vp, C.POINTER(C.c_long)]
@@ -287,7 +290,7 @@
         self._chk(self.L.vp_set_time_parallel(self.h, int(bool(on))))
 
     def set_wave_specialised(self, on):
-        self._chk(self.L.vp_set_wave_specialised(self.h, int(bool(on))))
+        self._chk(self.L.vp_set_wave_specialised(self.h, 2 if on == 2 else int(bool(on))))
 
     def set_yin_mode(self, mode):
         self._chk(self.L.vp_set_yin_mode(self.h, {"direct": 0, "fft": 1, "xcorr": 2, "xcorr_force_fallback": 3}[mode] if isinstance(mode, str) else int(mode)))
@@ -479,6 +482,9 @@
 
     def pitch_kernel_name(self):
         return self.L.vp_pitch_kernel_name(self.h).decode()
+
+    def debug_pitch_symbol(self):
+        return self.L.vp_debug_pitch_symbol(self.h).decode()
 
     def debug_set_spin_limit(self, polls):
         self._chk(self.L.vp_debug_set_spin_limit(self.h, int(polls)))
```

Measured after the change: 27.00 million, median of 6. 6.4% higher.
